# vgl-hub/kreeq

Hardware: AMD Instinct MI355X
Metric: distinct+total k-mers/sec at k=21 (count path) (higher is better)
Workload: dtype u64

## Files before the change

include/kreeq_amd.h:

```cpp
#ifndef KREEQ_AMD_H
#define KREEQ_AMD_H

#include <stdint.h>

#ifdef __cplusplus
extern "C" {
#endif

#define KQ_ABI_VERSION 4

typedef enum {
    KQ_OK = 0,
    KQ_ERR_INVALID = -1,
    KQ_ERR_NO_DEVICE = -2,
    KQ_ERR_HIP = -3,
    KQ_ERR_NOMEM = -4,
    KQ_ERR_TABLE_FULL = -5,
    KQ_ERR_CAPACITY = -6,
    KQ_ERR_MISMATCH = -7
} kq_status;

typedef struct kq_handle kq_handle;

typedef struct {
    uint64_t key;
    uint32_t fw[4], bw[4], cov;
    uint32_t hc;
} kq_entry;

typedef struct {
    uint32_t fw, bw, cov;
    uint8_t  isFw;
    uint8_t  pad[3];
} kq_dbgbase;

typedef struct {
    uint64_t total;
    uint64_t unique;
    uint64_t distinct;
    uint64_t missing;
    uint64_t edges;
} kq_stats;

typedef struct {
    uint64_t kmers_counted;
    uint64_t slots_used;
    uint64_t slots_total;
    uint64_t hc_used;
    uint64_t hc_total;
    uint64_t table_bytes;
    uint64_t table_passes;
} kq_info;


int  kq_create(kq_handle** out, int device, int k, int map_count, uint64_t capacity_hint);
void kq_destroy(kq_handle* h);
int  kq_clear(kq_handle* h);
int  kq_set_stream(kq_handle* h, void* hip_stream);
void* kq_get_stream(kq_handle* h);
enum { KQ_OPT_TRUST_CAPACITY = 1, KQ_OPT_COUNT_PATH = 2, KQ_OPT_SLICE_KMERS = 3, KQ_OPT_COUNT_MAP_RANGE = 4, KQ_OPT_PROFILE = 5,
       KQ_OPT_LOOKUP_PATH = 6, KQ_OPT_MERGE_PATH = 7, KQ_OPT_NARROW_MID = 8, KQ_OPT_PENDING_BYTES = 9, KQ_OPT_BUCKET_WINDOW = 10, KQ_OPT_OVERLAP = 11, KQ_OPT_COUNT_MAP_PASSES = 12, KQ_OPT_KERNEL_SET = 13, KQ_OPT_SHARD_WINDOW = 14,
       KQ_OPT_TEST_FAIL_PLAN = 100  };
int  kq_set_option(kq_handle* h, int option, int64_t value);
int  kq_get_profile(kq_handle* h, char* buf, uint64_t cap);
int  kq_sync(kq_handle* h);
int  kq_flush(kq_handle* h);
int  kq_get_info(kq_handle* h, kq_info* out);
const char* kq_last_error(void);
int  kq_abi_version(void);
int  kq_device_available(void);
int  kq_device_memory(int device, uint64_t* free_bytes, uint64_t* total_bytes);


int  kq_count_batch(kq_handle* h, const char* bases, uint64_t len);
int  kq_count_batch_dev(kq_handle* h, const char* d_bases, uint64_t len);

void* kq_host_alloc(uint64_t bytes);
void  kq_host_free(void* p);
int  kq_count_batch_async(kq_handle* h, const char* bases, uint64_t len, uint64_t* ticket);
int  kq_host_wait(kq_handle* h, uint64_t ticket);

void kq_pack_bases(const char* bases, uint64_t len, uint32_t* codes, uint16_t* inv);
int  kq_count_packed_dev(kq_handle* h, const uint32_t* d_codes, const uint16_t* d_inv, uint64_t n_bases);
int  kq_count_packed_async(kq_handle* h, const uint32_t* codes, const uint16_t* inv, uint64_t n_bases, uint64_t* ticket);

int  kq_pack_bases_dev(kq_handle* h, const char* d_bases, uint64_t len, uint32_t* d_codes, uint16_t* d_inv);

enum { KQ_FASTX_FASTQ = 1, KQ_FASTX_FASTA = 2 };
int  kq_parse_fastx_dev(kq_handle* h, const char* d_text, uint64_t len, int format, char* d_bases, uint64_t cap, uint64_t* n_bases);
int  kq_count_fastx_dev(kq_handle* h, const char* d_text, uint64_t len, int format);
int  kq_count_fastx_async(kq_handle* h, const char* text, uint64_t len, int format, uint64_t* ticket);

int  kq_emit_records(kq_handle* h, const char* bases, uint64_t len,
                     uint64_t* keys, uint8_t* edges, uint64_t cap, uint64_t* n_out);
int  kq_emit_partitioned_dev(kq_handle* h, const char* d_bases, uint64_t len, int n_parts,
                             uint64_t* d_keys, uint8_t* d_edges, uint64_t cap,
                             uint64_t* part_counts);

int  kq_emit_packed_dev(kq_handle* h, const char* d_bases, uint64_t len, int n_parts,
                        uint64_t* d_recs, uint64_t cap, uint64_t* part_counts);
int  kq_insert_packed_dev(kq_handle* h, const uint64_t* d_recs, uint64_t n);

int  kq_emit_sharded_dev(kq_handle* h, const char* d_bases, uint64_t len, int n_parts, uint32_t* d_recs, uint8_t* d_aux, uint64_t cap,
                         uint64_t* d_bucket_counts, uint64_t* part_counts);
int  kq_insert_sharded_dev(kq_handle* h, const uint32_t* d_recs, const uint8_t* d_aux, uint64_t n, int n_peers, const uint64_t* d_bucket_counts);

int  kq_emit_sharded8_dev(kq_handle* h, const char* d_bases, uint64_t len, int n_parts, uint64_t* d_recs, uint64_t cap,
                          uint64_t* d_bucket_counts, uint64_t* part_counts);
int  kq_insert_sharded8_dev(kq_handle* h, const uint64_t* d_recs, uint64_t n, int n_peers, const uint64_t* d_bucket_counts);

int  kq_insert_records(kq_handle* h, const uint64_t* keys, const uint8_t* edges, uint64_t n);
int  kq_insert_records_dev(kq_handle* h, const uint64_t* d_keys, const uint8_t* d_edges, uint64_t n);


int  kq_summary(kq_handle* h, kq_stats* out);
int  kq_histogram(kq_handle* h, uint64_t* cov, uint64_t* cnt, uint64_t cap, uint64_t* n_out);


int  kq_lookup_sequence(kq_handle* h, const char* bases, uint64_t len, uint32_t cov_cutoff,
                        uint16_t map_lo, uint16_t map_hi, kq_dbgbase* per_base,
                        uint64_t counters[3]);
int  kq_lookup_sequence_dev(kq_handle* h, const char* d_bases, uint64_t len, uint32_t cov_cutoff,
                            uint16_t map_lo, uint16_t map_hi, kq_dbgbase* d_per_base,
                            uint64_t* d_counters);


int  kq_lookup_keys(kq_handle* h, const uint64_t* keys, uint64_t n, kq_entry* out);

int  kq_branch_scan(kq_handle* h, const char* bases, uint64_t len, uint32_t cov_cutoff, uint8_t* flags);


int  kq_merge(kq_handle* dst, kq_handle* src);

int  kq_import(kq_handle* h, const kq_entry* entries, uint64_t n);
int  kq_export(kq_handle* h, uint16_t map_lo, uint16_t map_hi, kq_entry* out, uint64_t cap,
               uint64_t* n_out);

#ifdef __cplusplus
}
#endif
#endif
```

kreeq_amd/build.py:

```python
import os
import shutil
import subprocess

PKG = os.path.dirname(os.path.abspath(__file__))
ROOT = os.path.dirname(PKG)
LIB = os.path.join(PKG, "lib", "libkreeq_amd.so")
CLI = os.path.join(PKG, "bin", "kreeq")
HOSTLIB = os.path.join(PKG, "lib", "libkreeq_host.so")

HIP_SOURCES = [os.path.join(PKG, "csrc", "kreeq_amd.hip")]
HIP_DEPS = HIP_SOURCES + [os.path.join(PKG, "csrc", f) for f in ("kq_device.h", "kq_partition.h", "kq_kernels.h", "kq_fastx.h")] + [os.path.join(ROOT, "include", "kreeq_amd.h")]
HOST_DIR = os.path.join(PKG, "host")


def _stale(target, deps):
    if not os.path.exists(target):
        return True
    t = os.path.getmtime(target)
    return any(os.path.getmtime(d) > t for d in deps if os.path.exists(d))


def hipcc():
    for c in (shutil.which("hipcc"), "/opt/rocm/bin/hipcc"):
        if c and os.path.exists(c):
            return c
    raise RuntimeError("hipcc not found: the HIP library cannot be built (there is no CPU fallback)")


def build_lib(force=False, verbose=False, out=None, defines=()):
    target = out or LIB
    if force or _stale(target, HIP_DEPS):
        os.makedirs(os.path.dirname(target), exist_ok=True)
        cmd = [hipcc(), "-O3", "-std=c++17", "--offload-arch=gfx950", "-fPIC", "-shared", "-Wall", "-Wextra",
               "-o", target] + ["-D" + d for d in defines] + HIP_SOURCES
        if verbose:
            print(" ".join(cmd))
        subprocess.check_call(cmd)
    return target


def host_sources():
    if not os.path.isdir(HOST_DIR):
        return []
    return sorted(os.path.join(HOST_DIR, f) for f in os.listdir(HOST_DIR) if f.endswith(".cpp") and f != "hostlib.cpp")


def build_hostlib(force=False, verbose=False):
    srcs = [os.path.join(HOST_DIR, f) for f in ("hostlib.cpp", "kreeq_db.cpp")]
    deps = srcs + [os.path.join(HOST_DIR, "kreeq_db.h"), os.path.join(ROOT, "include", "kreeq_amd.h")]
    if force or _stale(HOSTLIB, deps):
        os.makedirs(os.path.dirname(HOSTLIB), exist_ok=True)
        cmd = ["g++", "-O2", "-std=c++17", "-Wall", "-Wextra", "-fPIC", "-shared", "-pthread", "-I", os.path.join(ROOT, "include"), "-o", HOSTLIB] + srcs
        if verbose:
            print(" ".join(cmd))
        subprocess.check_call(cmd)
    return HOSTLIB


def build_cli(force=False, verbose=False):
    srcs = host_sources()
    if not srcs:
        return None
    deps = srcs + [os.path.join(HOST_DIR, f) for f in os.listdir(HOST_DIR) if f.endswith(".h")] + [LIB]
    if force or _stale(CLI, deps):
        os.makedirs(os.path.dirname(CLI), exist_ok=True)
        cmd = ["g++", "-O2", "-std=c++17", "-Wall", "-Wextra", "-pthread", "-I", os.path.join(ROOT, "include"), "-o", CLI] + srcs + \
              ["-L", os.path.dirname(LIB), "-lkreeq_amd", "-lz", "-Wl,-rpath,$ORIGIN/../lib"]
        if verbose:
            print(" ".join(cmd))
        subprocess.check_call(cmd)
    return CLI


def build_all(force=False, verbose=False):
    build_lib(force, verbose)
    build_cli(force, verbose)
    build_hostlib(force, verbose)
```

kreeq_amd/capi.py:

```python
import ctypes as C
import os

import numpy as np

from . import build as _build

ENTRY_DTYPE = np.dtype([("key", "<u8"), ("fw", "<u4", 4), ("bw", "<u4", 4), ("cov", "<u4"), ("hc", "<u4")])
DBGBASE_DTYPE = np.dtype([("fw", "<u4"), ("bw", "<u4"), ("cov", "<u4"), ("isFw", "u1"), ("pad", "u1", 3)])

SYMBOLS = ["kq_create", "kq_destroy", "kq_clear", "kq_set_option", "kq_get_profile", "kq_set_stream", "kq_get_stream", "kq_sync", "kq_flush", "kq_get_info", "kq_last_error",
           "kq_abi_version", "kq_device_available", "kq_device_memory", "kq_count_batch", "kq_count_batch_dev", "kq_host_alloc", "kq_host_free", "kq_count_batch_async", "kq_host_wait", "kq_pack_bases", "kq_count_packed_dev", "kq_count_packed_async",
           "kq_pack_bases_dev", "kq_parse_fastx_dev", "kq_count_fastx_dev", "kq_count_fastx_async", "kq_emit_records",
           "kq_emit_partitioned_dev", "kq_emit_packed_dev", "kq_insert_packed_dev", "kq_emit_sharded_dev", "kq_insert_sharded_dev", "kq_emit_sharded8_dev", "kq_insert_sharded8_dev", "kq_insert_records", "kq_insert_records_dev", "kq_summary", "kq_histogram",
           "kq_lookup_sequence", "kq_lookup_sequence_dev", "kq_lookup_keys", "kq_branch_scan", "kq_merge", "kq_import", "kq_export"]

FASTX_FASTQ, FASTX_FASTA = 1, 2


class KqError(RuntimeError):
    def __init__(self, code, msg):
        super().__init__(f"kreeq_amd error {code}: {msg}")
        self.code = code


class Stats(C.Structure):
    _fields_ = [("total", C.c_uint64), ("unique", C.c_uint64), ("distinct", C.c_uint64), ("missing", C.c_uint64),
                ("edges", C.c_uint64)]


class Info(C.Structure):
    _fields_ = [("kmers_counted", C.c_uint64), ("slots_used", C.c_uint64), ("slots_total", C.c_uint64), ("hc_used", C.c_uint64),
                ("hc_total", C.c_uint64), ("table_bytes", C.c_uint64), ("table_passes", C.c_uint64)]


_lib = None


def lib_path():
    return _build.LIB


def _preload_process_hip_runtime():
    import importlib.util

    try:
        spec = importlib.util.find_spec("torch")
    except (ImportError, ValueError):
        spec = None
    if not spec or not spec.origin:
        return
    d = os.path.join(os.path.dirname(spec.origin), "lib")
    for name in ("libhsa-runtime64.so", "libamdhip64.so"):
        p = os.path.join(d, name)
        if os.path.exists(p):
            try:
                C.CDLL(p, mode=C.RTLD_GLOBAL)
            except OSError:
                return


def load():
    global _lib
    if _lib is not None:
        return _lib
    path = os.environ.get("KQ_LIB") or _build.LIB
    if not os.path.exists(path):
        raise KqError(-2, f"{path} is missing: build it with `python -c 'import __graft_entry__ as g; g.build()'` "
                          "(the product has no CPU fallback)")
    _preload_process_hip_runtime()
    L = C.CDLL(path)
    vp, u64, u32, u16, ci = C.c_void_p, C.c_uint64, C.c_uint32, C.c_uint16, C.c_int
    L.kq_create.argtypes = [C.POINTER(vp), ci, ci, ci, u64]
    L.kq_destroy.argtypes = [vp]
    L.kq_destroy.restype = None
    L.kq_clear.argtypes = [vp]
    L.kq_set_stream.argtypes = [vp, vp]
    L.kq_set_option.argtypes = [vp, ci, C.c_int64]
    L.kq_get_profile.argtypes = [vp, C.c_char_p, u64]
    L.kq_get_stream.argtypes = [vp]
    L.kq_get_stream.restype = vp
    L.kq_sync.argtypes = [vp]
    L.kq_flush.argtypes = [vp]
    L.kq_get_info.argtypes = [vp, C.POINTER(Info)]
    L.kq_last_error.restype = C.c_char_p
    L.kq_device_memory.argtypes = [ci, C.POINTER(u64), C.POINTER(u64)]
    L.kq_count_batch.argtypes = [vp, vp, u64]
    L.kq_count_batch_dev.argtypes = [vp, vp, u64]
    L.kq_host_alloc.argtypes = [u64]
    L.kq_host_alloc.restype = vp
    L.kq_host_free.argtypes = [vp]
    L.kq_host_free.restype = None
    L.kq_count_batch_async.argtypes = [vp, vp, u64, C.POINTER(u64)]
    L.kq_host_wait.argtypes = [vp, u64]
    L.kq_pack_bases.argtypes = [vp, u64, vp, vp]
    L.kq_pack_bases.restype = None
    L.kq_count_packed_dev.argtypes = [vp, vp, vp, u64]
    L.kq_count_packed_async.argtypes = [vp, vp, vp, u64, C.POINTER(u64)]
    L.kq_pack_bases_dev.argtypes = [vp, vp, u64, vp, vp]
    L.kq_parse_fastx_dev.argtypes = [vp, vp, u64, ci, vp, u64, C.POINTER(u64)]
    L.kq_count_fastx_dev.argtypes = [vp, vp, u64, ci]
    L.kq_count_fastx_async.argtypes = [vp, vp, u64, ci, C.POINTER(u64)]
    L.kq_emit_records.argtypes = [vp, vp, u64, vp, vp, u64, C.POINTER(u64)]
    L.kq_emit_partitioned_dev.argtypes = [vp, vp, u64, ci, vp, vp, u64, vp]
    L.kq_emit_packed_dev.argtypes = [vp, vp, u64, ci, vp, u64, vp]
    L.kq_insert_packed_dev.argtypes = [vp, vp, u64]
    L.kq_emit_sharded_dev.argtypes = [vp, vp, u64, ci, vp, vp, u64, vp, vp]
    L.kq_insert_sharded_dev.argtypes = [vp, vp, vp, u64, ci, vp]
    L.kq_emit_sharded8_dev.argtypes = [vp, vp, u64, ci, vp, u64, vp, vp]
    L.kq_insert_sharded8_dev.argtypes = [vp, vp, u64, ci, vp]
    L.kq_insert_records.argtypes = [vp, vp, vp, u64]
    L.kq_insert_records_dev.argtypes = [vp, vp, vp, u64]
    L.kq_summary.argtypes = [vp, C.POINTER(Stats)]
    L.kq_histogram.argtypes = [vp, vp, vp, u64, C.POINTER(u64)]
    L.kq_lookup_sequence.argtypes = [vp, vp, u64, u32, u16, u16, vp, vp]
    L.kq_lookup_sequence_dev.argtypes = [vp, vp, u64, u32, u16, u16, vp, vp]
    L.kq_lookup_keys.argtypes = [vp, vp, u64, vp]
    L.kq_branch_scan.argtypes = [vp, vp, u64, u32, vp]
    L.kq_merge.argtypes = [vp, vp]
    L.kq_import.argtypes = [vp, vp, u64]
    L.kq_export.argtypes = [vp, u16, u16, vp, u64, C.POINTER(u64)]
    _lib = L
    return L


def _check(rc):
    if rc != 0:
        raise KqError(rc, load().kq_last_error().decode(errors="replace"))


def _p(a):
    return a.ctypes.data_as(C.c_void_p) if a is not None else None


def pack_bases(bases: bytes):
    buf = np.frombuffer(bases, dtype=np.uint8)
    units = (len(buf) + 15) // 16
    codes, inv = np.zeros(max(units, 1), dtype=np.uint32), np.zeros(max(units, 1), dtype=np.uint16)
    load().kq_pack_bases(_p(buf) if len(buf) else None, len(buf), _p(codes), _p(inv))
    return codes[:units], inv[:units]


def device_available():
    return bool(load().kq_device_available())


def device_memory(device=0):
    f, t = C.c_uint64(0), C.c_uint64(0)
    _check(load().kq_device_memory(device, C.byref(f), C.byref(t)))
    return f.value, t.value


class KreeqDB:

    def __init__(self, k=21, map_count=128, device=0, capacity_hint=0):
        self.k, self.map_count, self.device = k, map_count, device
        self._h = C.c_void_p()
        _check(load().kq_create(C.byref(self._h), device, k, map_count, capacity_hint))

    def close(self, _load=load):
        if getattr(self, "_h", None):
            _load().kq_destroy(self._h)
            self._h = None

    __del__ = close

    @property
    def handle(self):
        return self._h

    def set_stream(self, hip_stream_ptr):
        _check(load().kq_set_stream(self._h, C.c_void_p(hip_stream_ptr)))

    def sync(self):
        _check(load().kq_sync(self._h))

    def flush(self):
        _check(load().kq_flush(self._h))

    def set_option(self, option, value):
        opt = {"trust_capacity": 1, "count_path": 2, "slice_kmers": 3, "count_map_range": 4, "profile": 5, "lookup_path": 6, "merge_path": 7, "narrow_mid": 8, "pending_bytes": 9, "bucket_window": 10, "overlap": 11, "count_map_passes": 12, "kernel_set": 13, "shard_window": 14, "test_fail_plan": 100}[option]
        if option == "count_map_range":
            value = int(value[0]) | (int(value[1]) << 16)
        if option in ("count_path", "lookup_path", "merge_path"):
            value = {"auto": 0, "direct": 1, "partitioned": 2}[value]
        _check(load().kq_set_option(self._h, opt, int(value)))

    def clear(self):
        _check(load().kq_clear(self._h))

    def profile(self):
        buf = C.create_string_buffer(1024)
        _check(load().kq_get_profile(self._h, buf, 1024))
        return {k: float(v) for k, v in (kv.split("=") for kv in buf.value.decode().split(";") if kv)}

    def info(self):
        i = Info()
        _check(load().kq_get_info(self._h, C.byref(i)))
        return {f: getattr(i, f) for f, _ in Info._fields_}

    def count_batch(self, bases: bytes):
        buf = np.frombuffer(bases, dtype=np.uint8)
        _check(load().kq_count_batch(self._h, _p(buf), len(buf)))

    def count_batch_async(self, host_ptr, n):
        t = C.c_uint64(0)
        _check(load().kq_count_batch_async(self._h, C.c_void_p(host_ptr), n, C.byref(t)))
        return t.value

    def count_packed_dev(self, codes_ptr, inv_ptr, n_bases):
        _check(load().kq_count_packed_dev(self._h, C.c_void_p(codes_ptr), C.c_void_p(inv_ptr), n_bases))

    def count_packed_async(self, codes_ptr, inv_ptr, n_bases):
        t = C.c_uint64(0)
        _check(load().kq_count_packed_async(self._h, C.c_void_p(codes_ptr), C.c_void_p(inv_ptr), n_bases, C.byref(t)))
        return t.value

    def pack_bases_dev(self, bases_ptr, n, codes_ptr, inv_ptr):
        _check(load().kq_pack_bases_dev(self._h, C.c_void_p(bases_ptr), n, C.c_void_p(codes_ptr), C.c_void_p(inv_ptr)))

    def parse_fastx_dev(self, text_ptr, n, fmt, out_ptr, cap):
        nb = C.c_uint64(0)
        rc = load().kq_parse_fastx_dev(self._h, C.c_void_p(text_ptr), n, fmt, C.c_void_p(out_ptr) if out_ptr else None, cap, C.byref(nb))
        if rc != 0:
            e = KqError(rc, load().kq_last_error().decode(errors="replace"))
            e.needed = nb.value
            raise e
        return nb.value

    def count_fastx_dev(self, text_ptr, n, fmt):
        _check(load().kq_count_fastx_dev(self._h, C.c_void_p(text_ptr), n, fmt))

    def count_fastx_async(self, host_ptr, n, fmt):
        t = C.c_uint64(0)
        _check(load().kq_count_fastx_async(self._h, C.c_void_p(host_ptr), n, fmt, C.byref(t)))
        return t.value

    def host_wait(self, ticket):
        _check(load().kq_host_wait(self._h, ticket))

    def count_batch_dev(self, ptr, n):
        _check(load().kq_count_batch_dev(self._h, C.c_void_p(ptr), n))

    def emit_records(self, bases: bytes):
        buf = np.frombuffer(bases, dtype=np.uint8)
        n = C.c_uint64(0)
        _check(load().kq_emit_records(self._h, _p(buf), len(buf), None, None, 0, C.byref(n)))
        keys = np.empty(n.value, dtype=np.uint64)
        edges = np.empty(n.value, dtype=np.uint8)
        if n.value:
            _check(load().kq_emit_records(self._h, _p(buf), len(buf), _p(keys), _p(edges), n.value, C.byref(n)))
        return keys, edges

    def emit_partitioned_dev(self, bases_ptr, n, n_parts, keys_ptr, edges_ptr, cap):
        counts = np.zeros(n_parts, dtype=np.uint64)
        _check(load().kq_emit_partitioned_dev(self._h, C.c_void_p(bases_ptr), n, n_parts, C.c_void_p(keys_ptr), C.c_void_p(edges_ptr),
                                              cap, _p(counts)))
        return counts

    def emit_packed_dev(self, bases_ptr, n, n_parts, recs_ptr, cap):
        counts = np.zeros(n_parts, dtype=np.uint64)
        _check(load().kq_emit_packed_dev(self._h, C.c_void_p(bases_ptr), n, n_parts, C.c_void_p(recs_ptr), cap, _p(counts)))
        return counts

    def insert_packed_dev(self, recs_ptr, n):
        _check(load().kq_insert_packed_dev(self._h, C.c_void_p(recs_ptr), n))

    def emit_sharded_dev(self, bases_ptr, n, n_parts, recs_ptr, aux_ptr, cap, bucket_counts_ptr, sync=True):
        counts = np.zeros(n_parts, dtype=np.uint64) if sync else None
        _check(load().kq_emit_sharded_dev(self._h, C.c_void_p(bases_ptr), n, n_parts, C.c_void_p(recs_ptr), C.c_void_p(aux_ptr), cap,
                                          C.c_void_p(bucket_counts_ptr), _p(counts)))
        return counts

    def insert_sharded_dev(self, recs_ptr, aux_ptr, n, n_peers, bucket_counts_ptr):
        _check(load().kq_insert_sharded_dev(self._h, C.c_void_p(recs_ptr), C.c_void_p(aux_ptr), n, n_peers, C.c_void_p(bucket_counts_ptr)))

    def emit_sharded8_dev(self, bases_ptr, n, n_parts, recs_ptr, cap, bucket_counts_ptr, sync=True):
        counts = np.zeros(n_parts, dtype=np.uint64) if sync else None
        _check(load().kq_emit_sharded8_dev(self._h, C.c_void_p(bases_ptr), n, n_parts, C.c_void_p(recs_ptr), cap,
                                           C.c_void_p(bucket_counts_ptr), _p(counts)))
        return counts

    def insert_sharded8_dev(self, recs_ptr, n, n_peers, bucket_counts_ptr):
        _check(load().kq_insert_sharded8_dev(self._h, C.c_void_p(recs_ptr), n, n_peers, C.c_void_p(bucket_counts_ptr)))

    def insert_records(self, keys, edges):
        keys = np.ascontiguousarray(keys, dtype=np.uint64)
        edges = np.ascontiguousarray(edges, dtype=np.uint8)
        assert len(keys) == len(edges)
        _check(load().kq_insert_records(self._h, _p(keys), _p(edges), len(keys)))

    def insert_records_dev(self, keys_ptr, edges_ptr, n):
        _check(load().kq_insert_records_dev(self._h, C.c_void_p(keys_ptr), C.c_void_p(edges_ptr), n))

    def summary(self, with_hist=False):
        st = Stats()
        _check(load().kq_summary(self._h, C.byref(st)))
        d = {f: getattr(st, f) for f, _ in Stats._fields_}
        if with_hist:
            n = C.c_uint64(0)
            _check(load().kq_histogram(self._h, None, None, 0, C.byref(n)))
            cov = np.zeros(n.value, dtype=np.uint64)
            cnt = np.zeros(n.value, dtype=np.uint64)
            _check(load().kq_histogram(self._h, _p(cov), _p(cnt), n.value, C.byref(n)))
            d["hist"] = dict(zip(cov.tolist(), cnt.tolist()))
        return d

    def lookup_sequence(self, bases: bytes, cov_cutoff=0, map_lo=0, map_hi=None, per_base=False, per_base_buf=None):
        if map_hi is None:
            map_hi = self.map_count
        buf = np.frombuffer(bases, dtype=np.uint8)
        ctr = np.zeros(3, dtype=np.uint64)
        pb = per_base_buf if per_base_buf is not None else (np.zeros(len(buf), dtype=DBGBASE_DTYPE) if per_base else None)
        _check(load().kq_lookup_sequence(self._h, _p(buf), len(buf), cov_cutoff, map_lo, map_hi, _p(pb), _p(ctr)))
        return ctr, pb

    def lookup_sequence_dev(self, bases_ptr, n, counters_ptr, cov_cutoff=0, map_lo=0, map_hi=None, per_base_ptr=None):
        if map_hi is None:
            map_hi = self.map_count
        _check(load().kq_lookup_sequence_dev(self._h, C.c_void_p(bases_ptr), n, cov_cutoff, map_lo, map_hi,
                                             C.c_void_p(per_base_ptr) if per_base_ptr else None, C.c_void_p(counters_ptr)))

    def lookup_keys(self, keys):
        keys = np.ascontiguousarray(keys, dtype=np.uint64)
        out = np.zeros(len(keys), dtype=ENTRY_DTYPE)
        _check(load().kq_lookup_keys(self._h, _p(keys), len(keys), _p(out)))
        return out

    def branch_scan(self, bases: bytes, cov_cutoff=0):
        buf = np.frombuffer(bases, dtype=np.uint8)
        flags = np.zeros(len(buf), dtype=np.uint8)
        _check(load().kq_branch_scan(self._h, _p(buf), len(buf), cov_cutoff, _p(flags)))
        return flags

    def merge(self, other):
        _check(load().kq_merge(self._h, other._h))

    def import_entries(self, entries):
        entries = np.ascontiguousarray(entries, dtype=ENTRY_DTYPE)
        _check(load().kq_import(self._h, _p(entries), len(entries)))

    def export(self, map_lo=0, map_hi=None):
        if map_hi is None:
            map_hi = self.map_count
        n = C.c_uint64(0)
        _check(load().kq_export(self._h, map_lo, map_hi, None, 0, C.byref(n)))
        out = np.zeros(n.value, dtype=ENTRY_DTYPE)
        if n.value:
            _check(load().kq_export(self._h, map_lo, map_hi, _p(out), n.value, C.byref(n)))
        return out
```

kreeq_amd/csrc/kq_kernels.h:

```cpp
#pragma once

#include <hip/hip_runtime.h>

#include <type_traits>

#include "../../include/kreeq_amd.h"
#include "kq_device.h"
#include "kq_partition.h"

using namespace kq;


__global__ __launch_bounds__(TILE_THREADS) void k_count_direct(TableView t, const uint8_t* __restrict__ ab,
                                                                uint64_t lead, uint64_t len, int k, EmitRange er, PartCfg filt,
                                                                const uint16_t* __restrict__ pinv ) {
    uint32_t n_new = 0;
    uint64_t n_kmers = 0;
    scan_tiles(ab, lead, len, k, [&](uint64_t pos, uint64_t fw, uint64_t rv, uint32_t prev, uint32_t next) {
        if (pos < er.lo || pos >= er.hi) return;
        const bool is_fw = fw < rv;
        const uint64_t key = is_fw ? fw : rv;
        if (filt.filt_lo != 0 || filt.filt_hi != filt.map_count) {
            const uint32_t m = map_index(key, filt.map_count, filt.map_mask);
            if (m < filt.filt_lo || m >= filt.filt_hi) return;
// ... 257 lines not shown
                else { recs[cg[it]] = (uint32_t)cv[it]; recs_aux[cg[it]] = (uint8_t)(cv[it] >> 48); }
            }
        }
    }
}

__global__ __launch_bounds__(1024) void k_lv_units(const unsigned long long* __restrict__ seg_off, const unsigned long long* __restrict__ seg_hi, LevelCfg lv,
                                                   unsigned long long* __restrict__ unit_base) {
    __shared__ unsigned long long s_part[1024];
    const uint32_t tid = threadIdx.x, per = (lv.n_seg + 1023) / 1024;
    const uint32_t lo = min(tid * per, lv.n_seg), hi = min(lo + per, lv.n_seg);
    unsigned long long sum = 0;
    for (uint32_t b = lo; b < hi; ++b) sum += (seg_hi[b] - seg_off[b] + P2_UNIT - 1) / P2_UNIT;
    s_part[tid] = sum;
    __syncthreads();
    if (tid < 64) {
        unsigned long long loc[16], tot = 0;
#pragma unroll
        for (int j = 0; j < 16; ++j) { loc[j] = s_part[tid * 16 + j]; tot += loc[j]; }
        unsigned long long incl = tot;
#pragma unroll
        for (int o = 1; o < 64; o <<= 1) { unsigned long long nn = __shfl_up(incl, o, 64); if ((int)tid >= o) incl += nn; }
        unsigned long long run = incl - tot;
#pragma unroll
        for (int j = 0; j < 16; ++j) { s_part[tid * 16 + j] = run; run += loc[j]; }
        if (tid == 63) unit_base[lv.n_seg] = incl;
    }
    __syncthreads();
    unsigned long long run = s_part[tid];
    for (uint32_t b = lo; b < hi; ++b) { unit_base[b] = run; run += (seg_hi[b] - seg_off[b] + P2_UNIT - 1) / P2_UNIT; }
}
__device__ __forceinline__ uint32_t seg_of_unit(const unsigned long long* unit_base, uint32_t n_seg, uint64_t u) {
    uint32_t lo = 0, hi = n_seg;
    while (hi - lo > 1) { uint32_t mid = (lo + hi) >> 1; if (unit_base[mid] <= u) lo = mid; else hi = mid; }
    return lo;
}
template <int FMT>
__global__ __launch_bounds__(MS_THREADS) void k_lv_hist(const uint64_t* __restrict__ recs, const uint8_t* __restrict__ , LevelCfg lv,
                                                        const unsigned long long* __restrict__ seg_off, const unsigned long long* __restrict__ seg_hi,
                                                        const unsigned long long* __restrict__ unit_base, uint32_t* __restrict__ m2) {
    __shared__ uint32_t s_hist[NB_MAX];
    const uint64_t n_units = unit_base[lv.n_seg];
    for (uint64_t u = blockIdx.x; u < n_units; u += gridDim.x) {
        const uint32_t b_in = seg_of_unit(unit_base, lv.n_seg, u);
        const uint32_t b = lv.spb > 1 ? b_in / lv.spb : b_in;
        const uint64_t lo = seg_off[b_in] + (u - unit_base[b_in]) * P2_UNIT;
        const uint64_t hi = lo + P2_UNIT < seg_hi[b_in] ? lo + P2_UNIT : seg_hi[b_in];
        for (uint32_t i = threadIdx.x; i < lv.nb; i += MS_THREADS) s_hist[i] = 0;
        __syncthreads();
        const uint64_t last = hi - 1;
        if (FMT == FMT_NARROW) {
            const uint4* v4 = reinterpret_cast<const uint4*>(recs);
            const uint64_t q0 = lo >> 2, q1 = (hi + 3) >> 2;
            for (uint64_t qb = q0; qb < q1; qb += 4ull * MS_THREADS) {
                uint4 q[4];
#pragma unroll
                for (int j = 0; j < 4; ++j) q[j] = v4[min(qb + (uint64_t)j * MS_THREADS + threadIdx.x, q1 - 1)];
#pragma unroll
                for (int j = 0; j < 4; ++j) {
                    const uint64_t qi = qb + (uint64_t)j * MS_THREADS + threadIdx.x;
                    const uint32_t e[4] = {q[j].x, q[j].y, q[j].z, q[j].w};
#pragma unroll
                    for (int c = 0; c < 4; ++c) {
                        const uint64_t ri = 4 * qi + c;
                        if (qi < q1 && ri >= lo && ri < hi) atomicAdd(&s_hist[narrow_bin(lv, b, e[c])], 1u);
                    }
                }
            }
        } else
        for (uint64_t base = lo; base < hi; base += 8ull * MS_THREADS) {
            uint64_t r[8];
#pragma unroll
            for (int j = 0; j < 8; ++j) {
                const uint64_t i = min(base + (uint64_t)j * MS_THREADS + threadIdx.x, last);
                r[j] = FMT == FMT_NARROW ? (uint64_t)reinterpret_cast<const uint32_t*>(recs)[i] : recs[i];
            }
#pragma unroll
            for (int j = 0; j < 8; ++j)
                if (base + (uint64_t)j * MS_THREADS + threadIdx.x < hi) {
                    const uint32_t bin = FMT == FMT_NARROW ? narrow_bin(lv, b, (uint32_t)r[j])
                        : FMT == FMT_TOP8 ? narrow_bin(lv, b, (uint32_t)(r[j] >> 32))
                        : (FMT == FMT_PACK8 && lv.top8) ? (uint32_t)(rec_hash<false>(r[j]) >> (64 - NARROW_CBITS))
                        : level_bin(lv, b, hash_region(lv.in_raw ? table_hash(r[j], lv.k) : rec_hash<FMT == FMT_WIDE>(r[j]), lv.n_regions));
                    atomicAdd(&s_hist[bin], 1u);
                }
        }
        __syncthreads();
        for (uint32_t i = threadIdx.x; i < lv.nb; i += MS_THREADS) m2[u * lv.nb + i] = s_hist[i];
        __syncthreads();
    }
}
__global__ __launch_bounds__(256) void k_lv_offsets(uint32_t* __restrict__ m2, LevelCfg lv, const unsigned long long* __restrict__ unit_base,
                                                    unsigned long long* __restrict__ group_count) {
    const uint64_t r = ((uint64_t)blockIdx.x * blockDim.x + threadIdx.x) >> 6;
    const uint32_t lane = threadIdx.x & 63;
    const uint32_t n_lseg = lv.n_seg / lv.spb;
    if (r >= (uint64_t)n_lseg * lv.nb) return;
    const uint32_t b = (uint32_t)(r / lv.nb), bin = (uint32_t)(r % lv.nb);
    const uint64_t u0 = unit_base[b * lv.spb], u1 = unit_base[(b + 1) * lv.spb];
    unsigned long long run = 0;
    for (uint64_t base = u0; base < u1; base += 64) {
        const uint64_t u = base + lane;
        const uint32_t c = u < u1 ? m2[u * lv.nb + bin] : 0u;
        unsigned long long incl = c;
#pragma unroll
        for (int o = 1; o < 64; o <<= 1) { const unsigned long long n = __shfl_up(incl, o, 64); if ((int)lane >= o) incl += n; }
        if (u < u1) m2[u * lv.nb + bin] = (uint32_t)(run + incl - c);
        run += __shfl(incl, 63, 64);
    }
    if (lane == 0) group_count[r] = run;
}
__global__ __launch_bounds__(256) void k_lv_offsets_thread(uint32_t* __restrict__ m2, LevelCfg lv, const unsigned long long* __restrict__ unit_base,
                                                           unsigned long long* __restrict__ group_count) {
    const uint64_t r = (uint64_t)blockIdx.x * blockDim.x + threadIdx.x;
    const uint32_t n_lseg = lv.n_seg / lv.spb;
    if (r >= (uint64_t)n_lseg * lv.nb) return;
    const uint32_t b = (uint32_t)(r / lv.nb), bin = (uint32_t)(r % lv.nb);
    const uint64_t u0 = unit_base[b * lv.spb], u1 = unit_base[(b + 1) * lv.spb];
    unsigned long long run = 0;
    for (uint64_t u = u0; u < u1; ++u) {
        const uint32_t c = m2[u * lv.nb + bin];
        m2[u * lv.nb + bin] = (uint32_t)run;
        run += c;
    }
    group_count[r] = run;
}
#ifndef KQ_LV_THREADS
#define KQ_LV_THREADS 512
#define KQ_LV_ITEMS 8
#define KQ_LV_OCC 4
#endif
constexpr int LV_THREADS = KQ_LV_THREADS, LV_ITEMS = KQ_LV_ITEMS, LV_TILE = LV_THREADS * LV_ITEMS;
template <int FMT, int NBC>
__global__ __launch_bounds__(LV_THREADS, KQ_LV_OCC) void k_lv_scatter(const uint64_t* __restrict__ recs, const uint8_t* __restrict__ recs_aux, LevelCfg lv,
                                                           const unsigned long long* __restrict__ seg_off, const unsigned long long* __restrict__ seg_hi,
                                                           const unsigned long long* __restrict__ unit_base, const uint32_t* __restrict__ m2,
                                                           const unsigned long long* __restrict__ group_base, uint64_t* __restrict__ out,
                                                           uint8_t* __restrict__ out_aux) {
    constexpr bool WIDE = FMT == FMT_WIDE, TIGHT = FMT == FMT_NARROW_TO_TIGHT, NARROW = FMT == FMT_NARROW || TIGHT, CONVERT = FMT == FMT_PACK8_TO_NARROW,
                   TOP8 = FMT == FMT_TOP8, HAS_AUX = WIDE || NARROW;
    constexpr int MS_FMT = (CONVERT || TIGHT) ? FMT_NARROW : TOP8 ? FMT_PACK8 : FMT;
    const uint32_t* recs32 = reinterpret_cast<const uint32_t*>(recs);
    __shared__ MsShared<NBC, MS_FMT, LV_TILE> s;
    __shared__ uint32_t s_rst[TIGHT ? NBC : 1];
    const uint32_t nb = lv.nb;
    const uint64_t n_units = unit_base[lv.n_seg];
    for (uint64_t u = blockIdx.x; u < n_units; u += gridDim.x) {
        const uint32_t b_in = seg_of_unit(unit_base, lv.n_seg, u);
        const uint32_t b = lv.spb > 1 ? b_in / lv.spb : b_in;
        const uint64_t lo = seg_off[b_in] + (u - unit_base[b_in]) * P2_UNIT;
        const uint64_t hi = lo + P2_UNIT < seg_hi[b_in] ? lo + P2_UNIT : seg_hi[b_in];
        for (uint32_t i = threadIdx.x; i < nb; i += LV_THREADS)
            s.gbase[i] = (uint32_t)(group_base[(uint64_t)b * nb + i] + m2[u * nb + i]);
        if (TIGHT) {
            const uint32_t first = (b >> lv.nr_shift) * lv.nr_rps + (b & ((1u << lv.nr_shift) - 1u)) * lv.nr_sub;
            for (uint32_t i = threadIdx.x; i < nb; i += LV_THREADS) s_rst[i] = lv.rstart[first + i];
        }
        __syncthreads();
        uint64_t nxt[LV_ITEMS];
        uint32_t nxt_aux[LV_ITEMS];
        const uint64_t last = hi - 1;
#pragma unroll
        for (int j = 0; j < LV_ITEMS; ++j) {
            const uint64_t i = min(lo + (uint64_t)j * LV_THREADS + threadIdx.x, last);
            nxt[j] = NARROW ? (uint64_t)recs32[i] : recs[i];
            nxt_aux[j] = HAS_AUX ? recs_aux[i] : 0;
        }
#pragma unroll
        for (int j = 0; j < LV_ITEMS; ++j) { landed(nxt[j]); if (HAS_AUX) landed(nxt_aux[j]); }
        for (uint64_t pos = lo; pos < hi; pos += LV_TILE) {
            uint64_t rec[LV_ITEMS];
            uint32_t aux[LV_ITEMS], bin[LV_ITEMS];
#pragma unroll
            for (int j = 0; j < LV_ITEMS; ++j) {
                const uint64_t i = pos + (uint64_t)j * LV_THREADS + threadIdx.x;
                rec[j] = (WIDE && lv.in_raw) ? table_hash(nxt[j], lv.k) : nxt[j];
                aux[j] = nxt_aux[j];
                if (TIGHT) {
                    const uint32_t bn = i >= hi ? nb : narrow_bin(lv, b, (uint32_t)rec[j]);
                    rec[j] = narrow_word(tight_rec(b >> lv.nr_shift, (uint32_t)rec[j], aux[j], s_rst[bn < nb ? bn : 0u]), 0u, bn);
                }
                else if (NARROW) rec[j] = narrow_word((uint32_t)rec[j], aux[j], i >= hi ? nb : narrow_bin(lv, b, (uint32_t)rec[j]));
                else if (CONVERT) {
                    const uint64_t hh = rec_hash<false>(rec[j]);
                    rec[j] = narrow_word(narrow_main(hh), narrow_aux(hh, (uint32_t)(rec[j] >> REC_EDGE_SHIFT) & 63u), i >= hi ? nb : (uint32_t)(hh >> (64 - NARROW_CBITS)));
                }
                else if (TOP8) bin[j] = i >= hi ? nb : narrow_bin(lv, b, (uint32_t)(rec[j] >> 32));
                else bin[j] = i >= hi ? nb : level_bin(lv, b, hash_region(rec_hash<WIDE>(rec[j]), lv.n_regions));
            }
#pragma unroll
            for (int j = 0; j < LV_ITEMS; ++j) {
                const uint64_t i = min(pos + LV_TILE + (uint64_t)j * LV_THREADS + threadIdx.x, last);
                nxt[j] = NARROW ? (uint64_t)recs32[i] : recs[i];
                nxt_aux[j] = HAS_AUX ? recs_aux[i] : 0;
            }
            block_multisplit<MS_FMT, LV_THREADS, LV_ITEMS>(s, rec, aux, bin, nb, out, out_aux, [&] {
#pragma unroll
                for (int j = 0; j < LV_ITEMS; ++j) { landed(nxt[j]); if (HAS_AUX) landed(nxt_aux[j]); }
            }, NBC <= 512 ? lv.rep_shift : 0u);
        }
    }
}
#ifndef KQ_LVS_OCC
#define KQ_LVS_OCC 4
#define KQ_LVS_OCC_TIGHT 4
#endif
template <bool TIGHT>
__global__ __launch_bounds__(LV_THREADS, TIGHT ? KQ_LVS_OCC_TIGHT : KQ_LVS_OCC) void k_lv_scatter_s(const uint32_t* __restrict__ recs32, const uint8_t* __restrict__ recs_aux, LevelCfg lv,
                                                           const unsigned long long* __restrict__ seg_off, const unsigned long long* __restrict__ seg_hi,
                                                           const unsigned long long* __restrict__ unit_base, const uint32_t* __restrict__ m2,
                                                           const unsigned long long* __restrict__ group_base, uint32_t* __restrict__ out,
                                                           uint8_t* __restrict__ out_aux) {
    constexpr int NC = 512;
    static_assert(LV_THREADS == NC && LV_ITEMS == 8, "one counter per thread");
    __shared__ uint64_t s_buf[LV_TILE];
    __shared__ uint32_t s_hist[2][NC], s_loff[NC + 1], s_grel[NC], s_wave[LV_THREADS / 64];
    __shared__ uint32_t s_rst[TIGHT ? NC : 1];
    const int tid = threadIdx.x;
    const uint32_t nb = lv.nb, rs = lv.rep_shift, n_ctr = (nb + 1) << rs;
    const uint32_t sub = (uint32_t)tid & ((1u << rs) - 1u), my_bin = (uint32_t)tid >> rs;
    const bool own_bin = sub == 0 && my_bin < nb;
    const uint64_t n_units = unit_base[lv.n_seg];
    for (uint64_t u = blockIdx.x; u < n_units; u += gridDim.x) {
        const uint32_t b_in = seg_of_unit(unit_base, lv.n_seg, u);
        const uint32_t b = lv.spb > 1 ? b_in / lv.spb : b_in;
        const uint64_t lo = seg_off[b_in] + (u - unit_base[b_in]) * P2_UNIT;
        const uint64_t hi = lo + P2_UNIT < seg_hi[b_in] ? lo + P2_UNIT : seg_hi[b_in];
        uint32_t gabs = own_bin ? (uint32_t)(group_base[(uint64_t)b * nb + my_bin] + m2[u * nb + my_bin]) : 0u;
        if (TIGHT) {
            const uint32_t first = (b >> lv.nr_shift) * lv.nr_rps + (b & ((1u << lv.nr_shift) - 1u)) * lv.nr_sub;
            if ((uint32_t)tid < nb) s_rst[tid] = lv.rstart[first + tid];
        }
        s_hist[0][tid] = 0;
        __syncthreads();
        uint32_t nxt[LV_ITEMS], nxt_aux[LV_ITEMS];
        const uint64_t last = hi - 1;
#pragma unroll
        for (int j = 0; j < LV_ITEMS; ++j) {
            const uint64_t i = min(lo + (uint64_t)j * LV_THREADS + tid, last);
            nxt[j] = recs32[i];
            nxt_aux[j] = recs_aux[i];
        }
#pragma unroll
        for (int j = 0; j < LV_ITEMS; ++j) { landed(nxt[j]); landed(nxt_aux[j]); }
        uint32_t par = 0;
        for (uint64_t pos = lo; pos < hi; pos += LV_TILE, par ^= 1u) {
            uint32_t* hist = s_hist[par];
            uint64_t w[LV_ITEMS];
#pragma unroll
            for (int j = 0; j < LV_ITEMS; ++j) {
                const uint64_t i = pos + (uint64_t)j * LV_THREADS + tid;
                const uint32_t bn = i >= hi ? nb : narrow_bin(lv, b, nxt[j]);
                w[j] = TIGHT ? narrow_word(tight_rec(b >> lv.nr_shift, nxt[j], nxt_aux[j], s_rst[bn < nb ? bn : 0u]), 0u, bn) : narrow_word(nxt[j], nxt_aux[j], bn);
                if (bn != nb) atomicAdd(&hist[(bn << rs) | sub], 1u);
            }
#pragma unroll
            for (int j = 0; j < LV_ITEMS; ++j) {
                const uint64_t i = min(pos + LV_TILE + (uint64_t)j * LV_THREADS + tid, last);
                nxt[j] = recs32[i];
                nxt_aux[j] = recs_aux[i];
            }
            __syncthreads();
            const uint32_t cnt = (uint32_t)tid < n_ctr ? hist[tid] : 0u;
            uint32_t incl = cnt;
#pragma unroll
            for (int o = 1; o < 64; o <<= 1) { const uint32_t n = __shfl_up(incl, o, 64); if ((tid & 63) >= o) incl += n; }
            if ((tid & 63) == 63) s_wave[tid >> 6] = incl;
            s_hist[par ^ 1u][tid] = 0;
            __syncthreads();
            uint32_t excl = incl - cnt;
            for (int v = 0; v < (tid >> 6); ++v) excl += s_wave[v];
            s_loff[tid] = excl;
            hist[tid] = excl;
            if (own_bin) s_grel[my_bin] = gabs - excl;
            __syncthreads();
            if (own_bin) gabs += s_loff[(my_bin + 1) << rs] - excl;
#pragma unroll
            for (int j = 0; j < LV_ITEMS; ++j) {
                const uint32_t bn = narrow_word_bin(w[j]);
                if (bn != nb) s_buf[atomicAdd(&hist[(bn << rs) | sub], 1u)] = w[j];
            }
            __syncthreads();
            const uint32_t total = s_loff[nb << rs];
            uint64_t cv[LV_ITEMS];
            uint32_t cg[LV_ITEMS];
#pragma unroll
            for (int it = 0; it < LV_ITEMS; ++it) cv[it] = s_buf[tid + it * LV_THREADS];
#pragma unroll
            for (int it = 0; it < LV_ITEMS; ++it) cg[it] = s_grel[(uint32_t)(tid + it * LV_THREADS) < total ? narrow_word_bin(cv[it]) : 0u] + (tid + it * LV_THREADS);
#pragma unroll
            for (int j = 0; j < LV_ITEMS; ++j) { landed(nxt[j]); landed(nxt_aux[j]); }
#pragma unroll
            for (int it = 0; it < LV_ITEMS; ++it) {
                if ((uint32_t)(tid + it * LV_THREADS) < total) {
                    out[cg[it]] = (uint32_t)cv[it];
                    if (!TIGHT) out_aux[cg[it]] = (uint8_t)(cv[it] >> 48);
                }
            }
        }
    }
}
__global__ void k_set2(unsigned long long* p, unsigned long long a, unsigned long long b) { p[0] = a; p[1] = b; }

constexpr uint32_t SCAN_CHUNK = 16384;
__global__ __launch_bounds__(1024) void k_scan_sums(const unsigned long long* __restrict__ a, uint64_t n, unsigned long long* __restrict__ sums) {
    const uint64_t lo = (uint64_t)blockIdx.x * SCAN_CHUNK, hi = lo + SCAN_CHUNK < n ? lo + SCAN_CHUNK : n;
    unsigned long long v = 0;
    for (uint64_t i = lo + threadIdx.x; i < hi; i += 1024) v += a[i];
    uint64_t t = block_sum(v);
    if (threadIdx.x == 0) sums[blockIdx.x] = t;
}
__global__ __launch_bounds__(1024) void k_scan_apply(unsigned long long* __restrict__ a, uint64_t n, const unsigned long long* __restrict__ sums) {
    __shared__ unsigned long long s_part[1024];
    const uint64_t lo = (uint64_t)blockIdx.x * SCAN_CHUNK + (uint64_t)threadIdx.x * (SCAN_CHUNK / 1024);
    unsigned long long v[SCAN_CHUNK / 1024], sum = 0;
#pragma unroll
    for (uint32_t j = 0; j < SCAN_CHUNK / 1024; ++j) { v[j] = lo + j < n ? a[lo + j] : 0; sum += v[j]; }
    s_part[threadIdx.x] = sum;
    __syncthreads();
    if (threadIdx.x < 64) {
        unsigned long long loc[16], tot = 0;
#pragma unroll
        for (int j = 0; j < 16; ++j) { loc[j] = s_part[threadIdx.x * 16 + j]; tot += loc[j]; }
        unsigned long long incl = tot;
#pragma unroll
        for (int o = 1; o < 64; o <<= 1) { unsigned long long nn = __shfl_up(incl, o, 64); if ((int)threadIdx.x >= o) incl += nn; }
        unsigned long long run = incl - tot;
#pragma unroll
        for (int j = 0; j < 16; ++j) { s_part[threadIdx.x * 16 + j] = run; run += loc[j]; }
    }
    __syncthreads();
    unsigned long long run = sums[blockIdx.x] + s_part[threadIdx.x];
#pragma unroll
    for (uint32_t j = 0; j < SCAN_CHUNK / 1024; ++j) { if (lo + j < n) a[lo + j] = run; run += v[j]; }
}


template <class T> __device__ __forceinline__ T ld_global(const T* p) { return *(const __attribute__((address_space(1))) T*)p; }

template <uint32_t GRP>
struct SetTickets {
    uint64_t lo; uint32_t cnt, first, n_grp;
    __device__ __forceinline__ void build(const P3Set* __restrict__ sets, uint32_t n_sets, uint64_t r, uint32_t lane) {
        lo = 0; cnt = 0;
        if (lane < n_sets) { const unsigned long long* b = ld_global(&sets[lane].base); lo = ld_global(b + r); cnt = (uint32_t)(ld_global(b + r + 1) - lo); }
        const uint32_t mine = (cnt + GRP - 1) / GRP;
        uint32_t incl = mine;
#pragma unroll
        for (int o = 1; o < P3_MAX_SETS; o <<= 1) { const uint32_t v = __shfl_up(incl, o, 64); if ((int)lane >= o) incl += v; }
        first = incl - mine;
        n_grp = __builtin_amdgcn_readlane(incl, 63);
    }
    __device__ __forceinline__ void locate(uint32_t g, uint32_t& q, uint32_t& off, uint32_t& q_cnt, uint64_t& q_lo) const {
        const uint64_t nonempty = __ballot(cnt != 0);
        const uint64_t m = __ballot(cnt != 0 && first <= g);
        q = (g < n_grp && m) ? 63u - (uint32_t)__clzll((unsigned long long)m) : (uint32_t)__ffsll((unsigned long long)nonempty) - 1u;
        const uint32_t f = __builtin_amdgcn_readlane(first, q);
        q_cnt = __builtin_amdgcn_readlane(cnt, q);
        q_lo = ((uint64_t)__builtin_amdgcn_readlane((uint32_t)(lo >> 32), q) << 32) | __builtin_amdgcn_readlane((uint32_t)lo, q);
        off = (g < n_grp ? g - f : 0u) * GRP;
    }
};

template <int THREADS, bool HOT, uint32_t GRP>
__device__ __forceinline__ bool region_gate(SetTickets<GRP>& tk, const TableView& t, const P3Set* __restrict__ sets, uint32_t n_sets, uint64_t r,
                                            int table_is_empty, unsigned long long* __restrict__ hot_list ) {
    const int tid = threadIdx.x;
    tk.build(sets, n_sets, r, (uint32_t)tid & 63u);
    uint64_t n_recs = tk.cnt;
#pragma unroll
    for (int o = 32; o > 0; o >>= 1) n_recs += __shfl_xor(n_recs, o, 64);
    if (n_recs == 0) {
        if (!HOT && table_is_empty == 2) {
            ulonglong2* g2 = reinterpret_cast<ulonglong2*>(t.slots + (r << REGION_SHIFT));
            for (int i = tid; i < (int)REGION_SLOTS; i += THREADS) g2[i] = make_ulonglong2(0ull, 0ull);
        }
        return false;
    }
    if (!HOT && n_recs > 32ull * REGION_SLOTS) {
        if (tid == 0) hot_list[1 + atomicAdd(&hot_list[0], 1ull)] = r;
        return false;
    }
    return true;
}
constexpr int HC_LDS = 64;
__device__ __forceinline__ void hc_lds_reset(uint64_t (&hckey)[HC_LDS], uint32_t (&hccnt)[HC_LDS][8]) {
    const int tid = threadIdx.x;
    if (tid < HC_LDS) {
        hckey[tid] = EMPTY_KEY;
#pragma unroll
        for (int e = 0; e < 8; ++e) hccnt[tid][e] = 0;
    }
}
__device__ __forceinline__ void hc_lds_add(const TableView& t, uint64_t (&hckey)[HC_LDS], uint32_t (&hccnt)[HC_LDS][8], uint64_t h, const uint32_t (&e)[8]) {
    const uint64_t key = key_of_hash(h, t.k);
    int hslot = -1;
    uint32_t hp = (uint32_t)(h >> 40) & (HC_LDS - 1);
    for (int probe = 0; probe < HC_LDS; ++probe, hp = (hp + 1) & (HC_LDS - 1)) {
        uint64_t cur = __hip_atomic_load(&hckey[hp], __ATOMIC_RELAXED, __HIP_MEMORY_SCOPE_WORKGROUP);
        if (cur == EMPTY_KEY) cur = atomicCAS((unsigned long long*)&hckey[hp], (unsigned long long)EMPTY_KEY, (unsigned long long)key);
        if (cur == EMPTY_KEY || cur == key) { hslot = (int)hp; break; }
    }
    if (hslot >= 0) {
#pragma unroll
        for (int w = 0; w < 8; ++w) if (e[w]) atomicAdd(&hccnt[hslot][w], e[w]);
    } else {
        hc_add(t, h, 0, 0, e);
    }
}
__device__ __forceinline__ void hc_lds_flush(const TableView& t, uint64_t (&hckey)[HC_LDS], uint32_t (&hccnt)[HC_LDS][8]) {
    const int tid = threadIdx.x;
    if (tid < HC_LDS && hckey[tid] != EMPTY_KEY) {
        HcSlot* hs = hc_upsert(t, hckey[tid]);
        if (!hs) atomicOr(&t.st->err_hc_full, 1u);
        else {
#pragma unroll
            for (int e = 0; e < 8; ++e) if (hccnt[tid][e]) atomicAdd((unsigned long long*)&hs->cnt[e], (unsigned long long)hccnt[tid][e]);
        }
    }
}
template <class C>
__device__ __forceinline__ void region_totals_wave(uint32_t n_new, uint32_t n_ok, C& s_new, C& s_kmers) {
#pragma unroll
    for (int o = 32; o > 0; o >>= 1) { n_new += __shfl_down(n_new, o, 64); n_ok += __shfl_down(n_ok, o, 64); }
    if ((threadIdx.x & 63) == 0) { if (n_new) atomicAdd(&s_new, (C)n_new); if (n_ok) atomicAdd(&s_kmers, (C)n_ok); }
}
template <class C>
__device__ __forceinline__ void region_totals_store(const TableView& t, const C& s_new, const C& s_kmers) {
    if (threadIdx.x == 0) {
        if (s_new) atomicAdd(&t.st->slots_used, (unsigned long long)s_new);
        if (s_kmers) atomicAdd(&t.st->kmers_added, (unsigned long long)s_kmers);
    }
}

#ifndef KQ_P3_THREADS
#define KQ_P3_THREADS 512
#define KQ_P3_OCC 6
#define KQ_P3_PF 2
#endif
constexpr int P3_THREADS = KQ_P3_THREADS;
template <int FMT, bool HOT>
__global__ __launch_bounds__(P3_THREADS, HOT ? 4 : KQ_P3_OCC) void k_count_regions(TableView t, const P3Set* __restrict__ sets, uint32_t n_sets,
                                                              int aux_fmt, int table_is_empty,
                                                              unsigned long long* __restrict__ hot_list ,
                                                              uint32_t narrow_rps ) {
    constexpr bool WIDE = FMT == FMT_WIDE, NARROW = FMT == FMT_NARROW, TOP8 = FMT == FMT_TOP8, HAS_AUX = WIDE || NARROW;
    constexpr int PF = KQ_P3_PF;
    constexpr uint64_t GRP = 64ull * PF;
// ... 844 lines not shown
```

kreeq_amd/csrc/kq_partition.h:

```cpp
#pragma once
#include "kq_device.h"

namespace kq {

constexpr int MS_THREADS = 256;
constexpr int MS_ITEMS = 16;
constexpr int MS_TILE = MS_THREADS * MS_ITEMS;
constexpr int NB_MAX = 2048;
constexpr int SEG_MAX = 65536;
constexpr uint32_t SUB_BITS_MAX = 8;
constexpr int REC_EDGE_SHIFT = 56;
constexpr int PART_MAX_K = 28;
constexpr int AUX_IDX6 = 0, AUX_EDGE_BYTE = 1, AUX_TIGHT = 2;

struct PartCfg {
    uint64_t n_regions;
    uint32_t g_shift;
    uint32_t n_coarse;
    uint32_t mode;
    uint32_t map_count;
    uint32_t map_mask;
    uint32_t filt_lo, filt_hi;
    uint32_t raw_out;
    uint32_t narrow;
    uint32_t owner_sub;
    uint32_t sub_bits;
    uint32_t win_lo, win_hi;
    uint32_t n_rng;
};

constexpr int P3_MAX_SETS = 64;
struct P3Set { const uint64_t* recs; const uint8_t* aux; const unsigned long long* base; uint64_t n_max; };

struct LevelCfg {
    uint64_t n_regions;
    uint32_t n_seg, nb, seg_shift, out_shift;
    uint32_t in_raw;
    uint32_t k;
    uint32_t narrow;
    uint32_t top8;
    uint32_t nr_shift, nr_rps, nr_sub, nr_div, nr_inv;
    uint32_t nr_mid, nr_fshift, nr_fmask, nr_f24;
    uint32_t spb;
    uint32_t rep_shift;
    const uint32_t* rstart = nullptr;
};
__device__ __forceinline__ uint32_t level_bin(const LevelCfg& lv, uint32_t b, uint64_t region) {
    return (uint32_t)(region >> lv.out_shift) - (lv.seg_shift >= 32 ? 0u : (b << (lv.seg_shift - lv.out_shift)));
}

__device__ __forceinline__ uint32_t edge_idx6(bool is_fw, uint32_t prev, uint32_t next) {
    uint32_t f, b;
    if (is_fw) { f = next < 4 ? next : 7u; b = prev < 4 ? prev : 7u; }
    else       { f = prev < 4 ? 3u - prev : 7u; b = next < 4 ? 3u - next : 7u; }
    return f | (b << 3);
}
__device__ __forceinline__ uint32_t edge_idx6_any(bool is_fw, uint32_t prev, uint32_t next) {
    const uint32_t f = is_fw ? next : prev, b = is_fw ? prev : next, m = is_fw ? 0u : 0x1Bu;
    return (f | (b << 3)) ^ m;
}
__device__ __forceinline__ uint64_t rec_pack(uint64_t key, bool is_fw, uint32_t prev, uint32_t next) {
    return key | ((uint64_t)edge_idx6(is_fw, prev, next) << REC_EDGE_SHIFT);
}
__device__ __forceinline__ uint64_t idx6_to_pack(uint32_t v) {
    const uint32_t f = v & 7u, b = (v >> 3) & 7u;
    return (f < 4 ? 1ull << (8 * f) : 0ull) | (b < 4 ? 1ull << (8 * (4 + b)) : 0ull);
}
__device__ __forceinline__ uint32_t idx6_to_edge_byte(uint32_t v) {
    const uint32_t f = v & 7u, b = (v >> 3) & 7u;
    return (f < 4 ? 1u << (7 - f) : 0u) | (b < 4 ? 1u << (7 - (4 + b)) : 0u);
}
__device__ __forceinline__ uint64_t rec_key(uint64_t rec) { return rec & ((1ull << REC_EDGE_SHIFT) - 1); }
__device__ __forceinline__ uint64_t rec_edge_pack(uint64_t rec) {
    const uint32_t f = (uint32_t)(rec >> REC_EDGE_SHIFT) & 7u, b = (uint32_t)(rec >> (REC_EDGE_SHIFT + 3)) & 7u;
    return (f < 4 ? 1ull << (8 * f) : 0ull) | (b < 4 ? 1ull << (8 * (4 + b)) : 0ull);
}
template <bool WIDE>
__device__ __forceinline__ uint64_t rec_hash(uint64_t rec) { return WIDE ? rec : rec << 8; }
__device__ __forceinline__ uint64_t rec_pack_hash(uint64_t h, bool is_fw, uint32_t prev, uint32_t next) {
    return (h >> 8) | ((uint64_t)edge_idx6(is_fw, prev, next) << REC_EDGE_SHIFT);
}

constexpr int FMT_PACK8 = 0, FMT_WIDE = 1, FMT_NARROW = 2;
constexpr int FMT_PACK8_TO_NARROW = 3;
constexpr uint32_t NARROW_CBITS = 8, NARROW_MAX_K = 21;
constexpr int FMT_TOP8 = 4;
constexpr int FMT_TIGHT = 5;
constexpr int FMT_NARROW_TO_TIGHT = 6;
constexpr uint64_t TIGHT_MIN_REGIONS = 1ull << 16;
__device__ __forceinline__ uint32_t tight_rec(uint32_t bucket, uint32_t main32, uint32_t aux, uint32_t rstart_r) {
    const uint32_t d = ((bucket << (32 - NARROW_CBITS)) | (main32 >> NARROW_CBITS)) - rstart_r;
    return (d << 16) | ((main32 & 0xFFu) << 8) | ((aux & 3u) << 6) | (aux >> 2);
}
__device__ __forceinline__ uint64_t tight_hash(uint32_t t, uint32_t rstart_r) { return ((uint64_t)((t >> 16) + rstart_r) << 32) | ((uint64_t)((t >> 6) & 1023u) << 22); }
__device__ __forceinline__ uint64_t top8_rec(uint64_t h, uint32_t idx6) { return ((h << NARROW_CBITS) & ~63ull) | idx6; }
__device__ __forceinline__ uint64_t top8_hash(uint32_t bucket, uint64_t rec) { return ((uint64_t)bucket << (64 - NARROW_CBITS)) | ((rec & ~63ull) >> NARROW_CBITS); }
__device__ __forceinline__ uint32_t narrow_main(uint64_t h) { return (uint32_t)(h >> (32 - NARROW_CBITS)); }
__device__ __forceinline__ uint32_t narrow_aux(uint64_t h, uint32_t idx6) { return ((uint32_t)(h >> (30 - NARROW_CBITS)) & 3u) | (idx6 << 2); }
__device__ __forceinline__ uint64_t narrow_hash(uint32_t bucket, uint32_t main32, uint32_t aux) {
    return ((uint64_t)bucket << (64 - NARROW_CBITS)) | ((uint64_t)main32 << (32 - NARROW_CBITS)) | ((uint64_t)(aux & 3u) << (30 - NARROW_CBITS));
}
__device__ __forceinline__ uint64_t narrow_word(uint32_t main32, uint32_t aux, uint32_t bin) { return (uint64_t)main32 | ((uint64_t)(bin | (aux << 16)) << 32); }
__device__ __forceinline__ uint32_t narrow_word_bin(uint64_t w) { return (uint32_t)(w >> 32) & 0xFFFFu; }
__device__ __forceinline__ uint32_t narrow_region(uint32_t bucket, uint32_t main32, uint64_t n_regions) {
    return __umulhi((bucket << (32 - NARROW_CBITS)) | (main32 >> NARROW_CBITS), (uint32_t)n_regions);
}
__device__ __forceinline__ uint32_t narrow_bin(const LevelCfg& lv, uint32_t , uint32_t main32) {
    const uint32_t f = main32 >> NARROW_CBITS;
    if (lv.nr_mid) return f >> lv.nr_fshift;
    const uint32_t fs = f & lv.nr_fmask;
    return lv.nr_f24 ? umul24u(fs, lv.nr_sub) >> lv.nr_fshift : (uint32_t)(((uint64_t)fs * lv.nr_sub) >> lv.nr_fshift);
}

template <int NBC, int FMT, int TILE = MS_TILE>
struct MsShared {
    static constexpr int tile = TILE;
    uint64_t stage[TILE];
    uint16_t sbin[FMT != FMT_NARROW ? TILE : 4];
    uint8_t  saux[FMT == FMT_WIDE ? TILE : 8];
    uint32_t hist[NBC];
    uint32_t loff[NBC];
    uint32_t gbase[NBC];
    uint32_t wave_sum[16];
};

template <int THREADS, class S>
__device__ __forceinline__ void ms_scan(S& s, uint32_t nb) {
    constexpr int NBC = (int)(sizeof(s.hist) / sizeof(uint32_t));
    constexpr int MS_BINS_PER_THREAD = (NBC + THREADS - 1) / THREADS;
    const int tid = threadIdx.x;
    uint32_t v[MS_BINS_PER_THREAD], sum = 0;
#pragma unroll
    for (int j = 0; j < MS_BINS_PER_THREAD; ++j) { uint32_t b = MS_BINS_PER_THREAD * tid + j; v[j] = (b < nb) ? s.hist[b] : 0; sum += v[j]; }
    uint32_t incl = sum;
#pragma unroll
    for (int o = 1; o < 64; o <<= 1) { uint32_t n = __shfl_up(incl, o, 64); if ((tid & 63) >= o) incl += n; }
    if ((tid & 63) == 63) s.wave_sum[tid >> 6] = incl;
    __syncthreads();
    uint32_t base = 0;
    for (int w = 0; w < (tid >> 6); ++w) base += s.wave_sum[w];
    uint32_t run = base + incl - sum;
#pragma unroll
    for (int j = 0; j < MS_BINS_PER_THREAD; ++j) { uint32_t b = MS_BINS_PER_THREAD * tid + j; if (b < nb) s.loff[b] = run; run += v[j]; }
    __syncthreads();
}

__device__ __forceinline__ void landed(uint32_t& v) { asm volatile("" : "+v"(v)); }
__device__ __forceinline__ void landed(uint64_t& v) { asm volatile("" : "+v"(v)); }
struct NoHook { __device__ __forceinline__ void operator()() const {} };
template <int FMT, int THREADS = MS_THREADS, int ITEMS = MS_ITEMS, class S, class F = NoHook>
__device__ __forceinline__ void block_multisplit(S& s, const uint64_t (&rec)[ITEMS], const uint32_t (&aux)[ITEMS],
                                                 const uint32_t (&bin)[ITEMS], uint32_t nb,
                                                 uint64_t* __restrict__ out, uint8_t* __restrict__ out_aux, F pre_store = F(), uint32_t rs = 0) {
    const int tid = threadIdx.x;
    const uint32_t sub = (uint32_t)tid & ((1u << rs) - 1u), n_ctr = (nb + 1) << rs;
    for (uint32_t b = tid; b < n_ctr; b += THREADS) s.hist[b] = 0;
    __syncthreads();
    static_assert(THREADS * ITEMS <= S::tile, "round size");
    uint32_t rank[ITEMS];
#pragma unroll
    for (int i = 0; i < ITEMS; ++i) {
        const uint32_t b = FMT == FMT_NARROW ? narrow_word_bin(rec[i]) : bin[i];
        rank[i] = 0;
        if (b != nb) rank[i] = atomicAdd(&s.hist[(b << rs) | sub], 1u);
    }
    __syncthreads();
    ms_scan<THREADS>(s, n_ctr);
    for (uint32_t b = tid; b < nb; b += THREADS) s.gbase[b] -= s.loff[b << rs];
#pragma unroll
    for (int i = 0; i < ITEMS; ++i) {
        const uint32_t b = FMT == FMT_NARROW ? narrow_word_bin(rec[i]) : bin[i];
        if (b == nb) continue;
        const uint32_t p = s.loff[(b << rs) | sub] + rank[i];
        if (FMT == FMT_NARROW) {
            s.stage[p] = rec[i];
        } else {
            s.stage[p] = rec[i];
            s.sbin[p] = (uint16_t)bin[i];
            if (FMT == FMT_WIDE) s.saux[p] = (uint8_t)aux[i];
        }
    }
    __syncthreads();
    const uint32_t total = s.loff[nb << rs];
    uint32_t cb[ITEMS];
    uint32_t cg[ITEMS];
    uint64_t cv[ITEMS];
    if (FMT == FMT_NARROW) {
#pragma unroll
        for (int it = 0; it < ITEMS; ++it) { cv[it] = s.stage[tid + it * THREADS]; cb[it] = (uint32_t)(tid + it * THREADS) < total ? narrow_word_bin(cv[it]) : 0u; }
    } else {
#pragma unroll
        for (int it = 0; it < ITEMS; ++it) { const uint32_t j = tid + it * THREADS; cb[it] = j < total ? s.sbin[j] : 0u; cv[it] = s.stage[j]; }
    }
#pragma unroll
    for (int it = 0; it < ITEMS; ++it) cg[it] = s.gbase[cb[it]] + (tid + it * THREADS);
    pre_store();
#pragma unroll
    for (int it = 0; it < ITEMS; ++it) {
// ... 34 lines not shown
```

kreeq_amd/csrc/kreeq_amd.hip:

```cpp
#include <hip/hip_runtime.h>
#include <hipcub/hipcub.hpp>

#include <algorithm>
#include <cstdarg>
#include <cstdio>
#include <cstdlib>
#include <cstring>
#include <mutex>
#include <new>
#include <numeric>
#include <string>
#include <thread>
#include <type_traits>
#include <vector>

#include "../../include/kreeq_amd.h"
#include "kq_device.h"
#include "kq_partition.h"

using namespace kq;

#include "kq_kernels.h"
#include "kq_fastx.h"


static thread_local std::string g_err;
static int fail(int code, const char* fmt, ...) {
    char buf[512];
    va_list ap; va_start(ap, fmt); vsnprintf(buf, sizeof buf, fmt, ap); va_end(ap);
    g_err = buf;
    return code;
}
#define HIPC(expr)                                                                                   \
    do {                                                                                             \
        hipError_t e_ = (expr);                                                                      \
        if (e_ != hipSuccess)                                                                        \
            return fail(e_ == hipErrorOutOfMemory ? KQ_ERR_NOMEM : KQ_ERR_HIP, "%s: %s (%s:%d)", #expr, \
                        hipGetErrorString(e_), __FILE__, __LINE__);                                  \
    } while (0)

struct Scrambled {
    void* p = nullptr; size_t bytes = 0, chunk = 0;
    std::vector<hipMemGenericAllocationHandle_t> hs;
    bool vmm = false;
};
static void scr_free(Scrambled& b) {
    if (!b.p) return;
    (void)hipDeviceSynchronize();
    if (b.vmm) {
        (void)hipMemUnmap(b.p, b.hs.size() * b.chunk);
        for (auto& hnd : b.hs) (void)hipMemRelease(hnd);
        (void)hipMemAddressFree(b.p, b.hs.size() * b.chunk);
    } else (void)hipFree(b.p);
    b = Scrambled();
}
static bool scr_try_vmm(Scrambled& b, size_t bytes, int device) {
    static const size_t chunk_mb = getenv("KQ_SCRAMBLE_MB") ? (size_t)atoi(getenv("KQ_SCRAMBLE_MB")) : 2;
    if (!chunk_mb) return false;
    hipMemAllocationProp prop = {};
    prop.type = hipMemAllocationTypePinned; prop.location.type = hipMemLocationTypeDevice; prop.location.id = device;
    size_t gran = 0;
    if (hipMemGetAllocationGranularity(&gran, &prop, hipMemAllocationGranularityMinimum) != hipSuccess || !gran) { (void)hipGetLastError(); return false; }
    const size_t chunk = ((chunk_mb << 20) + gran - 1) / gran * gran, n = (bytes + chunk - 1) / chunk;
    void* base = nullptr;
    if (hipMemAddressReserve(&base, n * chunk, 0, nullptr, 0) != hipSuccess) { (void)hipGetLastError(); return false; }
    std::vector<hipMemGenericAllocationHandle_t> hs;
    hs.reserve(n);
    bool ok = true;
    for (size_t i = 0; i < n && ok; ++i) { hipMemGenericAllocationHandle_t hnd; ok = hipMemCreate(&hnd, chunk, &prop, 0) == hipSuccess; if (ok) hs.push_back(hnd); }
    size_t mapped = 0;
    if (ok) {
        size_t mul = 7919;
        while (std::gcd(mul, n) != 1) ++mul;
        for (; mapped < n && ok; ++mapped) ok = hipMemMap((char*)base + mapped * chunk, chunk, 0, hs[(mapped * mul + 13) % n], 0) == hipSuccess;
        if (!ok) --mapped;
    }
    if (ok) {
        hipMemAccessDesc acc = {};
        acc.location = prop.location; acc.flags = hipMemAccessFlagsProtReadWrite;
        ok = hipMemSetAccess(base, n * chunk, &acc, 1) == hipSuccess;
    }
    if (!ok) {
        (void)hipGetLastError();
        if (mapped) (void)hipMemUnmap(base, mapped * chunk);
        for (auto& hnd : hs) (void)hipMemRelease(hnd);
        (void)hipMemAddressFree(base, n * chunk);
        return false;
    }
    b.p = base; b.bytes = n * chunk; b.chunk = chunk; b.hs.swap(hs); b.vmm = true;
    return true;
}
static int scr_ensure(Scrambled& b, size_t need, int device) {
    if (b.bytes >= need) return KQ_OK;
    scr_free(b);
    const size_t sz = need + std::min<size_t>(need / 4, (size_t)256 << 20) + 4096;
    if (scr_try_vmm(b, sz, device)) return KQ_OK;
    if (hipMalloc(&b.p, sz) != hipSuccess) { (void)hipGetLastError(); b.p = nullptr; return fail(KQ_ERR_NOMEM, "partition scratch allocation failed"); }
    b.bytes = sz; b.vmm = false;
    return KQ_OK;
}

struct DevBuf { void* p = nullptr; size_t bytes = 0; };
struct ScratchSet { DevBuf part; Scrambled part2; };

struct kq_handle;
static void arena_release(kq_handle* h);
struct kq_handle {
    int device = 0, k = 0, map_count = 0;
    hipStream_t own_stream = nullptr, stream = nullptr;
    int n_cu = 256;
    Slot* slots = nullptr;
    uint64_t n_regions = 0;
    uint32_t win_lo = 0, win_hi = 256;
    bool windowed = false;
    HcSlot* hc = nullptr;
    uint64_t hc_cap = 0;
    uint32_t* rstart = nullptr;
    DevState* st = nullptr;
    DevState* st_host = nullptr;
    DevBuf scratch;
    DevBuf stage;
    uint64_t kmers_bound = 0;
    uint64_t used_bound = 0;
    uint64_t hc_check_at = 0;
    bool table_empty = true;
    uint32_t mid_rps = 2048;
    int merge_path = 0;
    int lookup_path = 0;
    bool slots_dirty = false;
    bool trust_capacity = false;
    int count_path = 0;
    uint64_t slice_kmers = 1ull << 28;
    bool slice_user = false;
    uint32_t filt_lo = 0, filt_hi = 0;
    bool profile = false;
    std::vector<std::pair<const char*, hipEvent_t>> marks;
    ScratchSet work, fork_work;
    hipStream_t base = nullptr;
    hipStream_t fork_stream[2] = {nullptr, nullptr};
    bool fork_busy[2] = {false, false};
    bool fork_stale[2] = {false, false};
    static constexpr int EV_RING = 64;
    hipEvent_t ev_ring[EV_RING] = {};
    uint64_t ev_next = 0;
    hipEvent_t ev_pass = nullptr;
    int overlap = 1;
    int kernel_set = 0;
    struct HistKey { const void* ab; const void* pinv; uint64_t lead, len, er_lo, er_hi; uint32_t g1, n_rng; int k;
                     bool operator==(const HistKey& o) const { return ab == o.ab && pinv == o.pinv && lead == o.lead && len == o.len && er_lo == o.er_lo && er_hi == o.er_hi && g1 == o.g1 && n_rng == o.n_rng && k == o.k; } };
    struct HistEntry { HistKey key; unsigned long long* m1_all; size_t bytes; };
    std::vector<HistEntry> hist_cache;
    size_t hist_cache_bytes = 0;
    int map_passes = 1;
    void* arena = nullptr; size_t arena_bytes = 0, arena_used = 0;
    Scrambled arena_scr;
    P3Set* d_sets = nullptr;
    int n_pend = 0, pend_fmt = -1, pend_aux_fmt = 0;
    uint64_t pend_records = 0;
    int64_t pend_budget = -1;
    uint64_t table_passes = 0;
    static constexpr int IN_SLOTS = 3, IN_TICKETS = 512;
    hipStream_t copy_stream = nullptr;
    DevBuf in_buf[IN_SLOTS];
    hipEvent_t in_consumed[IN_SLOTS] = {nullptr, nullptr, nullptr};
    std::vector<hipEvent_t> in_copied;
    uint64_t in_next = 0;
    std::mutex in_m;
    uint8_t in_bad[IN_TICKETS] = {};
    DevBuf fx_units, fx_out, in_cmp[IN_SLOTS];
    FxResult* fx_res = nullptr;
    FxResult* fx_res_host = nullptr;
    int fx_bad = 0;
    bool hist_cache_off = false;
    bool test_fail_plan = false;
    DevBuf hot;

    TableView view() const {
        TableView v; v.slots = slots - (reg_lo() << REGION_SHIFT); v.n_regions = n_regions; v.hc = hc; v.hc_mask = hc_cap - 1; v.st = st; v.k = (uint32_t)k;
        v.reg_lo = reg_lo(); v.reg_hi = reg_hi();
        v.rps = k >= HI_K ? (uint32_t)(n_regions >> 8) : 0u;
        v.rstart = rstart;
        return v;
    }
    uint64_t reg_lo() const { return windowed ? (uint64_t)win_lo * (n_regions >> 8) : 0; }
    uint64_t reg_hi() const { return windowed ? (uint64_t)win_hi * (n_regions >> 8) : n_regions; }
    uint64_t n_alloc_regions() const { return reg_hi() - reg_lo(); }
    uint64_t n_slots() const { return n_alloc_regions() << REGION_SHIFT; }
};

static void marks_reset(kq_handle* h);
static int flush_pending(kq_handle* h);

static int ev_get(kq_handle* h, hipEvent_t* out) {
    hipEvent_t& e = h->ev_ring[h->ev_next++ % kq_handle::EV_RING];
    if (!e) HIPC(hipEventCreateWithFlags(&e, hipEventDisableTiming));
    else HIPC(hipEventSynchronize(e));
    *out = e;
    return KQ_OK;
}
static int join_forks(kq_handle* h) {
    for (int w = 0; w < 2; ++w) {
        if (!h->fork_busy[w]) continue;
        hipEvent_t e; int rc = ev_get(h, &e); if (rc) return rc;
        HIPC(hipEventRecord(e, h->fork_stream[w]));
        HIPC(hipStreamWaitEvent(h->base, e, 0));
        h->fork_busy[w] = false;
    }
    return KQ_OK;
}

static int grid_for(const kq_handle* h, uint64_t work_items, int per_block, int per_cu = 8) {
    uint64_t blocks = (work_items + per_block - 1) / per_block;
    uint64_t cap = (uint64_t)h->n_cu * per_cu;
    if (blocks > cap) blocks = cap;
    if (blocks < 1) blocks = 1;
    return (int)blocks;
}

static void arena_release(kq_handle* h) {
    if (!h->arena) return;
    if (h->arena_scr.p) scr_free(h->arena_scr); else (void)hipFree(h->arena);
    h->arena = nullptr; h->arena_bytes = 0;
}
static int ensure_buf(DevBuf& b, size_t need) {
    if (b.bytes >= need) return KQ_OK;
    if (b.p) { HIPC(hipFree(b.p)); b = DevBuf(); }
    size_t sz = need + std::min<size_t>(need / 4, (size_t)256 << 20) + 4096;
    HIPC(hipMalloc(&b.p, sz));
    b.bytes = sz;
    return KQ_OK;
}

static void clear_words(kq_handle* h, void* p, uint32_t words_per_slot, uint64_t n_slots) {
    const uint64_t n_pairs = n_slots * words_per_slot / 2;
    hipLaunchKernelGGL(k_clear_slots, dim3(grid_for(h, n_pairs, 256)), dim3(256), 0, h->stream, (ulonglong2*)p, words_per_slot, n_pairs);
}
static void clear_main(kq_handle* h, Slot* p, uint64_t n_slots) { (void)hipMemsetAsync(p, 0, (size_t)n_slots * sizeof(Slot), h->stream); }
static void materialize(kq_handle* h) {
    if (!h->slots_dirty) return;
    clear_main(h, h->slots, h->n_slots());
    h->slots_dirty = false;
}
static int alloc_main(kq_handle* h, uint64_t n_regions, uint64_t alloc_regions, Slot** out, uint32_t** rstart_out) {
    Slot* p = nullptr;
    uint32_t* rs = nullptr;
    size_t bytes = (size_t)(alloc_regions << REGION_SHIFT) * sizeof(Slot);
    HIPC(hipMalloc((void**)&p, bytes));
    if (hipMalloc((void**)&rs, (size_t)(n_regions + 1) * sizeof(uint32_t)) != hipSuccess) { (void)hipFree(p); return fail(KQ_ERR_NOMEM, "region index allocation failed"); }
    clear_main(h, p, alloc_regions << REGION_SHIFT);
    hipLaunchKernelGGL(k_region_starts, dim3(grid_for(h, n_regions + 1, 256)), dim3(256), 0, h->stream, rs, n_regions);
    *out = p; *rstart_out = rs;
    return KQ_OK;
}
static int alloc_hc(kq_handle* h, uint64_t cap, HcSlot** out) {
    HcSlot* p = nullptr;
    size_t bytes = (size_t)cap * sizeof(HcSlot);
    HIPC(hipMalloc((void**)&p, bytes));
    clear_words(h, p, sizeof(HcSlot) / 8, cap);
    *out = p;
    return KQ_OK;
}

static int read_state_raw(kq_handle* h) {
    HIPC(hipMemcpyAsync(h->st_host, h->st, sizeof(DevState), hipMemcpyDeviceToHost, h->stream));
    HIPC(hipStreamSynchronize(h->stream));
    return KQ_OK;
}
static int read_state(kq_handle* h) {
    int frc = flush_pending(h);
    if (frc) return frc;
    return read_state_raw(h);
}
static int check_errors(kq_handle* h) {
    int rc = read_state(h);
    if (rc) return rc;
    if (h->st_host->err_table_full) return fail(KQ_ERR_TABLE_FULL, "k-mer table region overflow (slots %llu / %llu)",
                                                 (unsigned long long)h->st_host->slots_used, (unsigned long long)h->n_slots());
    if (h->st_host->err_hc_full) return fail(KQ_ERR_TABLE_FULL, "high-copy side table overflow (%llu / %llu)",
                                              (unsigned long long)h->st_host->hc_used, (unsigned long long)h->hc_cap);
    return KQ_OK;
}

static int grow_main(kq_handle* h, uint64_t need_slots) {
    int frc = flush_pending(h);
    if (frc) return frc;
    uint64_t want = h->n_slots(), new_regions = h->n_regions;
    while (want < need_slots) { want *= 2; new_regions *= 2; }
    if (new_regions >= (1ull << 32)) return fail(KQ_ERR_TABLE_FULL, "cannot grow k-mer table to %llu slots: region index overflow", (unsigned long long)want);
    Slot* fresh = nullptr;
    uint32_t* fresh_rs = nullptr;
    int rc = alloc_main(h, new_regions, want >> REGION_SHIFT, &fresh, &fresh_rs);
    if (rc) return rc == KQ_ERR_NOMEM ? fail(KQ_ERR_TABLE_FULL, "cannot grow k-mer table to %llu slots: out of device memory",
                                             (unsigned long long)want) : rc;
    Slot* old = h->slots; const uint64_t n_old = h->n_slots();
    const TableView old_view = h->view();
    uint32_t* old_rs = h->rstart;
    h->slots = fresh; h->n_regions = new_regions; h->rstart = fresh_rs;
    if (h->slots_dirty) h->slots_dirty = false;
    else hipLaunchKernelGGL(k_rehash, dim3(grid_for(h, n_old, 256)), dim3(256), 0, h->stream, h->view(), old_view);
    HIPC(hipStreamSynchronize(h->stream));
    HIPC(hipFree(old));
    if (old_rs) HIPC(hipFree(old_rs));
    return KQ_OK;
}
static int grow_hc(kq_handle* h, uint64_t need) {
    uint64_t want = h->hc_cap;
    while (want < need) want *= 2;
    HcSlot* fresh = nullptr;
    int rc = alloc_hc(h, want, &fresh);
    if (rc) return rc;
    HcSlot* old = h->hc; const uint64_t n_old = h->hc_cap;
    h->hc = fresh; h->hc_cap = want;
    HIPC(hipMemsetAsync(&h->st->hc_used, 0, sizeof(unsigned long long), h->stream));
    hipLaunchKernelGGL(k_rehash_hc, dim3(grid_for(h, n_old, 256)), dim3(256), 0, h->stream, h->view(), old, n_old);
    HIPC(hipStreamSynchronize(h->stream));
    HIPC(hipFree(old));
    return KQ_OK;
}

constexpr uint64_t HC_CAP_BIG = 1ull << 25;
static int reserve(kq_handle* h, uint64_t extra, uint64_t extra_instances) {
    int rc;
    bool state_read = false;
    if (!h->trust_capacity) {
        uint64_t need = (uint64_t)((double)(h->used_bound + extra) / 0.85) + REGION_SLOTS;
        if (need > h->n_slots()) {
            rc = read_state(h); if (rc) return rc;
            state_read = true;
            h->used_bound = h->st_host->slots_used;
            need = (uint64_t)((double)(h->used_bound + extra) / 0.85) + REGION_SLOTS;
            if (need > h->n_slots()) { rc = grow_main(h, need); if (rc) return rc; }
        }
    }
    h->used_bound += extra;
    h->kmers_bound += extra_instances;
    const uint64_t bound = h->kmers_bound / 255 + 1;
    uint64_t need_hc = 2 * std::min<uint64_t>(bound, 1ull << 23);
    if (bound > (1ull << 23)) need_hc = HC_CAP_BIG;
    if (bound > (1ull << 23) && h->kmers_bound >= h->hc_check_at && h->n_pend == 0) {
        if (!state_read) { rc = read_state_raw(h); if (rc) return rc; }
        need_hc = std::max<uint64_t>(need_hc, 8 * h->st_host->hc_used);
        h->hc_check_at = 2 * h->kmers_bound;
    }
    if (need_hc > h->hc_cap) { rc = grow_hc(h, need_hc); if (rc) return rc; }
    return KQ_OK;
}

static inline void aligned_view(const char* d, const uint8_t** ab, uint64_t* lead) {
    uintptr_t p = (uintptr_t)d;
    *lead = p & 15;
    *ab = (const uint8_t*)(p - *lead);
}

static int stage_in(kq_handle* h, const void* host, size_t bytes, void** dev) {
    int rc = ensure_buf(h->stage, bytes + 64);
    if (rc) return rc;
    if (bytes) HIPC(hipMemcpyAsync(h->stage.p, host, bytes, hipMemcpyHostToDevice, h->stream));
    *dev = h->stage.p;
    return KQ_OK;
}

static void parallel_sort_entries(kq_entry* a, uint64_t n) {
    auto less = [](const kq_entry& x, const kq_entry& y) { return x.key < y.key; };
    unsigned hw = std::thread::hardware_concurrency();
    unsigned t = std::max(1u, std::min(16u, hw ? hw : 1u));
    while (t > 1 && n / t < (1u << 16)) t /= 2;
    if (t <= 1) { std::sort(a, a + n, less); return; }
    std::vector<uint64_t> cut(t + 1);
    for (unsigned i = 0; i <= t; ++i) cut[i] = n * i / t;
    {
        std::vector<std::thread> th;
        for (unsigned i = 0; i < t; ++i) th.emplace_back([&, i] { std::sort(a + cut[i], a + cut[i + 1], less); });
        for (auto& x : th) x.join();
    }
    for (unsigned width = 1; width < t; width *= 2) {
        std::vector<std::thread> th;
        for (unsigned i = 0; i + width < t; i += 2 * width) {
            const uint64_t lo = cut[i], mid = cut[i + width], hi = cut[std::min(i + 2 * width, t)];
            th.emplace_back([=] { std::inplace_merge(a + lo, a + mid, a + hi, less); });
        }
        for (auto& x : th) x.join();
    }
}

extern "C" {

const char* kq_last_error(void) { return g_err.c_str(); }
int kq_abi_version(void) { return KQ_ABI_VERSION; }

int kq_device_available(void) {
    int n = 0;
    if (hipGetDeviceCount(&n) != hipSuccess || n <= 0) return 0;
    hipDeviceProp_t p;
    if (hipGetDeviceProperties(&p, 0) != hipSuccess) return 0;
    return strncmp(p.gcnArchName, "gfx950", 6) == 0 ? 1 : 0;
}

int kq_device_memory(int device, uint64_t* free_bytes, uint64_t* total_bytes) {
    if (!free_bytes || !total_bytes) return fail(KQ_ERR_INVALID, "null argument");
    int n = 0;
    if (hipGetDeviceCount(&n) != hipSuccess || n <= 0) return fail(KQ_ERR_NO_DEVICE, "no HIP device visible (this library has no CPU path)");
    if (device < 0 || device >= n) return fail(KQ_ERR_NO_DEVICE, "device %d out of range (%d visible)", device, n);
    HIPC(hipSetDevice(device));
    size_t f = 0, t = 0;
    HIPC(hipMemGetInfo(&f, &t));
    *free_bytes = f; *total_bytes = t;
    return KQ_OK;
}

static uint64_t round_regions(uint64_t regions, int k) {
    if (regions < 16) regions = 16;
    if (regions >= (uint64_t)NB_MAX || k >= HI_K) regions = (regions + 255) / 256 * 256;
    if (regions >= (1ull << 19)) {
        uint32_t sbits = 3;
        while (sbits < SUB_BITS_MAX && (((regions + 255) / 256) >> sbits) > 256) ++sbits;
        const uint64_t unit = 256ull << sbits;
        regions = (regions + unit - 1) / unit * unit;
    }
    return regions;
}
static int set_window(kq_handle* h, uint32_t lo, uint32_t hi, bool shard = false) {
    if (lo >= hi || hi > 256) return fail(KQ_ERR_INVALID, "bucket window [%u, %u) is not a range of the 256 hash-prefix buckets", lo, hi);
    if (shard && h->k > (int)NARROW_MAX_K && h->k < HI_K)
        return fail(KQ_ERR_INVALID, "shard windows need k <= %u (5-byte records) or k >= %d (8-byte hash-remainder records); k = %u..%d shards own map ranges", NARROW_MAX_K, HI_K, NARROW_MAX_K + 1, HI_K - 1);
    if (!shard && h->k > (int)NARROW_MAX_K) return fail(KQ_ERR_INVALID, "bucket windows need k <= %u (5-byte records)", NARROW_MAX_K);
    if (!h->table_empty || h->n_pend || h->kmers_bound) return fail(KQ_ERR_INVALID, "the bucket window is chosen before anything is counted");
    if (h->windowed && hi - lo == h->win_hi - h->win_lo && !(lo == 0 && hi == 256)) {
        HIPC(hipStreamSynchronize(h->stream));
        h->win_lo = lo; h->win_hi = hi;
        return KQ_OK;
    }
    const uint64_t nb = hi - lo;
    const uint64_t alloc_now = h->n_alloc_regions();
    uint64_t virt = round_regions(std::max<uint64_t>((alloc_now + nb - 1) / nb * 256, (uint64_t)NB_MAX), h->k);
    if (virt >= (1ull << 32)) return fail(KQ_ERR_INVALID, "bucket window too narrow for a table of %llu regions", (unsigned long long)alloc_now);
    HIPC(hipStreamSynchronize(h->stream));
    const bool windowed = !(lo == 0 && hi == 256);
    const uint64_t alloc_new = windowed ? (uint64_t)(hi - lo) * (virt >> 8) : virt;
    Slot* fresh = nullptr;
    uint32_t* fresh_rs = nullptr;
    int rc = alloc_main(h, virt, alloc_new, &fresh, &fresh_rs);
    if (rc) return rc;
    HIPC(hipStreamSynchronize(h->stream));
    if (h->slots) (void)hipFree(h->slots);
    if (h->rstart) (void)hipFree(h->rstart);
    h->slots = fresh; h->rstart = fresh_rs;
    h->n_regions = virt; h->win_lo = lo; h->win_hi = hi; h->windowed = windowed;
    h->slots_dirty = false;
    return KQ_OK;
}

int kq_create(kq_handle** out, int device, int k, int map_count, uint64_t capacity_hint) {
    if (!out) return fail(KQ_ERR_INVALID, "out is null");
    *out = nullptr;
    if (k < 2 || k > 32) return fail(KQ_ERR_INVALID, "k must be in 2..32 (got %d)", k);
    if (map_count < 1 || map_count > 65535) return fail(KQ_ERR_INVALID, "map_count must be in 1..65535 (got %d)", map_count);
    int n = 0;
    if (hipGetDeviceCount(&n) != hipSuccess || n <= 0) return fail(KQ_ERR_NO_DEVICE, "no HIP device visible (this library has no CPU path)");
    if (device < 0 || device >= n) return fail(KQ_ERR_NO_DEVICE, "device %d out of range (%d visible)", device, n);
    HIPC(hipSetDevice(device));
    hipDeviceProp_t prop;
    HIPC(hipGetDeviceProperties(&prop, device));
    if (strncmp(prop.gcnArchName, "gfx950", 6) != 0)
        return fail(KQ_ERR_NO_DEVICE, "device %d is %s; this library carries gfx950 code only", device, prop.gcnArchName);
    kq_handle* h = new (std::nothrow) kq_handle();
    if (!h) return fail(KQ_ERR_NOMEM, "host allocation failed");
    h->device = device; h->k = k; h->map_count = map_count; h->n_cu = prop.multiProcessorCount;
    h->filt_hi = (uint32_t)map_count;
    hipError_t e = hipStreamCreateWithFlags(&h->own_stream, hipStreamNonBlocking);
    if (e != hipSuccess) { delete h; return fail(KQ_ERR_HIP, "hipStreamCreate: %s", hipGetErrorString(e)); }
    h->stream = h->base = h->own_stream;
    int rc = KQ_OK;
    do {
        if (hipMalloc((void**)&h->st, sizeof(DevState)) != hipSuccess || hipHostMalloc((void**)&h->st_host, sizeof(DevState)) != hipSuccess) {
            rc = fail(KQ_ERR_NOMEM, "state allocation failed"); break;
        }
        (void)hipMemsetAsync(h->st, 0, sizeof(DevState), h->stream);
        uint64_t slots = (uint64_t)((double)(capacity_hint ? capacity_hint : (1u << 20)) / 0.7);
        const uint64_t regions = round_regions((slots + REGION_SLOTS - 1) >> REGION_SHIFT, k);
        rc = alloc_main(h, regions, regions, &h->slots, &h->rstart); if (rc) break;
        h->n_regions = regions;
        uint64_t hc = 1u << 16;
        rc = alloc_hc(h, hc, &h->hc); if (rc) break;
        h->hc_cap = hc;
        if (hipStreamSynchronize(h->stream) != hipSuccess) { rc = fail(KQ_ERR_HIP, "table initialisation failed"); break; }
    } while (0);
    if (rc) { kq_destroy(h); return rc; }
    *out = h;
    return KQ_OK;
}

void kq_destroy(kq_handle* h) {
    if (!h) return;
    (void)hipSetDevice(h->device);
    if (h->stream) (void)hipStreamSynchronize(h->stream);
    if (h->slots) (void)hipFree(h->slots);
    if (h->rstart) (void)hipFree(h->rstart);
    if (h->hc) (void)hipFree(h->hc);
    if (h->st) (void)hipFree(h->st);
    if (h->st_host) (void)hipHostFree(h->st_host);
    if (h->scratch.p) (void)hipFree(h->scratch.p);
    if (h->stage.p) (void)hipFree(h->stage.p);
    if (h->work.part.p) (void)hipFree(h->work.part.p);
    scr_free(h->work.part2); scr_free(h->fork_work.part2);
    for (auto& e : h->hist_cache) (void)hipFree(e.m1_all);
    for (int w = 0; w < 2; ++w) { if (h->fork_stream[w]) { (void)hipStreamSynchronize(h->fork_stream[w]); (void)hipStreamDestroy(h->fork_stream[w]); } }
    if (h->fork_work.part.p) (void)hipFree(h->fork_work.part.p);
    for (auto e : h->ev_ring) if (e) (void)hipEventDestroy(e);
    if (h->ev_pass) (void)hipEventDestroy(h->ev_pass);
    for (int i = 0; i < kq_handle::IN_SLOTS; ++i) { if (h->in_buf[i].p) (void)hipFree(h->in_buf[i].p); if (h->in_consumed[i]) (void)hipEventDestroy(h->in_consumed[i]); }
    for (auto e : h->in_copied) (void)hipEventDestroy(e);
    for (int i = 0; i < kq_handle::IN_SLOTS; ++i) if (h->in_cmp[i].p) (void)hipFree(h->in_cmp[i].p);
    if (h->fx_units.p) (void)hipFree(h->fx_units.p);
    if (h->fx_out.p) (void)hipFree(h->fx_out.p);
    if (h->fx_res) (void)hipFree(h->fx_res);
    if (h->fx_res_host) (void)hipHostFree(h->fx_res_host);
    if (h->copy_stream) (void)hipStreamDestroy(h->copy_stream);
    arena_release(h);
    if (h->d_sets) (void)hipFree(h->d_sets);
    if (h->hot.p) (void)hipFree(h->hot.p);
    marks_reset(h);
    if (h->own_stream) (void)hipStreamDestroy(h->own_stream);
    delete h;
}

int kq_clear(kq_handle* h) {
    if (!h) return fail(KQ_ERR_INVALID, "null handle");
    HIPC(hipSetDevice(h->device));
    h->slots_dirty = true;
    clear_words(h, h->hc, sizeof(HcSlot) / 8, h->hc_cap);
    HIPC(hipMemsetAsync(h->st, 0, sizeof(DevState), h->stream));
    h->kmers_bound = 0;
    h->used_bound = 0;
    h->hc_check_at = 0;
    h->table_empty = true;
    h->n_pend = 0; h->arena_used = 0; h->pend_records = 0;
    h->fx_bad = 0;
    return KQ_OK;
}

int kq_set_stream(kq_handle* h, void* s) {
    if (!h) return fail(KQ_ERR_INVALID, "null handle");
    HIPC(hipStreamSynchronize(h->stream));
    h->stream = h->base = s ? (hipStream_t)s : h->own_stream;
    return KQ_OK;
}
int kq_set_option(kq_handle* h, int option, int64_t value) {
    if (!h) return fail(KQ_ERR_INVALID, "null handle");
    switch (option) {
        case KQ_OPT_TRUST_CAPACITY: h->trust_capacity = value != 0; return KQ_OK;
        case KQ_OPT_COUNT_PATH:
            if (value < 0 || value > 2) return fail(KQ_ERR_INVALID, "KQ_OPT_COUNT_PATH must be 0, 1 or 2");
            h->count_path = (int)value; return KQ_OK;
        case KQ_OPT_COUNT_MAP_RANGE: {
            const int64_t lo = value & 0xFFFF, hi = (value >> 16) & 0xFFFF;
            if (lo >= hi || hi > h->map_count) return fail(KQ_ERR_INVALID, "map range [%lld,%lld) outside [0,%d]", (long long)lo, (long long)hi, h->map_count);
            h->filt_lo = (uint32_t)lo; h->filt_hi = (uint32_t)hi; return KQ_OK;
        }
        case KQ_OPT_NARROW_MID:
            if (value < 2 || value > (1 << 14)) return fail(KQ_ERR_INVALID, "KQ_OPT_NARROW_MID must be in [2, 16384]");
            h->mid_rps = (uint32_t)value; return KQ_OK;
        case KQ_OPT_MERGE_PATH:
            if (value < 0 || value > 2) return fail(KQ_ERR_INVALID, "KQ_OPT_MERGE_PATH must be 0, 1 or 2");
            h->merge_path = (int)value; return KQ_OK;
        case KQ_OPT_LOOKUP_PATH:
            if (value < 0 || value > 2) return fail(KQ_ERR_INVALID, "KQ_OPT_LOOKUP_PATH must be 0, 1 or 2");
            h->lookup_path = (int)value; return KQ_OK;
        case KQ_OPT_PROFILE: h->profile = value != 0; if (!h->profile) marks_reset(h); return KQ_OK;
        case KQ_OPT_TEST_FAIL_PLAN: h->test_fail_plan = value != 0; return KQ_OK;
        case KQ_OPT_COUNT_MAP_PASSES: {
            if (value != 1 && value != 2 && value != 4 && value != 8) return fail(KQ_ERR_INVALID, "KQ_OPT_COUNT_MAP_PASSES must be 1, 2, 4 or 8");
            if ((h->map_count & (h->map_count - 1)) != 0 || value > h->map_count) return fail(KQ_ERR_INVALID, "KQ_OPT_COUNT_MAP_PASSES needs a power-of-two map count");
            HIPC(hipStreamSynchronize(h->stream));
            for (auto& e : h->hist_cache) (void)hipFree(e.m1_all);
            h->hist_cache.clear(); h->hist_cache_bytes = 0;
            h->map_passes = (int)value; return KQ_OK;
        }
        case KQ_OPT_KERNEL_SET:
            if (value < 0 || value > 7) return fail(KQ_ERR_INVALID, "KQ_OPT_KERNEL_SET is a mask of bits 1, 2, 4");
            h->kernel_set = (int)value; return KQ_OK;
        case KQ_OPT_OVERLAP:
            if (value < 0 || value > 2) return fail(KQ_ERR_INVALID, "KQ_OPT_OVERLAP must be 0, 1 or 2");
            h->overlap = (int)value; return KQ_OK;
        case KQ_OPT_PENDING_BYTES: {
            if (value < -1) return fail(KQ_ERR_INVALID, "KQ_OPT_PENDING_BYTES must be -1 (auto), 0 (off) or a byte count");
            int rc = flush_pending(h);
            if (rc) return rc;
            if (h->arena && value != h->pend_budget) { HIPC(hipStreamSynchronize(h->stream)); arena_release(h); }
            h->pend_budget = value; return KQ_OK;
        }
        case KQ_OPT_BUCKET_WINDOW:
            HIPC(hipSetDevice(h->device));
            return set_window(h, (uint32_t)(value & 0xFFFF), (uint32_t)((value >> 16) & 0xFFFF));
        case KQ_OPT_SHARD_WINDOW:
            HIPC(hipSetDevice(h->device));
            return set_window(h, (uint32_t)(value & 0xFFFF), (uint32_t)((value >> 16) & 0xFFFF), true);
        case KQ_OPT_SLICE_KMERS:
            if (value < 1) return fail(KQ_ERR_INVALID, "KQ_OPT_SLICE_KMERS must be positive");
            h->slice_kmers = (uint64_t)value; h->slice_user = true; return KQ_OK;
        default: return fail(KQ_ERR_INVALID, "unknown option %d", option);
    }
}
int kq_get_profile(kq_handle* h, char* buf, uint64_t cap) {
    if (!h || !buf || !cap) return fail(KQ_ERR_INVALID, "null argument");
    HIPC(hipSetDevice(h->device));
    HIPC(hipStreamSynchronize(h->stream));
    std::string out;
    for (size_t i = 1; i < h->marks.size(); ++i) {
        float ms = 0;
        HIPC(hipEventElapsedTime(&ms, h->marks[i - 1].second, h->marks[i].second));
        char tmp[96];
        snprintf(tmp, sizeof tmp, "%s%s=%.4f", out.empty() ? "" : ";", h->marks[i].first, ms);
        out += tmp;
    }
    if (out.size() + 1 > cap) return fail(KQ_ERR_CAPACITY, "profile buffer too small: need %zu", out.size() + 1);
    memcpy(buf, out.c_str(), out.size() + 1);
    return KQ_OK;
}
void* kq_get_stream(kq_handle* h) { return h ? (void*)h->stream : nullptr; }
int kq_sync(kq_handle* h) {
    if (!h) return fail(KQ_ERR_INVALID, "null handle");
    HIPC(hipSetDevice(h->device));
    HIPC(hipStreamSynchronize(h->stream));
    const int rc = check_errors(h);
    if (h->fx_bad) return fail(KQ_ERR_INVALID, "malformed %s text was submitted for counting and skipped (kq_clear resets this)", h->fx_bad == KQ_FASTX_FASTQ ? "FASTQ" : "FASTA");
    return rc;
}
int kq_flush(kq_handle* h) {
    if (!h) return fail(KQ_ERR_INVALID, "null handle");
    HIPC(hipSetDevice(h->device));
    return flush_pending(h);
}
int kq_get_info(kq_handle* h, kq_info* out) {
    if (!h || !out) return fail(KQ_ERR_INVALID, "null argument");
    HIPC(hipSetDevice(h->device));
    int rc = read_state(h);
    if (rc) return rc;
    out->kmers_counted = h->st_host->kmers_added;
    out->slots_used = h->st_host->slots_used;
    out->slots_total = h->n_slots();
    out->hc_used = h->st_host->hc_used;
    out->hc_total = h->hc_cap;
    out->table_bytes = h->n_slots() * sizeof(Slot) + h->hc_cap * sizeof(HcSlot);
    out->table_passes = h->table_passes;
    return KQ_OK;
}

struct PartPlan {
    PartCfg cfg;
    bool two_level;
    int fmt;
    uint64_t n_max, R;
    uint32_t g1;
    uint64_t m1_n, m2_n, sums_n, groups_n;
    uint64_t *recs1, *recs2;
    uint8_t *aux1, *aux2;
    unsigned long long *m1, *seg_off, *unit_base, *group_base, *sums, *total, *hot;
    uint32_t* m2;
    uint8_t* a1() const { return fmt == FMT_WIDE || fmt == FMT_NARROW ? aux1 : nullptr; }
    uint8_t* a2() const { return fmt == FMT_WIDE || fmt == FMT_NARROW ? aux2 : nullptr; }
};
static void plan_cfg(const kq_handle* h, PartCfg* cfg, bool allow_narrow = false) {
    cfg->n_regions = h->n_regions;
    uint32_t g = 1;
    while (((cfg->n_regions + (1ull << g) - 1) >> g) > 512 && g < 10) ++g;
    while (((cfg->n_regions + (1ull << g) - 1) >> g) >= (uint64_t)NB_MAX) ++g;
    cfg->g_shift = cfg->n_regions < (uint64_t)NB_MAX ? 0 : g;
    cfg->n_coarse = (uint32_t)((cfg->n_regions + (1ull << cfg->g_shift) - 1) >> cfg->g_shift);
    cfg->mode = 0; cfg->map_count = (uint32_t)h->map_count;
    cfg->map_mask = (h->map_count & (h->map_count - 1)) == 0 ? (uint32_t)h->map_count - 1 : 0;
    cfg->filt_lo = 0; cfg->filt_hi = (uint32_t)h->map_count;
    cfg->raw_out = 0;
    cfg->narrow = 0; cfg->sub_bits = 0; cfg->owner_sub = 0; cfg->n_rng = 0; cfg->win_lo = 0; cfg->win_hi = 1u << NARROW_CBITS;
    if (allow_narrow && (h->k <= (int)NARROW_MAX_K || h->k > PART_MAX_K) && cfg->n_regions >= (uint64_t)NB_MAX && cfg->n_regions % (1u << NARROW_CBITS) == 0) {
        const uint64_t rps = cfg->n_regions >> NARROW_CBITS;
        uint32_t sb = 0;
        if (rps >= h->mid_rps) {
            const uint64_t target_nb = std::max<uint64_t>(1, std::min<uint64_t>(256, h->mid_rps / 8));
            while ((rps >> sb) > target_nb && sb < SUB_BITS_MAX && rps % (2ull << sb) == 0) ++sb;
        }
        if ((rps >> sb) < (uint64_t)NB_MAX && (sb > 0 || rps < (uint64_t)NB_MAX)) { cfg->narrow = 1; cfg->sub_bits = sb; }
    }
    if (cfg->narrow) { cfg->n_coarse = 1u << NARROW_CBITS; if (cfg->g_shift == 0) cfg->g_shift = 1; }
}
static int plan_alloc(kq_handle* h, PartPlan* p, uint64_t n_max, uint64_t n_tiles, uint32_t p1_bins, bool allow_narrow = false,
                      uint64_t min_segs = 0 ) {
    if (h->test_fail_plan) { h->test_fail_plan = false; return fail(KQ_ERR_NOMEM, "partition scratch allocation failed (injected by KQ_OPT_TEST_FAIL_PLAN)"); }
    if (n_max >= (1ull << 32) - 16) return fail(KQ_ERR_INVALID, "a partition pass handles fewer than 2^32 records (got %llu): slice the input", (unsigned long long)n_max);
    plan_cfg(h, &p->cfg, allow_narrow);
    n_max = (n_max + 7) & ~7ull;
    p->two_level = p->cfg.g_shift != 0;
    p->fmt = !p->cfg.narrow ? FMT_PACK8 : h->k > PART_MAX_K ? FMT_TOP8 : FMT_NARROW;
    p->n_max = n_max; p->R = p->cfg.n_regions;
    p->g1 = (uint32_t)std::max<uint64_t>(1, std::min<uint64_t>(n_tiles, (uint64_t)h->n_cu * (p1_bins < 512 ? 18 : 12)));
    p->m1_n = (uint64_t)p1_bins * p->g1 * P1_F;
    const uint64_t nb_max = std::max<uint64_t>(std::max<uint64_t>(1ull << p->cfg.g_shift, p->cfg.n_coarse), p->cfg.narrow ? (p->cfg.n_regions >> NARROW_CBITS) >> p->cfg.sub_bits : 0);
    const uint64_t seg_max = std::max<uint64_t>(min_segs, p->cfg.narrow ? ((uint64_t)1 << NARROW_CBITS) << p->cfg.sub_bits : (uint64_t)NB_MAX);
    p->m2_n = (n_max / P2_UNIT + seg_max + 2) * nb_max;
    p->groups_n = std::max<uint64_t>(std::max<uint64_t>(p->R, (uint64_t)p->cfg.n_coarse << p->cfg.g_shift), min_segs) + 2;
    p->sums_n = std::max(p->m1_n, p->groups_n) / SCAN_CHUNK + 2;
    const uint64_t aux_words = (n_max + 7) / 8 + 1;
    const uint64_t rec_words = p->fmt == FMT_NARROW ? n_max / 2 + 2 : n_max;
    const bool split2 = (rec_words + aux_words) * 8 >= ((size_t)512 << 20);
    if (split2) { int rc2 = scr_ensure(h->work.part2, (size_t)(rec_words + aux_words) * 8, h->device); if (rc2) return rc2; }
    const size_t words = (size_t)((split2 ? 1 : 2) * (rec_words + aux_words) + p->m1_n + 2 * (seg_max + 2) + p->groups_n + p->sums_n + 4 + (p->R + 2) + (p->m2_n + 1) / 2);
    int rc = ensure_buf(h->work.part, words * 8);
    if (rc) return rc;
    p->recs1 = (uint64_t*)h->work.part.p;
    p->aux1 = (uint8_t*)(p->recs1 + rec_words);
    uint64_t* rest = (uint64_t*)(p->aux1 + aux_words * 8);
    if (split2) { p->recs2 = (uint64_t*)h->work.part2.p; p->aux2 = (uint8_t*)(p->recs2 + rec_words); }
    else { p->recs2 = rest; p->aux2 = (uint8_t*)(p->recs2 + rec_words); rest = (uint64_t*)(p->aux2 + aux_words * 8); }
    p->m1 = (unsigned long long*)rest;
    p->seg_off = p->m1 + p->m1_n;
    p->unit_base = p->seg_off + seg_max + 2;
    p->group_base = p->unit_base + seg_max + 2;
    p->sums = p->group_base + p->groups_n;
    p->total = p->sums + p->sums_n;
    p->hot = p->total + 4;
    p->m2 = (uint32_t*)(p->hot + p->R + 2);
    return KQ_OK;
}
static void scan_u64(kq_handle* h, unsigned long long* a, uint64_t n, unsigned long long* sums_scratch, unsigned long long* total) {
    if (n <= 2 * SCAN_CHUNK) {
        hipLaunchKernelGGL(k_exclusive_scan, dim3(1), dim3(1024), 0, h->stream, a, n, total);
        return;
    }
    const uint64_t chunks = (n + SCAN_CHUNK - 1) / SCAN_CHUNK;
    hipLaunchKernelGGL(k_scan_sums, dim3((unsigned)chunks), dim3(1024), 0, h->stream, a, n, sums_scratch);
    hipLaunchKernelGGL(k_exclusive_scan, dim3(1), dim3(1024), 0, h->stream, sums_scratch, chunks, total);
    hipLaunchKernelGGL(k_scan_apply, dim3((unsigned)chunks), dim3(1024), 0, h->stream, a, n, sums_scratch);
}
static void mark(kq_handle* h, const char* name) {
    if (!h->profile) return;
    hipEvent_t e;
    if (hipEventCreate(&e) != hipSuccess) return;
    (void)hipEventRecord(e, h->stream);
    h->marks.emplace_back(name, e);
}
static void marks_reset(kq_handle* h) {
    for (auto& m : h->marks) (void)hipEventDestroy(m.second);
    h->marks.clear();
}

static void run_p1(kq_handle* h, PartPlan* p, const PartCfg& cfg, const uint8_t* ab, uint64_t lead, uint64_t len, EmitRange er, uint64_t* out,
                   uint8_t* out_aux, int aux_fmt, const uint16_t* pinv = nullptr ) {
    const bool plain = cfg.mode == 0 && cfg.filt_lo == 0 && cfg.filt_hi == cfg.map_count;
    const bool owner_plain = cfg.mode == 1 && cfg.map_mask != 0 && cfg.filt_lo == 0 && cfg.filt_hi == cfg.map_count;
    const bool narrow_filt = cfg.mode == 0 && cfg.narrow && !plain && cfg.map_mask != 0 && h->k <= (int)NARROW_MAX_K;
    const bool narrow_win = plain && cfg.narrow && (h->k <= (int)NARROW_MAX_K || h->k > PART_MAX_K) && (cfg.win_lo != 0 || cfg.win_hi != (1u << NARROW_CBITS));
    const int binmode = owner_plain ? 3 : narrow_filt ? 4 : narrow_win ? 6 : !plain ? 0 : cfg.narrow ? 2 : 1;
    auto cached_hist = [&](const kq_handle::HistKey& key, size_t bytes, auto launch) -> kq_handle::HistEntry* {
        for (auto& e : h->hist_cache) if (e.key == key) return &e;
        if (h->hist_cache_bytes + bytes > ((size_t)4 << 30)) return nullptr;
        unsigned long long* buf = nullptr;
        if (hipMalloc((void**)&buf, bytes) != hipSuccess) { (void)hipGetLastError(); return nullptr; }
        launch(buf);
        h->hist_cache.push_back(kq_handle::HistEntry{key, buf, bytes});
        h->hist_cache_bytes += bytes;
        return &h->hist_cache.back();
    };
    bool have_hist = false;
    const size_t row = (size_t)p->g1 * sizeof(unsigned long long), block = row << NARROW_CBITS;
    if (narrow_filt && h->map_passes > 1 && P1_F == 1 && !h->hist_cache_off) {
        const uint32_t n = (uint32_t)h->map_passes, per = cfg.map_count / n, rr = cfg.filt_lo / per;
        if (cfg.filt_lo == rr * per && cfg.filt_hi == (rr + 1) * per) {
            const auto* ent = cached_hist({ab, pinv, lead, len, er.lo, er.hi, p->g1, n, h->k}, n * block, [&](unsigned long long* buf) {
                PartCfg all = cfg;
                all.n_rng = n; all.n_coarse = n << NARROW_CBITS;
                if (h->k == 21) hipLaunchKernelGGL((k_p1_hist<5, 21>), dim3(p->g1), dim3(TILE_THREADS), 0, h->stream, ab, lead, len, h->k, all, er, p->g1, buf, pinv);
                else hipLaunchKernelGGL((k_p1_hist<5, 0>), dim3(p->g1), dim3(TILE_THREADS), 0, h->stream, ab, lead, len, h->k, all, er, p->g1, buf, pinv);
            });
            if (ent) {
                (void)hipMemcpyAsync(p->m1, (const char*)ent->m1_all + rr * block, block, hipMemcpyDeviceToDevice, h->stream);
                have_hist = true;
            }
        }
    }
    if (narrow_win && h->map_passes > 1 && P1_F == 1 && !h->hist_cache_off) {
        const auto* ent = cached_hist({ab, pinv, lead, len, er.lo, er.hi, p->g1, 0xB0C4E7u, h->k}, block, [&](unsigned long long* buf) {
            PartCfg all = cfg;
            all.win_lo = 0; all.win_hi = 1u << NARROW_CBITS;
            if (h->k == 21) hipLaunchKernelGGL((k_p1_hist<2, 21>), dim3(p->g1), dim3(TILE_THREADS), 0, h->stream, ab, lead, len, h->k, all, er, p->g1, buf, pinv);
            else hipLaunchKernelGGL((k_p1_hist<2, 0>), dim3(p->g1), dim3(TILE_THREADS), 0, h->stream, ab, lead, len, h->k, all, er, p->g1, buf, pinv);
        });
        if (ent) {
            (void)hipMemcpyAsync(p->m1, ent->m1_all, block, hipMemcpyDeviceToDevice, h->stream);
            if (cfg.win_lo) (void)hipMemsetAsync(p->m1, 0, (size_t)cfg.win_lo * row, h->stream);
            if (cfg.win_hi < (1u << NARROW_CBITS)) (void)hipMemsetAsync((char*)p->m1 + (size_t)cfg.win_hi * row, 0, (size_t)((1u << NARROW_CBITS) - cfg.win_hi) * row, h->stream);
            have_hist = true;
        }
    }
#define KQ_P1H(B, K) hipLaunchKernelGGL((k_p1_hist<B, K>), dim3(p->g1 * P1_F), dim3(TILE_THREADS), 0, h->stream, ab, lead, len, h->k, cfg, er, p->g1, p->m1, pinv)
    if (have_hist) { }
    else if (binmode == 6) { if (h->k == 21) KQ_P1H(6, 21); else if (h->k == 31) KQ_P1H(6, 31); else KQ_P1H(6, 0); }
    else if (binmode == 2) { if (h->k == 21) KQ_P1H(2, 21); else KQ_P1H(2, 0); }
    else if (binmode == 1) { if (h->k == 31) KQ_P1H(1, 31); else KQ_P1H(1, 0); }
    else if (binmode == 3) { if (h->k == 21) KQ_P1H(3, 21); else KQ_P1H(3, 0); }
    else if (binmode == 4) { if (h->k == 21) KQ_P1H(4, 21); else KQ_P1H(4, 0); }
    else KQ_P1H(0, 0);
#undef KQ_P1H
    scan_u64(h, p->m1, (uint64_t)cfg.n_coarse * p->g1 * P1_F, p->sums, p->total);
    hipLaunchKernelGGL(k_p1_offsets, dim3((cfg.n_coarse + 256) / 256), dim3(256), 0, h->stream, p->m1, p->total, cfg, p->g1, p->seg_off);
    mark(h, "k_p1_hist+scan");
    const bool small = cfg.n_coarse < 512;
#define KQ_P1S(W, N, B, K) hipLaunchKernelGGL((k_p1_scatter<W, N, B, K>), dim3(p->g1), dim3(TILE_THREADS), 0, h->stream, ab, lead, len, h->k, cfg, er, p->m1, out, out_aux, aux_fmt, pinv)
#define KQ_P1T(B, K) do { if (h->kernel_set & 1) KQ_P1S(FMT_TOP8, 512, B, K); else \
        hipLaunchKernelGGL((k_p1_scatter_s<B, K, 1, true>), dim3(p->g1), dim3(TILE_THREADS), 0, h->stream, ab, lead, len, h->k, cfg, er, p->m1, (uint32_t*)out, out_aux, pinv); } while (0)
    if (cfg.narrow && h->k > PART_MAX_K) {
        if (narrow_win) { if (h->k == 31) KQ_P1T(6, 31); else KQ_P1T(6, 0); }
        else if (plain && h->k == 31) KQ_P1T(2, 31); else if (plain) KQ_P1T(2, 0); else KQ_P1T(0, 0);
    }
#define KQ_P1N(B, K, T) do { if (h->kernel_set & 1) KQ_P1S(FMT_NARROW, 512, B, K); else \
        hipLaunchKernelGGL((k_p1_scatter_s<B, K, T>), dim3(p->g1), dim3(TILE_THREADS * T), 0, h->stream, ab, lead, len, h->k, cfg, er, p->m1, (uint32_t*)out, out_aux, pinv); } while (0)
    else if (narrow_filt)  { if (h->k == 21) KQ_P1N(4, 21, 1); else KQ_P1N(4, 0, 1); }
    else if (narrow_win)   { if (h->k == 21) KQ_P1N(6, 21, 1); else KQ_P1N(6, 0, 1); }
    else if (cfg.narrow)   { if (plain && h->k == 21) KQ_P1N(2, 21, KQ_P1S_TPR); else if (plain) KQ_P1N(2, 0, KQ_P1S_TPR); else KQ_P1N(0, 0, 1); }
    else if (out_aux && plain && h->k == 31) { if (small) KQ_P1S(FMT_WIDE, 512, 1, 31); else KQ_P1S(FMT_WIDE, NB_MAX, 1, 31); }
    else if (out_aux) { if (small) KQ_P1S(FMT_WIDE, 512, 0, 0); else KQ_P1S(FMT_WIDE, NB_MAX, 0, 0); }
    else if (owner_plain && !out_aux && small) { if (h->k == 21) KQ_P1S(FMT_PACK8, 512, 3, 21); else KQ_P1S(FMT_PACK8, 512, 3, 0); }
    else if (plain)   { if (small) KQ_P1S(FMT_PACK8, 512, 1, 0); else KQ_P1S(FMT_PACK8, NB_MAX, 1, 0); }
    else              { if (small) KQ_P1S(FMT_PACK8, 512, 0, 0); else KQ_P1S(FMT_PACK8, NB_MAX, 0, 0); }
#undef KQ_P1S
#undef KQ_P1N
#undef KQ_P1T
    mark(h, "k_p1_scatter");
}
struct LevelIn { const uint64_t* recs; const uint8_t* aux; const unsigned long long *seg_lo, *seg_hi; uint32_t n_seg, spb; };
static LevelIn own_segments(const PartPlan& p, const uint64_t* recs, const uint8_t* aux, uint32_t n_seg) { return LevelIn{recs, aux, p.seg_off, p.seg_off + 1, n_seg, 1}; }
static void run_level(kq_handle* h, PartPlan* p, const LevelCfg& lv, const LevelIn& src, uint64_t* out, uint8_t* out_aux,
                      unsigned long long* gb = nullptr ) {
    if (!gb) gb = p->group_base;
    const uint64_t* in = src.recs; const uint8_t* in_aux = src.aux;
    const unsigned long long *seg_lo = src.seg_lo, *seg_hi = src.seg_hi;
    LevelCfg lvr = lv;
    lvr.rep_shift = 0;
    while (lvr.rep_shift < 6 && (((uint64_t)lv.nb + 1) << (lvr.rep_shift + 1)) <= 512) ++lvr.rep_shift;
    const LevelCfg& lv_ = lvr;
    const int fmt = lv.narrow == 2 ? FMT_TOP8 : lv.narrow ? FMT_NARROW : in_aux != nullptr ? FMT_WIDE : FMT_PACK8;
    const uint64_t groups = (uint64_t)(lv.n_seg / lv.spb) * lv.nb;
    hipLaunchKernelGGL(k_lv_units, dim3(1), dim3(1024), 0, h->stream, seg_lo, seg_hi, lv_, p->unit_base);
    const unsigned unit_grid = (unsigned)std::min<uint64_t>(p->n_max / P2_UNIT + lv.n_seg + 1, 1u << 30);
    if (fmt == FMT_TOP8) hipLaunchKernelGGL(k_lv_hist<FMT_TOP8>, dim3(unit_grid), dim3(MS_THREADS), 0, h->stream, in, in_aux, lv_, seg_lo, seg_hi, p->unit_base, p->m2);
    else if (fmt == FMT_NARROW) hipLaunchKernelGGL(k_lv_hist<FMT_NARROW>, dim3(unit_grid), dim3(MS_THREADS), 0, h->stream, in, in_aux, lv_, seg_lo, seg_hi, p->unit_base, p->m2);
    else if (fmt == FMT_WIDE) hipLaunchKernelGGL(k_lv_hist<FMT_WIDE>, dim3(unit_grid), dim3(MS_THREADS), 0, h->stream, in, in_aux, lv_, seg_lo, seg_hi, p->unit_base, p->m2);
    else hipLaunchKernelGGL(k_lv_hist<FMT_PACK8>, dim3(unit_grid), dim3(MS_THREADS), 0, h->stream, in, in_aux, lv_, seg_lo, seg_hi, p->unit_base, p->m2);
    if (p->n_max / P2_UNIT + 1 <= 8 * (uint64_t)(lv.n_seg / lv.spb))
        hipLaunchKernelGGL(k_lv_offsets_thread, dim3((unsigned)((groups + 255) / 256)), dim3(256), 0, h->stream, p->m2, lv_, p->unit_base, gb);
    else
        hipLaunchKernelGGL(k_lv_offsets, dim3((unsigned)((groups * 64 + 255) / 256)), dim3(256), 0, h->stream, p->m2, lv_, p->unit_base, gb);
    (void)hipMemsetAsync(gb + groups, 0, 8, h->stream);
    scan_u64(h, gb, groups + 1, p->sums, p->total + 1);
    mark(h, "k_lv_hist+offsets+scan");
    const bool small = lv.nb < 512;
#define KQ_LVS(W, N) hipLaunchKernelGGL((k_lv_scatter<W, N>), dim3(unit_grid), dim3(LV_THREADS), 0, h->stream, in, in_aux, lv_, \
                                        seg_lo, seg_hi, p->unit_base, p->m2, gb, out, out_aux)
    if (lv.top8)              { KQ_LVS(FMT_PACK8_TO_NARROW, 512); }
    else if (fmt == FMT_TOP8) { if (small) KQ_LVS(FMT_TOP8, 512); else KQ_LVS(FMT_TOP8, NB_MAX); }
#define KQ_LVN(T) hipLaunchKernelGGL((k_lv_scatter_s<T>), dim3(unit_grid), dim3(LV_THREADS), 0, h->stream, (const uint32_t*)in, in_aux, lv_, \
                                      seg_lo, seg_hi, p->unit_base, p->m2, gb, (uint32_t*)out, out_aux)
    else if (fmt == FMT_NARROW && small && lv.rstart && !(h->kernel_set & 4)) { KQ_LVN(true); }
    else if (fmt == FMT_NARROW && small && !lv.rstart && (h->kernel_set & 2)) { KQ_LVN(false); }
#undef KQ_LVN
    else if (fmt == FMT_NARROW && lv.rstart) { if (small) KQ_LVS(FMT_NARROW_TO_TIGHT, 512); else KQ_LVS(FMT_NARROW_TO_TIGHT, NB_MAX); }
    else if (fmt == FMT_NARROW) { if (small) KQ_LVS(FMT_NARROW, 512); else KQ_LVS(FMT_NARROW, NB_MAX); }
    else if (fmt == FMT_WIDE) { if (small) KQ_LVS(FMT_WIDE, 512); else KQ_LVS(FMT_WIDE, NB_MAX); }
    else                      { if (small) KQ_LVS(FMT_PACK8, 512); else KQ_LVS(FMT_PACK8, NB_MAX); }
#undef KQ_LVS
    mark(h, "k_lv_scatter");
}
static LevelCfg level_coarse_to_regions(const PartCfg& cfg) {
    LevelCfg lv; lv.n_regions = cfg.n_regions; lv.n_seg = cfg.n_coarse; lv.nb = 1u << cfg.g_shift; lv.seg_shift = cfg.g_shift; lv.out_shift = 0; lv.in_raw = 0; lv.k = 0; lv.narrow = 0; lv.top8 = 0;
    lv.nr_shift = lv.nr_rps = lv.nr_sub = lv.nr_inv = 0; lv.nr_div = 1;
    lv.nr_mid = 0; lv.nr_fshift = 24; lv.nr_fmask = 0xFFFFFFu; lv.nr_f24 = 0;
    lv.spb = 1;
    return lv;
}
static LevelCfg level_narrow(const PartCfg& cfg, uint32_t sub_bits = 0, bool middle = false, bool top8_records = false) {
    LevelCfg lv; lv.n_regions = cfg.n_regions;
    const uint32_t rps = (uint32_t)(cfg.n_regions >> NARROW_CBITS), subsz = rps >> sub_bits;
    lv.seg_shift = 0; lv.out_shift = 0; lv.in_raw = 0; lv.k = 0; lv.narrow = top8_records ? 2 : 1; lv.top8 = 0;
    lv.nr_rps = rps; lv.nr_sub = subsz;
    if (middle) { lv.n_seg = 1u << NARROW_CBITS; lv.nb = 1u << sub_bits; lv.nr_shift = 0; lv.nr_div = subsz; }
    else        { lv.n_seg = (1u << NARROW_CBITS) << sub_bits; lv.nb = subsz; lv.nr_shift = sub_bits; lv.nr_div = 1; }
    lv.nr_inv = lv.nr_div > 1 ? (uint32_t)(((1ull << 32) + lv.nr_div - 1) / lv.nr_div) : 0;
    lv.nr_mid = middle ? 1u : 0u; lv.nr_fshift = 24 - sub_bits; lv.nr_fmask = (1u << (24 - sub_bits)) - 1u;
    lv.nr_f24 = ((uint64_t)subsz << (24 - sub_bits)) <= (1ull << 32) && subsz < (1u << 24) ? 1u : 0u;
    lv.spb = 1;
    return lv;
}
static bool tight_ok(const kq_handle* h, const PartPlan& p) { return p.fmt == FMT_NARROW && p.R >= TIGHT_MIN_REGIONS && h->rstart != nullptr; }
static LevelCfg level_flat_to_coarse(const PartCfg& cfg) {
    LevelCfg lv; lv.n_regions = cfg.n_regions; lv.n_seg = 1; lv.nb = cfg.n_coarse; lv.seg_shift = 32; lv.out_shift = cfg.g_shift; lv.in_raw = 0; lv.k = 0; lv.narrow = 0; lv.top8 = 0;
    lv.nr_shift = lv.nr_rps = lv.nr_sub = lv.nr_inv = 0; lv.nr_div = 1;
    lv.nr_mid = 0; lv.nr_fshift = 24; lv.nr_fmask = 0xFFFFFFu; lv.nr_f24 = 0;
    lv.spb = 1;
    return lv;
}
__global__ void k_p3set(P3Set* sets, int i, P3Set v) { sets[i] = v; }

struct SetLayout { bool has_aux; size_t aux_off , base_off, total; };
static SetLayout set_bytes(uint64_t n_max, int fmt, uint64_t R) {
    const size_t rec = (fmt == FMT_NARROW || fmt == FMT_TIGHT) ? 4 : 8;
    SetLayout l;
    l.has_aux = fmt == FMT_NARROW || fmt == FMT_WIDE;
    l.aux_off = ((size_t)n_max * rec + 63) & ~(size_t)63;
    l.base_off = l.aux_off + (l.has_aux ? ((size_t)n_max + 63) & ~(size_t)63 : 0);
    l.total = (l.base_off + (size_t)(R + 2) * 8 + 255) & ~(size_t)255;
    return l;
}
struct Dest {
    int fmt, aux_fmt;
    bool tight = false;
    uint64_t* recs = nullptr; uint8_t* aux = nullptr; unsigned long long* base = nullptr; uint64_t n_max = 0;
    bool in_arena() const { return recs != nullptr; }
};
static int arena_take(kq_handle* h, uint64_t n_max, uint64_t R, Dest* d) {
    if (h->pend_budget == 0) return KQ_OK;
    const int fmt = d->fmt;
    const SetLayout lay = set_bytes(n_max, fmt, R);
    const size_t need = lay.total;
    bool was_full = false;
    if (h->n_pend && (h->n_pend >= P3_MAX_SETS || h->pend_fmt != fmt || h->arena_used + need > h->arena_bytes)) {
        was_full = h->pend_fmt == fmt && h->n_pend < P3_MAX_SETS;
        int rc = flush_pending(h);
        if (rc) return rc;
    }
    size_t want = h->arena_bytes;
    if (need > want) want = h->pend_budget > 0 ? (size_t)h->pend_budget : std::max<size_t>(4 * need, (size_t)64 << 20);
    else if (was_full && h->pend_budget < 0) want = 2 * h->arena_bytes;
    if (want > h->arena_bytes) {
        size_t free_b = 0, total_b = 0;
        if (hipMemGetInfo(&free_b, &total_b) != hipSuccess) return KQ_OK;
        size_t budget = want;
        const size_t avail = free_b + h->arena_bytes, reserve = std::max<size_t>(total_b / 8, (size_t)8 << 30);
        const size_t ceiling = avail > 2 * reserve ? avail - reserve : avail / 2;
        if (h->pend_budget < 0) budget = std::min<size_t>(want, std::min<size_t>(ceiling, std::max<size_t>(4 * need, 4 * (size_t)h->n_slots() * sizeof(Slot))));
        if (budget <= h->arena_bytes && need <= h->arena_bytes) budget = 0;
        if (budget && budget < need) return KQ_OK;
        if (budget) {
            if (h->arena) { HIPC(hipStreamSynchronize(h->stream)); HIPC(hipStreamSynchronize(h->base)); arena_release(h); }
            static const bool scramble_arena = !getenv("KQ_SCRAMBLE_ARENA") || atoi(getenv("KQ_SCRAMBLE_ARENA")) != 0;
            if (scramble_arena && budget >= ((size_t)1 << 30) && scr_try_vmm(h->arena_scr, budget, h->device)) h->arena = h->arena_scr.p;
            else
            if (hipMalloc(&h->arena, budget) != hipSuccess) { (void)hipGetLastError(); h->arena = nullptr; return KQ_OK; }
            h->arena_bytes = budget; h->arena_used = 0;
        }
    }
    uint8_t* set = (uint8_t*)h->arena + h->arena_used;
    d->recs = (uint64_t*)set;
    d->aux = lay.has_aux ? set + lay.aux_off : nullptr;
    d->base = (unsigned long long*)(set + lay.base_off);
    d->n_max = n_max;
    h->arena_used += need;
    return KQ_OK;
}
static int pend_add(kq_handle* h, const P3Set& set, int fmt, int aux_fmt) {
    if (h->n_pend && (h->n_pend >= P3_MAX_SETS || h->pend_fmt != fmt || h->pend_aux_fmt != aux_fmt)) {
        int rc = flush_pending(h);
        if (rc) return rc;
    }
    if (!h->d_sets) HIPC(hipMalloc((void**)&h->d_sets, sizeof(P3Set) * P3_MAX_SETS));
    hipLaunchKernelGGL(k_p3set, dim3(1), dim3(1), 0, h->stream, h->d_sets, h->n_pend, set);
    h->pend_fmt = fmt; h->pend_aux_fmt = aux_fmt;
    ++h->n_pend;
    h->pend_records += set.n_max;
    return KQ_OK;
}
static int flush_pending_base(kq_handle* h);
static int flush_pending(kq_handle* h) {
    if (!h->n_pend) return KQ_OK;
    hipStream_t work = h->stream;
    h->stream = h->base;
    int rc = join_forks(h);
    if (!rc) rc = flush_pending_base(h);
    if (!rc && h->fork_stream[0]) {
        hipEvent_t e; rc = ev_get(h, &e);
        if (!rc && hipEventRecord(e, h->base) != hipSuccess) rc = fail(KQ_ERR_HIP, "hipEventRecord failed");
        for (int w = 0; w < 2 && !rc; ++w) if (hipStreamWaitEvent(h->fork_stream[w], e, 0) != hipSuccess) rc = fail(KQ_ERR_HIP, "hipStreamWaitEvent failed");
    }
    h->stream = work;
    return rc;
}
static int flush_pending_base(kq_handle* h) {
    const uint64_t R = h->n_regions;
    int rc = ensure_buf(h->hot, (size_t)(R + 2) * 8);
    if (rc) return rc;
    if (h->kmers_bound / 255 + 1 > (1ull << 23)) {
        rc = read_state_raw(h); if (rc) return rc;
        const uint64_t need_hc = std::max<uint64_t>(HC_CAP_BIG, 8 * h->st_host->hc_used);
        if (need_hc > h->hc_cap) { rc = grow_hc(h, need_hc); if (rc) return rc; }
    }
    unsigned long long* hot = (unsigned long long*)h->hot.p;
    HIPC(hipMemsetAsync(hot, 0, 8, h->stream));
    const dim3 grid((unsigned)std::min<uint64_t>(h->n_alloc_regions(), 1u << 30)), grid_hot(h->n_cu), block(P3_THREADS);
    const int empty = h->slots_dirty ? 2 : h->table_empty ? 1 : 0;
    const int fmt = h->pend_fmt;
    const uint32_t rps = (fmt == FMT_NARROW || fmt == FMT_TIGHT || fmt == FMT_TOP8) ? (uint32_t)(R >> NARROW_CBITS) : 1u;
#define KQ_HOT(F) hipLaunchKernelGGL((k_count_regions<F, true>), grid_hot, block, 0, h->stream, h->view(), h->d_sets, (uint32_t)h->n_pend, h->pend_aux_fmt, empty, hot, rps)
#define KQ_P3(F) do { \
        hipLaunchKernelGGL((k_count_regions<F, false>), grid, block, 0, h->stream, h->view(), h->d_sets, (uint32_t)h->n_pend, h->pend_aux_fmt, empty, hot, rps); \
        KQ_HOT(F); } while (0)
#define KQ_Q4(KC, T) do { \
        hipLaunchKernelGGL((k_count_regions_q4<KC, T>), grid, dim3(Q4_THREADS), 0, h->stream, h->view(), h->d_sets, (uint32_t)h->n_pend, empty, hot, rps); \
        KQ_HOT(FMT_NARROW); } while (0)
    if (fmt == FMT_TIGHT)       { if (h->k == 21) KQ_Q4(21, true); else KQ_Q4(0, true); }
    else if (fmt == FMT_NARROW) { if (h->k == 21) KQ_Q4(21, false); else KQ_Q4(0, false); }
    else if (fmt == FMT_TOP8) KQ_P3(FMT_TOP8);
    else if (fmt == FMT_WIDE) KQ_P3(FMT_WIDE);
    else KQ_P3(FMT_PACK8);
#undef KQ_Q4
#undef KQ_P3
#undef KQ_HOT
    h->n_pend = 0; h->arena_used = 0; h->pend_records = 0;
    ++h->table_passes;
    h->slots_dirty = false;
    h->table_empty = false;
    mark(h, "k_count_regions");
    HIPC(hipGetLastError());
    return KQ_OK;
}

static bool part_table_ok(const kq_handle* h, bool narrow_possible) {
    if (h->n_regions <= (1ull << 20)) return true;
    if (!narrow_possible) return false;
    PartCfg c; plan_cfg(h, &c, true);
    return c.narrow != 0;
}
static int dest_take(kq_handle* h, const PartPlan& p, uint64_t n_max, Dest* d) {
    d->tight = tight_ok(h, p);
    if (d->tight) { d->fmt = FMT_TIGHT; d->aux_fmt = AUX_TIGHT; }
    return arena_take(h, n_max, p.R, d);
}
static P3Set sort_to_regions(kq_handle* h, PartPlan* p, const LevelIn& in, const Dest& d) {
    const bool arena = d.in_arena();
    uint64_t* fin = arena ? d.recs : p->recs2;
    uint8_t* fin_aux = arena ? d.aux : p->a2();
    unsigned long long* fin_base = arena ? d.base : p->group_base;
    if (p->fmt == FMT_NARROW || p->fmt == FMT_TOP8) {
        const uint32_t sb = p->cfg.sub_bits;
        const bool t8 = p->fmt == FMT_TOP8;
        const bool mid_to_2 = sb != 0 && in.recs == p->recs1;
        if (!arena && mid_to_2) { fin = p->recs1; fin_aux = p->a1(); }
        if (d.tight) fin_aux = nullptr;
        LevelCfg last = level_narrow(p->cfg, sb, false, t8);
        if (d.tight) last.rstart = h->rstart;
        if (sb == 0) {
            last.n_seg = in.n_seg; last.spb = in.spb;
            run_level(h, p, last, in, fin, fin_aux, fin_base);
        } else {
            LevelCfg mid = level_narrow(p->cfg, sb, true, t8);
            mid.n_seg = in.n_seg; mid.spb = in.spb;
            uint64_t* m = mid_to_2 ? p->recs2 : p->recs1;
            uint8_t* m_aux = mid_to_2 ? p->a2() : p->a1();
            run_level(h, p, mid, in, m, m_aux);
            (void)hipMemcpyAsync(p->seg_off, p->group_base, (size_t)(((1u << NARROW_CBITS) << sb) + 1) * 8, hipMemcpyDeviceToDevice, h->stream);
            run_level(h, p, last, own_segments(*p, m, m_aux, last.n_seg), fin, fin_aux, fin_base);
        }
    } else if (p->two_level) {
        run_level(h, p, level_coarse_to_regions(p->cfg), in, fin, fin_aux, fin_base);
    } else {
        return P3Set{in.recs, in.aux, in.seg_lo, p->n_max};
    }
    return P3Set{fin, fin_aux, fin_base, arena ? d.n_max : p->n_max};
}

static int submit(kq_handle* h, const P3Set& set, const Dest& d) {
    HIPC(hipGetLastError());
    int rc = pend_add(h, set, d.fmt, d.aux_fmt);
    if (rc) return rc;
    return d.in_arena() ? KQ_OK : flush_pending(h);
}

static int plan_sequence(kq_handle* h, PartPlan* p, uint64_t lead, uint64_t len) {
    PartCfg c0; plan_cfg(h, &c0, true);
    int rc = plan_alloc(h, p, len, n_tiles_of(lead, len), c0.n_coarse, true);
    if (rc) return rc;
    if (h->k > PART_MAX_K && p->fmt != FMT_TOP8) p->fmt = FMT_WIDE;
    return KQ_OK;
}

static int count_partitioned(kq_handle* h, const uint8_t* ab, uint64_t lead, uint64_t len, EmitRange er, const uint16_t* pinv = nullptr) {
    PartPlan p;
    int rc = plan_sequence(h, &p, lead, len);
    if (rc) return rc;
    p.cfg.filt_lo = h->filt_lo; p.cfg.filt_hi = h->filt_hi;
    if (h->windowed) { p.cfg.win_lo = h->win_lo; p.cfg.win_hi = h->win_hi; }
    const bool leveled = p.fmt == FMT_NARROW || p.fmt == FMT_TOP8 || p.two_level;
    Dest dst{p.fmt, AUX_IDX6};
    const bool filtered = p.cfg.filt_lo != 0 || p.cfg.filt_hi != p.cfg.map_count || h->windowed;
    if (leveled && !filtered) { rc = dest_take(h, p, p.n_max, &dst); if (rc) return rc; }
    marks_reset(h);
    mark(h, "start");
    run_p1(h, &p, p.cfg, ab, lead, len, er, p.recs1, p.a1(), AUX_IDX6, pinv);
    if (leveled && filtered) {
        unsigned long long n_recs = 0;
        HIPC(hipMemcpyAsync(&n_recs, p.total, sizeof n_recs, hipMemcpyDeviceToHost, h->stream));
        HIPC(hipStreamSynchronize(h->stream));
        rc = dest_take(h, p, std::min<uint64_t>(p.n_max, ((uint64_t)n_recs + 15) & ~7ull), &dst); if (rc) return rc;
    }
    return submit(h, sort_to_regions(h, &p, own_segments(p, p.recs1, p.a1(), p.cfg.n_coarse), dst), dst);
}
static int count_partitioned_records(kq_handle* h, const uint64_t* d_recs, const uint8_t* d_aux, int aux_fmt, uint64_t n, bool raw) {
    PartPlan p;
    int rc = plan_alloc(h, &p, n, 0, 1, !d_aux && !raw);
    if (rc) return rc;
    if (d_aux) p.fmt = FMT_WIDE;
    Dest dst{p.fmt, aux_fmt};
    LevelCfg first = level_flat_to_coarse(p.cfg);
    if (p.fmt == FMT_NARROW) {
        rc = dest_take(h, p, p.n_max, &dst); if (rc) return rc;
        first.top8 = 1;
    } else {
        first.in_raw = raw ? 1 : 0; first.k = (uint32_t)h->k;
    }
    hipLaunchKernelGGL(k_set2, dim3(1), dim3(1), 0, h->stream, p.seg_off, 0ull, (unsigned long long)n);
    run_level(h, &p, first, own_segments(p, d_recs, d_aux, 1), p.recs1, p.a1());
    LevelIn coarse{p.recs1, p.a1(), p.group_base, p.group_base + 1, p.cfg.n_coarse, 1};
    if (p.two_level) {
        HIPC(hipMemcpyAsync(p.seg_off, p.group_base, (size_t)(p.cfg.n_coarse + 1) * 8, hipMemcpyDeviceToDevice, h->stream));
        coarse = own_segments(p, p.recs1, p.a1(), p.cfg.n_coarse);
    }
    return submit(h, sort_to_regions(h, &p, coarse, dst), dst);
}

struct SliceView { const uint8_t* ab; const uint16_t* pinv; uint64_t lead, len; EmitRange er; };
static SliceView slice_view(const char* d_bases, const uint16_t* d_inv, uint64_t len, int k, uint64_t a, uint64_t b) {
    const uint64_t sub_off = a ? a - 1 : 0;
    SliceView v;
    v.len = std::min(len, b + k) - sub_off;
    v.er = EmitRange{a - sub_off, b - sub_off};
    v.pinv = nullptr;
    if (d_inv) { v.ab = (const uint8_t*)(reinterpret_cast<const uint32_t*>(d_bases) + sub_off / 16); v.pinv = d_inv + sub_off / 16; v.lead = sub_off % 16; }
    else aligned_view(d_bases + sub_off, &v.ab, &v.lead);
    return v;
}

static int count_seq_dev(kq_handle* h, const char* d_bases, const uint16_t* d_inv, uint64_t len) {
    if (!h || (!d_bases && len)) return fail(KQ_ERR_INVALID, "null argument");
    HIPC(hipSetDevice(h->device));
    if (len < (uint64_t)h->k) return KQ_OK;
    const uint64_t kmers = len - h->k + 1;
    uint64_t slice = h->slice_kmers;
    if (h->pend_budget != 0 && !h->slice_user && kmers > slice) {
        const uint64_t base_slice = slice;
        for (uint64_t cap : {1ull << 31, 1ull << 30}) {
            slice = std::min<uint64_t>(cap, std::max<uint64_t>(base_slice, h->n_slots() / 4));
            const uint64_t n_slices = (kmers + slice - 1) / slice;
            slice = (kmers + n_slices - 1) / n_slices;
            size_t free_b = 0, total_b = 0;
            if (cap == (1ull << 30) || slice <= (1ull << 30)) break;
            if (hipMemGetInfo(&free_b, &total_b) == hipSuccess && free_b + h->work.part.bytes >= (size_t)11 * slice + ((size_t)2 << 30)) break;
        }
    }
    if (h->pend_budget == 0 && !h->slice_user && kmers > slice && 2 * h->n_slots() > slice) {
        size_t free_b = 0, total_b = 0;
        if (hipMemGetInfo(&free_b, &total_b) == hipSuccess) {
            const uint64_t by_mem = (uint64_t)((free_b + h->work.part.bytes) / 24);
            slice = std::max(slice, std::min<uint64_t>(std::min<uint64_t>(2 * h->n_slots(), 1ull << 31), by_mem));
        }
    }
    struct ForkGuard {
        kq_handle* h; bool swapped = false;
        void leave() { if (swapped) { std::swap(h->work, h->fork_work); swapped = false; } h->stream = h->base; }
        ~ForkGuard() { leave(); (void)join_forks(h); }
    } guard{h};
    const bool forked = h->overlap && !h->profile && h->count_path != 1 && (kmers + slice - 1) / slice >= 2 && slice >= (1u << 20) &&
                        (h->overlap == 2 || (h->filt_lo == 0 && h->filt_hi == (uint32_t)h->map_count && !h->windowed));
    if (forked) {
        for (int w = 0; w < 2; ++w) if (!h->fork_stream[w]) HIPC(hipStreamCreateWithFlags(&h->fork_stream[w], hipStreamNonBlocking));
        hipEvent_t e_in; int erc = ev_get(h, &e_in); if (erc) return erc;
        HIPC(hipEventRecord(e_in, h->base));
        for (int w = 0; w < 2; ++w) HIPC(hipStreamWaitEvent(h->fork_stream[w], e_in, 0));
    }
    uint64_t slice_no = 0;
    for (uint64_t a = 0; a < kmers; a += slice, ++slice_no) {
        const uint64_t b = std::min(kmers, a + slice);
        int rc = reserve(h, b - a, b - a);
        if (rc) return rc;
        const SliceView v = slice_view(d_bases, d_inv, len, h->k, a, b);
        double pass_records = (double)(b - a);
        if (h->pend_budget != 0) {
            const double per_set = (double)set_bytes(b - a, FMT_PACK8, h->n_regions).total;
            const double room = h->arena ? (double)h->arena_bytes : 4.0 * (double)h->n_slots() * sizeof(Slot);
            pass_records = (double)h->pend_records + (double)(b - a) * std::max(1.0, std::min(8.0, room / per_set));
        }
        bool part = (b - a) >= (1u << 20) && part_table_ok(h, true) &&
                    (double)h->n_slots() * sizeof(Slot) <= 200.0 * pass_records;
        if (h->count_path == 1) part = false;
        if (h->count_path == 2) {
            if (!part_table_ok(h, true)) return fail(KQ_ERR_INVALID, "table too large for the partitioned path");
            part = true;
        }
        if (part) {
            if (forked) {
                const int w = (int)(slice_no & 1);
                if (w == 1) { std::swap(h->work, h->fork_work); guard.swapped = true; }
                h->stream = h->fork_stream[w];
                h->fork_busy[w] = true;
            }
            rc = count_partitioned(h, v.ab, v.lead, v.len, v.er, v.pinv);
            if (forked) h->fork_busy[slice_no & 1] = true;
            guard.leave();
            if (rc) return rc;
            continue;
        }
        if (forked) { rc = join_forks(h); if (rc) return rc; }
        PartCfg filt; plan_cfg(h, &filt);
        filt.filt_lo = h->filt_lo; filt.filt_hi = h->filt_hi;
        materialize(h);
        h->table_empty = false;
        hipLaunchKernelGGL(k_count_direct, dim3(grid_for(h, n_tiles_of(v.lead, v.len), 1, 32)), dim3(TILE_THREADS), 0, h->stream,
                           h->view(), v.ab, v.lead, v.len, h->k, v.er, filt, v.pinv);
        HIPC(hipGetLastError());
    }
    return KQ_OK;
}
int kq_count_batch_dev(kq_handle* h, const char* d_bases, uint64_t len) { return count_seq_dev(h, d_bases, nullptr, len); }
int kq_count_packed_dev(kq_handle* h, const uint32_t* d_codes, const uint16_t* d_inv, uint64_t n_bases) {
    if (!d_inv && n_bases) return fail(KQ_ERR_INVALID, "null argument");
    return count_seq_dev(h, (const char*)d_codes, d_inv, n_bases);
}
void kq_pack_bases(const char* bases, uint64_t len, uint32_t* codes, uint16_t* inv) {
    static const struct Lut { uint8_t v[256]; Lut() { for (int i = 0; i < 256; ++i) v[i] = 4; v['A'] = v['a'] = 0; v['C'] = v['c'] = 1; v['G'] = v['g'] = 2; v['T'] = v['t'] = 3; } } lut;
    const uint64_t full = len / 16;
    const uint8_t* b = (const uint8_t*)bases;
    for (uint64_t u = 0; u < full; ++u, b += 16) {
        uint32_t c = 0, m = 0;
        for (int i = 0; i < 16; ++i) { const uint32_t x = lut.v[b[i]]; c |= (x & 3u) << (2 * i); m |= (x >> 2) << i; }
        codes[u] = c; inv[u] = (uint16_t)m;
    }
    if (len % 16) {
        uint32_t c = 0, m = 0xFFFFu;
        for (uint64_t i = 0; i < len % 16; ++i) { const uint32_t x = lut.v[b[i]]; c |= (x & 3u) << (2 * i); if (!(x >> 2)) m &= ~(1u << i); }
        codes[full] = c; inv[full] = (uint16_t)m;
    }
}
int kq_count_batch(kq_handle* h, const char* bases, uint64_t len) {
    if (!h || (!bases && len)) return fail(KQ_ERR_INVALID, "null argument");
    HIPC(hipSetDevice(h->device));
    void* d = nullptr;
    int rc = stage_in(h, bases, len, &d);
    if (rc) return rc;
    rc = kq_count_batch_dev(h, (const char*)d, len);
    if (rc) return rc;
    HIPC(hipStreamSynchronize(h->stream));
    return KQ_OK;
}

void* kq_host_alloc(uint64_t bytes) {
    const size_t n = ((size_t)(bytes ? bytes : 1) + 4095) & ~(size_t)4095;
    void* p = aligned_alloc(4096, n);
// ... 780 lines not shown
```

Before: 51.31 billion.

## Split pending record arena into per-band extents so passes flush per region band

Adds an extent allocator and a banded pending mode. The pending record arena is split into per-band extents sized from the per-coarse-segment counts, and the tight last level writes each band through a displacement. Flushes then run the count pass one region band at a time, and only bands that were touched get cleared. The aim is to avoid full-table flushes and clears when the arena fills, and to keep more sets pending. In exchange it adds a host sync to read the segment bounds, much more bookkeeping, and per-band kernel launches, which may add overhead.

```diff
diff --git a/include/kreeq_amd.h b/include/kreeq_amd.h
--- a/include/kreeq_amd.h
+++ b/include/kreeq_amd.h
@@ -60,10 +60,12 @@
 void* kq_get_stream(kq_handle* h);
 enum { KQ_OPT_TRUST_CAPACITY = 1, KQ_OPT_COUNT_PATH = 2, KQ_OPT_SLICE_KMERS = 3, KQ_OPT_COUNT_MAP_RANGE = 4, KQ_OPT_PROFILE = 5,
        KQ_OPT_LOOKUP_PATH = 6, KQ_OPT_MERGE_PATH = 7, KQ_OPT_NARROW_MID = 8, KQ_OPT_PENDING_BYTES = 9, KQ_OPT_BUCKET_WINDOW = 10, KQ_OPT_OVERLAP = 11, KQ_OPT_COUNT_MAP_PASSES = 12, KQ_OPT_KERNEL_SET = 13, KQ_OPT_SHARD_WINDOW = 14,
+       KQ_OPT_PASS_BANDS = 15,
        KQ_OPT_TEST_FAIL_PLAN = 100  };
 int  kq_set_option(kq_handle* h, int option, int64_t value);
 int  kq_get_profile(kq_handle* h, char* buf, uint64_t cap);
 int  kq_sync(kq_handle* h);
+int kq_get_pass_regions(kq_handle* h, uint64_t* out);
 int  kq_flush(kq_handle* h);
 int  kq_get_info(kq_handle* h, kq_info* out);
 const char* kq_last_error(void);
diff --git a/kreeq_amd/build.py b/kreeq_amd/build.py
--- a/kreeq_amd/build.py
+++ b/kreeq_amd/build.py
@@ -9,7 +9,7 @@
 HOSTLIB = os.path.join(PKG, "lib", "libkreeq_host.so")
 
 HIP_SOURCES = [os.path.join(PKG, "csrc", "kreeq_amd.hip")]
-HIP_DEPS = HIP_SOURCES + [os.path.join(PKG, "csrc", f) for f in ("kq_device.h", "kq_partition.h", "kq_kernels.h", "kq_fastx.h")] + [os.path.join(ROOT, "include", "kreeq_amd.h")]
+HIP_DEPS = HIP_SOURCES + [os.path.join(PKG, "csrc", f) for f in ("kq_device.h", "kq_partition.h", "kq_kernels.h", "kq_fastx.h", "kq_arena.h")] + [os.path.join(ROOT, "include", "kreeq_amd.h")]
 HOST_DIR = os.path.join(PKG, "host")
 
 
diff --git a/kreeq_amd/capi.py b/kreeq_amd/capi.py
--- a/kreeq_amd/capi.py
+++ b/kreeq_amd/capi.py
@@ -8,7 +8,7 @@
 ENTRY_DTYPE = np.dtype([("key", "<u8"), ("fw", "<u4", 4), ("bw", "<u4", 4), ("cov", "<u4"), ("hc", "<u4")])
 DBGBASE_DTYPE = np.dtype([("fw", "<u4"), ("bw", "<u4"), ("cov", "<u4"), ("isFw", "u1"), ("pad", "u1", 3)])
 
-SYMBOLS = ["kq_create", "kq_destroy", "kq_clear", "kq_set_option", "kq_get_profile", "kq_set_stream", "kq_get_stream", "kq_sync", "kq_flush", "kq_get_info", "kq_last_error",
+SYMBOLS = ["kq_create", "kq_destroy", "kq_clear", "kq_set_option", "kq_get_profile", "kq_set_stream", "kq_get_stream", "kq_sync", "kq_flush", "kq_get_info", "kq_get_pass_regions", "kq_last_error",
            "kq_abi_version", "kq_device_available", "kq_device_memory", "kq_count_batch", "kq_count_batch_dev", "kq_host_alloc", "kq_host_free", "kq_count_batch_async", "kq_host_wait", "kq_pack_bases", "kq_count_packed_dev", "kq_count_packed_async",
            "kq_pack_bases_dev", "kq_parse_fastx_dev", "kq_count_fastx_dev", "kq_count_fastx_async", "kq_emit_records",
            "kq_emit_partitioned_dev", "kq_emit_packed_dev", "kq_insert_packed_dev", "kq_emit_sharded_dev", "kq_insert_sharded_dev", "kq_emit_sharded8_dev", "kq_insert_sharded8_dev", "kq_insert_records", "kq_insert_records_dev", "kq_summary", "kq_histogram",
@@ -178,7 +178,7 @@
         _check(load().kq_flush(self._h))
 
     def set_option(self, option, value):
-        opt = {"trust_capacity": 1, "count_path": 2, "slice_kmers": 3, "count_map_range": 4, "profile": 5, "lookup_path": 6, "merge_path": 7, "narrow_mid": 8, "pending_bytes": 9, "bucket_window": 10, "overlap": 11, "count_map_passes": 12, "kernel_set": 13, "shard_window": 14, "test_fail_plan": 100}[option]
+        opt = {"trust_capacity": 1, "count_path": 2, "slice_kmers": 3, "count_map_range": 4, "profile": 5, "lookup_path": 6, "merge_path": 7, "narrow_mid": 8, "pending_bytes": 9, "bucket_window": 10, "overlap": 11, "count_map_passes": 12, "kernel_set": 13, "shard_window": 14, "pass_bands": 15, "test_fail_plan": 100}[option]
         if option == "count_map_range":
             value = int(value[0]) | (int(value[1]) << 16)
         if option in ("count_path", "lookup_path", "merge_path"):
@@ -197,6 +197,11 @@
         i = Info()
         _check(load().kq_get_info(self._h, C.byref(i)))
         return {f: getattr(i, f) for f, _ in Info._fields_}
+
+    def pass_regions(self):
+        n = C.c_uint64(0)
+        _check(load().kq_get_pass_regions(self._h, C.byref(n)))
+        return n.value
 
     def count_batch(self, bases: bytes):
         buf = np.frombuffer(bases, dtype=np.uint8)
diff --git a/kreeq_amd/csrc/kq_arena.h b/kreeq_amd/csrc/kq_arena.h
--- /dev/null
+++ b/kreeq_amd/csrc/kq_arena.h
@@ -0,0 +1,66 @@
+#pragma once
+#include <cstddef>
+#include <cstdint>
+#include <vector>
+
+namespace kq {
+
+struct ExtentArena {
+    static constexpr size_t ALIGN = 256, NPOS = ~(size_t)0;
+    struct Range { size_t off, len; };
+    std::vector<Range> free_list;
+    size_t cap = 0, used = 0;
+    size_t cls = 0;
+
+    static size_t up(size_t v) { return (v + ALIGN - 1) & ~(ALIGN - 1); }
+    static size_t down(size_t v) { return v & ~(ALIGN - 1); }
+
+    void reset(size_t capacity) {
+        cap = down(capacity); used = 0; cls = 0;
+        free_list.clear();
+        if (cap) free_list.push_back(Range{0, cap});
+    }
+    bool empty() const { return used == 0; }
+
+    size_t alloc(size_t bytes) {
+        const size_t n = up(bytes ? bytes : 1);
+        for (size_t i = 0; i < free_list.size(); ++i) {
+            Range& r = free_list[i];
+            if (r.len < n) continue;
+            const size_t off = r.off;
+            if (r.len == n) free_list.erase(free_list.begin() + (std::ptrdiff_t)i);
+            else { r.off += n; r.len -= n; }
+            used += n;
+            return off;
+        }
+        return NPOS;
+    }
+    bool free(size_t off, size_t bytes) {
+        if (!bytes) return true;
+        if (off % ALIGN || bytes % ALIGN || off > cap || bytes > cap - off) return false;
+        size_t i = 0;
+        while (i < free_list.size() && free_list[i].off < off) ++i;
+        if (i > 0 && free_list[i - 1].off + free_list[i - 1].len > off) return false;
+        if (i < free_list.size() && off + bytes > free_list[i].off) return false;
+        const bool left = i > 0 && free_list[i - 1].off + free_list[i - 1].len == off;
+        const bool right = i < free_list.size() && off + bytes == free_list[i].off;
+        if (left && right) { free_list[i - 1].len += bytes + free_list[i].len; free_list.erase(free_list.begin() + (std::ptrdiff_t)i); }
+        else if (left) free_list[i - 1].len += bytes;
+        else if (right) { free_list[i].off = off; free_list[i].len += bytes; }
+        else free_list.insert(free_list.begin() + (std::ptrdiff_t)i, Range{off, bytes});
+        used -= bytes;
+        if (used == 0) cls = 0;
+        return true;
+    }
+    size_t largest_free() const { size_t m = 0; for (const Range& r : free_list) if (r.len > m) m = r.len; return m; }
+
+    size_t piece_bytes(size_t bytes) {
+        size_t step = ALIGN;
+        while (step * 128 <= bytes) step *= 2;
+        const size_t mine = (bytes + bytes / 64 + ALIGN + step - 1) / step * step;
+        if (mine > cls) cls = mine;
+        return bytes >= cls / 2 ? cls : mine;
+    }
+};
+
+}
diff --git a/kreeq_amd/csrc/kq_kernels.h b/kreeq_amd/csrc/kq_kernels.h
--- a/kreeq_amd/csrc/kq_kernels.h
+++ b/kreeq_amd/csrc/kq_kernels.h
@@ -433,6 +433,8 @@
         const uint64_t hi = lo + P2_UNIT < seg_hi[b_in] ? lo + P2_UNIT : seg_hi[b_in];
         for (uint32_t i = threadIdx.x; i < nb; i += LV_THREADS)
             s.gbase[i] = (uint32_t)(group_base[(uint64_t)b * nb + i] + m2[u * nb + i]);
+        uint64_t* outb = out;
+        if (TIGHT && lv.disp) outb = reinterpret_cast<uint64_t*>(reinterpret_cast<uint32_t*>(out) + lv.disp[(b >> lv.nr_shift) >> lv.disp_shift]);
         if (TIGHT) {
             const uint32_t first = (b >> lv.nr_shift) * lv.nr_rps + (b & ((1u << lv.nr_shift) - 1u)) * lv.nr_sub;
             for (uint32_t i = threadIdx.x; i < nb; i += LV_THREADS) s_rst[i] = lv.rstart[first + i];
@@ -475,7 +477,7 @@
                 nxt[j] = NARROW ? (uint64_t)recs32[i] : recs[i];
                 nxt_aux[j] = HAS_AUX ? recs_aux[i] : 0;
             }
-            block_multisplit<MS_FMT, LV_THREADS, LV_ITEMS>(s, rec, aux, bin, nb, out, out_aux, [&] {
+            block_multisplit<MS_FMT, LV_THREADS, LV_ITEMS>(s, rec, aux, bin, nb, outb, out_aux, [&] {
 #pragma unroll
                 for (int j = 0; j < LV_ITEMS; ++j) { landed(nxt[j]); if (HAS_AUX) landed(nxt_aux[j]); }
             }, NBC <= 512 ? lv.rep_shift : 0u);
@@ -508,6 +510,8 @@
         const uint64_t lo = seg_off[b_in] + (u - unit_base[b_in]) * P2_UNIT;
         const uint64_t hi = lo + P2_UNIT < seg_hi[b_in] ? lo + P2_UNIT : seg_hi[b_in];
         uint32_t gabs = own_bin ? (uint32_t)(group_base[(uint64_t)b * nb + my_bin] + m2[u * nb + my_bin]) : 0u;
+        uint32_t* outb = out;
+        if (TIGHT && lv.disp) outb = out + lv.disp[(b >> lv.nr_shift) >> lv.disp_shift];
         if (TIGHT) {
             const uint32_t first = (b >> lv.nr_shift) * lv.nr_rps + (b & ((1u << lv.nr_shift) - 1u)) * lv.nr_sub;
             if ((uint32_t)tid < nb) s_rst[tid] = lv.rstart[first + tid];
@@ -574,7 +578,7 @@
 #pragma unroll
             for (int it = 0; it < LV_ITEMS; ++it) {
                 if ((uint32_t)(tid + it * LV_THREADS) < total) {
-                    out[cg[it]] = (uint32_t)cv[it];
+                    outb[cg[it]] = (uint32_t)cv[it];
                     if (!TIGHT) out_aux[cg[it]] = (uint8_t)(cv[it] >> 48);
                 }
             }
diff --git a/kreeq_amd/csrc/kq_partition.h b/kreeq_amd/csrc/kq_partition.h
--- a/kreeq_amd/csrc/kq_partition.h
+++ b/kreeq_amd/csrc/kq_partition.h
@@ -44,6 +44,8 @@
     uint32_t spb;
     uint32_t rep_shift;
     const uint32_t* rstart = nullptr;
+    const long long* disp = nullptr;
+    uint32_t disp_shift = 0;
 };
 __device__ __forceinline__ uint32_t level_bin(const LevelCfg& lv, uint32_t b, uint64_t region) {
     return (uint32_t)(region >> lv.out_shift) - (lv.seg_shift >= 32 ? 0u : (b << (lv.seg_shift - lv.out_shift)));
diff --git a/kreeq_amd/csrc/kreeq_amd.hip b/kreeq_amd/csrc/kreeq_amd.hip
--- a/kreeq_amd/csrc/kreeq_amd.hip
+++ b/kreeq_amd/csrc/kreeq_amd.hip
@@ -17,6 +17,7 @@
 #include "../../include/kreeq_amd.h"
 #include "kq_device.h"
 #include "kq_partition.h"
+#include "kq_arena.h"
 
 using namespace kq;
 
@@ -103,6 +104,13 @@
 struct DevBuf { void* p = nullptr; size_t bytes = 0; };
 struct ScratchSet { DevBuf part; Scrambled part2; };
 
+constexpr int BANDS_MAX = 64;
+static int default_pass_bands() {
+    const char* e = getenv("KQ_PASS_BANDS");
+    if (!e) return 8;
+    const int v = atoi(e);
+    return (v == 0 || (v >= 2 && v <= BANDS_MAX && (v & (v - 1)) == 0)) ? v : 8;
+}
 struct kq_handle;
 static void arena_release(kq_handle* h);
 struct kq_handle {
@@ -159,6 +167,28 @@
     uint64_t pend_records = 0;
     int64_t pend_budget = -1;
     uint64_t table_passes = 0;
+    uint64_t pass_regions = 0;
+    int pass_bands = default_pass_bands();
+    bool ext_mode = false;
+    ExtentArena ext;
+    struct Piece { size_t off = 0, len = 0; };
+    struct PendSet {
+        bool own_extents = false;
+        size_t off = ExtentArena::NPOS, total = 0;
+        const unsigned long long* base = nullptr; uint64_t n_max = 0;
+        Piece piece[BANDS_MAX], base_ext;
+        uint8_t live[BANDS_MAX] = {}, freed[BANDS_MAX] = {};
+        long long disp[BANDS_MAX] = {};
+        int n_live = 0;
+    };
+    std::vector<PendSet> psets;
+    PendSet staged; bool staged_valid = false;
+    P3Set pend_host[P3_MAX_SETS];
+    P3Set* d_band_sets = nullptr;
+    int band_n[BANDS_MAX] = {}, band_next = 0;
+    uint8_t band_state[BANDS_MAX] = {};
+    static constexpr size_t PIN_SETS = 264, PIN_WORDS = PIN_SETS + (size_t)P3_MAX_SETS * (BANDS_MAX + 1);
+    unsigned long long* pin = nullptr;
     static constexpr int IN_SLOTS = 3, IN_TICKETS = 512;
     hipStream_t copy_stream = nullptr;
     DevBuf in_buf[IN_SLOTS];
@@ -190,6 +220,7 @@
 
 static void marks_reset(kq_handle* h);
 static int flush_pending(kq_handle* h);
+static void ext_reset(kq_handle* h);
 
 static int ev_get(kq_handle* h, hipEvent_t* out) {
     hipEvent_t& e = h->ev_ring[h->ev_next++ % kq_handle::EV_RING];
@@ -237,6 +268,15 @@
 }
 static void clear_main(kq_handle* h, Slot* p, uint64_t n_slots) { (void)hipMemsetAsync(p, 0, (size_t)n_slots * sizeof(Slot), h->stream); }
 static void materialize(kq_handle* h) {
+    if (h->ext_mode) {
+        const uint64_t band_slots = (h->n_regions / (uint64_t)h->pass_bands) << REGION_SHIFT;
+        for (int b = 0; b < h->pass_bands; ++b) {
+            if (h->band_state[b] == 2) clear_main(h, h->slots + (uint64_t)b * band_slots, band_slots);
+            h->band_state[b] = 0;
+        }
+        h->slots_dirty = false;
+        return;
+    }
     if (!h->slots_dirty) return;
     clear_main(h, h->slots, h->n_slots());
     h->slots_dirty = false;
@@ -518,6 +558,8 @@
     if (h->copy_stream) (void)hipStreamDestroy(h->copy_stream);
     arena_release(h);
     if (h->d_sets) (void)hipFree(h->d_sets);
+    if (h->d_band_sets) (void)hipFree(h->d_band_sets);
+    if (h->pin) (void)hipHostFree(h->pin);
     if (h->hot.p) (void)hipFree(h->hot.p);
     marks_reset(h);
     if (h->own_stream) (void)hipStreamDestroy(h->own_stream);
@@ -535,6 +577,7 @@
     h->hc_check_at = 0;
     h->table_empty = true;
     h->n_pend = 0; h->arena_used = 0; h->pend_records = 0;
+    ext_reset(h);
     h->fx_bad = 0;
     return KQ_OK;
 }
@@ -589,6 +632,12 @@
             if (h->arena && value != h->pend_budget) { HIPC(hipStreamSynchronize(h->stream)); arena_release(h); }
             h->pend_budget = value; return KQ_OK;
         }
+        case KQ_OPT_PASS_BANDS: {
+            if (value != 0 && (value < 2 || value > BANDS_MAX || (value & (value - 1)) != 0)) return fail(KQ_ERR_INVALID, "KQ_OPT_PASS_BANDS must be 0 (off) or a power of two in [2, %d]", BANDS_MAX);
+            int rc = flush_pending(h);
+            if (rc) return rc;
+            h->pass_bands = (int)value; return KQ_OK;
+        }
         case KQ_OPT_BUCKET_WINDOW:
             HIPC(hipSetDevice(h->device));
             return set_window(h, (uint32_t)(value & 0xFFFF), (uint32_t)((value >> 16) & 0xFFFF));
@@ -643,6 +692,12 @@
     out->hc_total = h->hc_cap;
     out->table_bytes = h->n_slots() * sizeof(Slot) + h->hc_cap * sizeof(HcSlot);
     out->table_passes = h->table_passes;
+    return KQ_OK;
+}
+
+int kq_get_pass_regions(kq_handle* h, uint64_t* out) {
+    if (!h || !out) return fail(KQ_ERR_INVALID, "null argument");
+    *out = h->pass_regions;
     return KQ_OK;
 }
 
@@ -913,96 +968,67 @@
     int fmt, aux_fmt;
     bool tight = false;
     uint64_t* recs = nullptr; uint8_t* aux = nullptr; unsigned long long* base = nullptr; uint64_t n_max = 0;
+    const long long* disp = nullptr; uint32_t disp_shift = 0;
+    bool need_bounds = false;
     bool in_arena() const { return recs != nullptr; }
 };
-static int arena_take(kq_handle* h, uint64_t n_max, uint64_t R, Dest* d) {
-    if (h->pend_budget == 0) return KQ_OK;
-    const int fmt = d->fmt;
-    const SetLayout lay = set_bytes(n_max, fmt, R);
-    const size_t need = lay.total;
-    bool was_full = false;
-    if (h->n_pend && (h->n_pend >= P3_MAX_SETS || h->pend_fmt != fmt || h->arena_used + need > h->arena_bytes)) {
-        was_full = h->pend_fmt == fmt && h->n_pend < P3_MAX_SETS;
-        int rc = flush_pending(h);
-        if (rc) return rc;
-    }
-    size_t want = h->arena_bytes;
-    if (need > want) want = h->pend_budget > 0 ? (size_t)h->pend_budget : std::max<size_t>(4 * need, (size_t)64 << 20);
-    else if (was_full && h->pend_budget < 0) want = 2 * h->arena_bytes;
-    if (want > h->arena_bytes) {
-        size_t free_b = 0, total_b = 0;
-        if (hipMemGetInfo(&free_b, &total_b) != hipSuccess) return KQ_OK;
-        size_t budget = want;
-        const size_t avail = free_b + h->arena_bytes, reserve = std::max<size_t>(total_b / 8, (size_t)8 << 30);
-        const size_t ceiling = avail > 2 * reserve ? avail - reserve : avail / 2;
-        if (h->pend_budget < 0) budget = std::min<size_t>(want, std::min<size_t>(ceiling, std::max<size_t>(4 * need, 4 * (size_t)h->n_slots() * sizeof(Slot))));
-        if (budget <= h->arena_bytes && need <= h->arena_bytes) budget = 0;
-        if (budget && budget < need) return KQ_OK;
-        if (budget) {
-            if (h->arena) { HIPC(hipStreamSynchronize(h->stream)); HIPC(hipStreamSynchronize(h->base)); arena_release(h); }
-            static const bool scramble_arena = !getenv("KQ_SCRAMBLE_ARENA") || atoi(getenv("KQ_SCRAMBLE_ARENA")) != 0;
-            if (scramble_arena && budget >= ((size_t)1 << 30) && scr_try_vmm(h->arena_scr, budget, h->device)) h->arena = h->arena_scr.p;
-            else
-            if (hipMalloc(&h->arena, budget) != hipSuccess) { (void)hipGetLastError(); h->arena = nullptr; return KQ_OK; }
-            h->arena_bytes = budget; h->arena_used = 0;
-        }
-    }
-    uint8_t* set = (uint8_t*)h->arena + h->arena_used;
-    d->recs = (uint64_t*)set;
-    d->aux = lay.has_aux ? set + lay.aux_off : nullptr;
-    d->base = (unsigned long long*)(set + lay.base_off);
-    d->n_max = n_max;
-    h->arena_used += need;
-    return KQ_OK;
-}
-static int pend_add(kq_handle* h, const P3Set& set, int fmt, int aux_fmt) {
-    if (h->n_pend && (h->n_pend >= P3_MAX_SETS || h->pend_fmt != fmt || h->pend_aux_fmt != aux_fmt)) {
-        int rc = flush_pending(h);
-        if (rc) return rc;
-    }
-    if (!h->d_sets) HIPC(hipMalloc((void**)&h->d_sets, sizeof(P3Set) * P3_MAX_SETS));
-    hipLaunchKernelGGL(k_p3set, dim3(1), dim3(1), 0, h->stream, h->d_sets, h->n_pend, set);
-    h->pend_fmt = fmt; h->pend_aux_fmt = aux_fmt;
-    ++h->n_pend;
-    h->pend_records += set.n_max;
-    return KQ_OK;
-}
-static int flush_pending_base(kq_handle* h);
-static int flush_pending(kq_handle* h) {
-    if (!h->n_pend) return KQ_OK;
-    hipStream_t work = h->stream;
-    h->stream = h->base;
-    int rc = join_forks(h);
-    if (!rc) rc = flush_pending_base(h);
-    if (!rc && h->fork_stream[0]) {
-        hipEvent_t e; rc = ev_get(h, &e);
-        if (!rc && hipEventRecord(e, h->base) != hipSuccess) rc = fail(KQ_ERR_HIP, "hipEventRecord failed");
-        for (int w = 0; w < 2 && !rc; ++w) if (hipStreamWaitEvent(h->fork_stream[w], e, 0) != hipSuccess) rc = fail(KQ_ERR_HIP, "hipStreamWaitEvent failed");
-    }
-    h->stream = work;
-    return rc;
-}
-static int flush_pending_base(kq_handle* h) {
-    const uint64_t R = h->n_regions;
-    int rc = ensure_buf(h->hot, (size_t)(R + 2) * 8);
+__global__ void k_band_bounds(const P3Set* __restrict__ sets, uint32_t n_sets, uint32_t nb, uint64_t regions_per_band, unsigned long long* __restrict__ out) {
+    const uint32_t i = blockIdx.x * blockDim.x + threadIdx.x;
+    if (i < n_sets * (nb + 1)) out[i] = sets[i / (nb + 1)].base[(uint64_t)(i % (nb + 1)) * regions_per_band];
+}
+__global__ void k_band_fill(P3Set* __restrict__ band_sets, const P3Set* __restrict__ sets, uint32_t n_sets, uint32_t nb) {
+    const uint32_t i = blockIdx.x * blockDim.x + threadIdx.x;
+    if (i < n_sets * nb) band_sets[(i / n_sets) * P3_MAX_SETS + i % n_sets] = sets[i % n_sets];
+}
+struct BandPieces { const unsigned long long* base; uint64_t n_max; uint32_t nb; const uint64_t* recs[BANDS_MAX]; uint8_t idx[BANDS_MAX]; };
+__global__ void k_band_add(P3Set* __restrict__ band_sets, BandPieces a) {
+    const uint32_t b = threadIdx.x;
+    if (b < a.nb) band_sets[b * P3_MAX_SETS + a.idx[b]] = P3Set{a.recs[b], nullptr, a.base, a.n_max};
+}
+struct Disp64 { long long v[BANDS_MAX]; };
+__global__ void k_band_disp(long long* __restrict__ out, Disp64 a, uint32_t nb) { if (threadIdx.x < nb) out[threadIdx.x] = a.v[threadIdx.x]; }
+
+static bool bands_ok(const kq_handle* h, int fmt) { return h->pass_bands > 0 && fmt == FMT_TIGHT && !h->windowed && h->pend_budget != 0; }
+static uint64_t band_regions(const kq_handle* h) { return h->n_regions / (uint64_t)h->pass_bands; }
+static int band_scratch(kq_handle* h) {
+    if (!h->d_band_sets) HIPC(hipMalloc((void**)&h->d_band_sets, sizeof(P3Set) * P3_MAX_SETS * BANDS_MAX));
+    if (!h->pin) HIPC(hipHostMalloc((void**)&h->pin, sizeof(unsigned long long) * kq_handle::PIN_WORDS));
+    return KQ_OK;
+}
+static void ext_reset(kq_handle* h) {
+    h->ext_mode = false; h->psets.clear(); h->staged_valid = false;
+    for (int b = 0; b < BANDS_MAX; ++b) { h->band_n[b] = 0; h->band_state[b] = 0; }
+    h->ext.reset(0);
+}
+static void ext_leave(kq_handle* h) {
+    ext_reset(h);
+    h->n_pend = 0; h->arena_used = 0; h->pend_records = 0;
+    h->slots_dirty = false; h->table_empty = false;
+}
+static int pass_prepare(kq_handle* h) {
+    int rc = ensure_buf(h->hot, (size_t)(h->n_regions + 2) * 8);
     if (rc) return rc;
     if (h->kmers_bound / 255 + 1 > (1ull << 23)) {
         rc = read_state_raw(h); if (rc) return rc;
         const uint64_t need_hc = std::max<uint64_t>(HC_CAP_BIG, 8 * h->st_host->hc_used);
         if (need_hc > h->hc_cap) { rc = grow_hc(h, need_hc); if (rc) return rc; }
     }
+    return KQ_OK;
+}
+static int pass_launch(kq_handle* h, uint64_t reg_lo, uint64_t reg_hi, const P3Set* sets, int n_sets, int empty) {
     unsigned long long* hot = (unsigned long long*)h->hot.p;
     HIPC(hipMemsetAsync(hot, 0, 8, h->stream));
-    const dim3 grid((unsigned)std::min<uint64_t>(h->n_alloc_regions(), 1u << 30)), grid_hot(h->n_cu), block(P3_THREADS);
-    const int empty = h->slots_dirty ? 2 : h->table_empty ? 1 : 0;
+    TableView view = h->view();
+    view.reg_lo = reg_lo; view.reg_hi = reg_hi;
+    const dim3 grid((unsigned)std::min<uint64_t>(reg_hi - reg_lo, 1u << 30)), grid_hot(h->n_cu), block(P3_THREADS);
     const int fmt = h->pend_fmt;
-    const uint32_t rps = (fmt == FMT_NARROW || fmt == FMT_TIGHT || fmt == FMT_TOP8) ? (uint32_t)(R >> NARROW_CBITS) : 1u;
-#define KQ_HOT(F) hipLaunchKernelGGL((k_count_regions<F, true>), grid_hot, block, 0, h->stream, h->view(), h->d_sets, (uint32_t)h->n_pend, h->pend_aux_fmt, empty, hot, rps)
+    const uint32_t rps = (fmt == FMT_NARROW || fmt == FMT_TIGHT || fmt == FMT_TOP8) ? (uint32_t)(h->n_regions >> NARROW_CBITS) : 1u;
+#define KQ_HOT(F) hipLaunchKernelGGL((k_count_regions<F, true>), grid_hot, block, 0, h->stream, view, sets, (uint32_t)n_sets, h->pend_aux_fmt, empty, hot, rps)
 #define KQ_P3(F) do { \
-        hipLaunchKernelGGL((k_count_regions<F, false>), grid, block, 0, h->stream, h->view(), h->d_sets, (uint32_t)h->n_pend, h->pend_aux_fmt, empty, hot, rps); \
+        hipLaunchKernelGGL((k_count_regions<F, false>), grid, block, 0, h->stream, view, sets, (uint32_t)n_sets, h->pend_aux_fmt, empty, hot, rps); \
         KQ_HOT(F); } while (0)
 #define KQ_Q4(KC, T) do { \
-        hipLaunchKernelGGL((k_count_regions_q4<KC, T>), grid, dim3(Q4_THREADS), 0, h->stream, h->view(), h->d_sets, (uint32_t)h->n_pend, empty, hot, rps); \
+        hipLaunchKernelGGL((k_count_regions_q4<KC, T>), grid, dim3(Q4_THREADS), 0, h->stream, view, sets, (uint32_t)n_sets, empty, hot, rps); \
         KQ_HOT(FMT_NARROW); } while (0)
     if (fmt == FMT_TIGHT)       { if (h->k == 21) KQ_Q4(21, true); else KQ_Q4(0, true); }
     else if (fmt == FMT_NARROW) { if (h->k == 21) KQ_Q4(21, false); else KQ_Q4(0, false); }
@@ -1012,12 +1038,288 @@
 #undef KQ_Q4
 #undef KQ_P3
 #undef KQ_HOT
-    h->n_pend = 0; h->arena_used = 0; h->pend_records = 0;
+    h->pass_regions += reg_hi - reg_lo;
+    HIPC(hipGetLastError());
+    return KQ_OK;
+}
+static int on_base(kq_handle* h, int (*fn)(kq_handle*, int), int arg) {
+    hipStream_t work = h->stream;
+    h->stream = h->base;
+    int rc = join_forks(h);
+    if (!rc) rc = fn(h, arg);
+    if (!rc && h->fork_stream[0]) {
+        hipEvent_t e; rc = ev_get(h, &e);
+        if (!rc && hipEventRecord(e, h->base) != hipSuccess) rc = fail(KQ_ERR_HIP, "hipEventRecord failed");
+        for (int w = 0; w < 2 && !rc; ++w) if (hipStreamWaitEvent(h->fork_stream[w], e, 0) != hipSuccess) rc = fail(KQ_ERR_HIP, "hipStreamWaitEvent failed");
+    }
+    h->stream = work;
+    return rc;
+}
+static int ext_enter(kq_handle* h) {
+    int rc = band_scratch(h);
+    if (rc) return rc;
+    const uint32_t nb = (uint32_t)h->pass_bands, n = (uint32_t)h->n_pend;
+    hipLaunchKernelGGL(k_band_bounds, dim3((n * (nb + 1) + 255) / 256), dim3(256), 0, h->stream, h->d_sets, n, nb, band_regions(h), h->pin + kq_handle::PIN_SETS);
+    hipLaunchKernelGGL(k_band_fill, dim3((n * nb + 255) / 256), dim3(256), 0, h->stream, h->d_band_sets, h->d_sets, n, nb);
+    HIPC(hipGetLastError());
+    HIPC(hipStreamSynchronize(h->stream));
+    ext_reset(h);
+    h->ext.reset(h->arena_bytes);
+    if (h->arena_used) (void)h->ext.alloc(h->arena_used);
+    for (uint32_t i = 0; i < n; ++i) {
+        const P3Set& st = h->pend_host[i];
+        kq_handle::PendSet ps;
+        ps.base = st.base; ps.n_max = st.n_max; ps.n_live = (int)nb;
+        const uint8_t* lo = (const uint8_t*)st.recs;
+        const bool mine = h->arena && lo >= (const uint8_t*)h->arena && lo < (const uint8_t*)h->arena + h->arena_used;
+        if (mine) { ps.off = (size_t)(lo - (const uint8_t*)h->arena); ps.total = set_bytes(st.n_max, FMT_TIGHT, h->n_regions).total; }
+        const unsigned long long* bd = h->pin + kq_handle::PIN_SETS + (size_t)i * (nb + 1);
+        for (uint32_t b = 0; b < nb; ++b) {
+            kq_handle::Piece pc{0, 0};
+            if (mine) {
+                const size_t a = ExtentArena::up(ps.off + 4 * (size_t)bd[b]), e = ExtentArena::down(ps.off + 4 * (size_t)bd[b + 1]);
+                if (e > a) pc = kq_handle::Piece{a, e - a};
+            }
+            ps.piece[b] = pc; ps.live[b] = 1;
+        }
+        h->psets.push_back(ps);
+    }
+    const int empty = h->slots_dirty ? 2 : h->table_empty ? 1 : 0;
+    for (uint32_t b = 0; b < nb; ++b) { h->band_n[b] = (int)n; h->band_state[b] = (uint8_t)empty; }
+    h->ext_mode = true;
+    return KQ_OK;
+}
+static void band_release(kq_handle* h, int b) {
+    for (size_t i = 0; i < h->psets.size();) {
+        kq_handle::PendSet& ps = h->psets[i];
+        if (ps.live[b]) {
+            ps.live[b] = 0; --ps.n_live;
+            if (ps.piece[b].len && (ps.own_extents || ps.n_live > 0)) { (void)h->ext.free(ps.piece[b].off, ps.piece[b].len); ps.freed[b] = 1; }
+        }
+        if (ps.n_live > 0) { ++i; continue; }
+        if (ps.own_extents) { if (ps.base_ext.len) (void)h->ext.free(ps.base_ext.off, ps.base_ext.len); }
+        else if (ps.off != ExtentArena::NPOS) {
+            std::vector<kq_handle::Piece> gone;
+            for (int q = 0; q < h->pass_bands; ++q) if (ps.freed[q]) gone.push_back(ps.piece[q]);
+            std::sort(gone.begin(), gone.end(), [](const kq_handle::Piece& x, const kq_handle::Piece& y) { return x.off < y.off; });
+            size_t at = ps.off;
+            for (const auto& g : gone) { if (g.off > at) (void)h->ext.free(at, g.off - at); at = g.off + g.len; }
+            if (ps.off + ps.total > at) (void)h->ext.free(at, ps.off + ps.total - at);
+        }
+        h->psets.erase(h->psets.begin() + (std::ptrdiff_t)i);
+        --h->n_pend;
+    }
+    h->band_n[b] = 0; h->band_state[b] = 0;
+}
+static int band_pass_base(kq_handle* h, int want) {
+    int rc = pass_prepare(h);
+    if (rc) return rc;
+    int b = want;
+    for (int i = 0; b < 0 && i < h->pass_bands; ++i) { const int c = (h->band_next + i) % h->pass_bands; if (h->band_n[c]) b = c; }
+    if (b < 0) return KQ_OK;
+    h->band_next = (b + 1) % h->pass_bands;
+    const uint64_t rb = band_regions(h);
+    rc = pass_launch(h, (uint64_t)b * rb, (uint64_t)(b + 1) * rb, h->d_band_sets + (size_t)b * P3_MAX_SETS, h->band_n[b], h->band_state[b]);
+    if (rc) return rc;
+    band_release(h, b);
     ++h->table_passes;
-    h->slots_dirty = false;
-    h->table_empty = false;
     mark(h, "k_count_regions");
-    HIPC(hipGetLastError());
+    if (h->psets.empty()) ext_leave(h);
+    return KQ_OK;
+}
+static int band_pass_entered(kq_handle* h, int want) {
+    if (!h->ext_mode) { int rc = ext_enter(h); if (rc) return rc; }
+    return band_pass_base(h, want);
+}
+static int band_pass(kq_handle* h, int want = -1) { return on_base(h, band_pass_entered, want); }
+
+static size_t arena_budget(kq_handle* h, size_t need, size_t want) {
+    size_t free_b = 0, total_b = 0;
+    if (hipMemGetInfo(&free_b, &total_b) != hipSuccess) return ~(size_t)0;
+    size_t budget = want;
+    const size_t avail = free_b + h->arena_bytes, reserve = std::max<size_t>(total_b / 8, (size_t)8 << 30);
+    const size_t ceiling = avail > 2 * reserve ? avail - reserve : avail / 2;
+    if (h->pend_budget < 0) budget = std::min<size_t>(want, std::min<size_t>(ceiling, std::max<size_t>(4 * need, 4 * (size_t)h->n_slots() * sizeof(Slot))));
+    if (budget <= h->arena_bytes && need <= h->arena_bytes) budget = 0;
+    return budget;
+}
+static int arena_take(kq_handle* h, uint64_t n_max, uint64_t R, Dest* d, const unsigned long long* bounds = nullptr, bool can_bound = false);
+static int ext_take(kq_handle* h, uint64_t n_max, uint64_t R, Dest* d, const unsigned long long* bounds) {
+    const int nb = h->pass_bands;
+    const SetLayout lay = set_bytes(n_max, FMT_TIGHT, R);
+    if (h->staged_valid) {
+        kq_handle::PendSet& ps = h->staged;
+        if (ps.own_extents) { for (int b = 0; b < nb; ++b) if (ps.piece[b].len) (void)h->ext.free(ps.piece[b].off, ps.piece[b].len); if (ps.base_ext.len) (void)h->ext.free(ps.base_ext.off, ps.base_ext.len); }
+        else if (ps.off != ExtentArena::NPOS) (void)h->ext.free(ps.off, ps.total);
+        h->staged_valid = false;
+    }
+    for (int attempt = 0; attempt <= nb + 1; ++attempt) {
+        if (h->ext_mode) for (int b = 0; b < nb; ++b) if (h->band_n[b] >= P3_MAX_SETS) { int rc = band_pass(h, b); if (rc) return rc; break; }
+        if (attempt) { int rc = band_pass(h); if (rc) return rc; }
+        else if (!h->ext_mode) { int rc = band_pass(h); if (rc) return rc; }
+        if (!h->ext_mode) return arena_take(h, n_max, R, d);
+        kq_handle::PendSet ps;
+        ps.n_max = n_max; ps.n_live = nb;
+        bool ok = true;
+        if (bounds) {
+            ps.own_extents = true;
+            for (int b = 0; b < nb && ok; ++b) {
+                const size_t bytes = 4 * (size_t)(bounds[b + 1] - bounds[b]), shift = (4 * (size_t)bounds[b]) & (ExtentArena::ALIGN - 1);
+                if (!bytes) continue;
+                size_t len = h->ext.piece_bytes(bytes), off = h->ext.alloc(len);
+                if (off == ExtentArena::NPOS) { len = ExtentArena::up(bytes + shift); off = h->ext.alloc(len); }
+                ok = off != ExtentArena::NPOS;
+                if (ok) ps.piece[b] = kq_handle::Piece{off, len};
+            }
+            const size_t base_bytes = ExtentArena::up((size_t)(R + 2) * 8 + (size_t)nb * 8);
+            const size_t bo = ok ? h->ext.alloc(base_bytes) : ExtentArena::NPOS;
+            ok = bo != ExtentArena::NPOS;
+            if (ok) ps.base_ext = kq_handle::Piece{bo, base_bytes};
+            if (!ok) { for (int b = 0; b < nb; ++b) if (ps.piece[b].len) (void)h->ext.free(ps.piece[b].off, ps.piece[b].len); if (ps.base_ext.len) (void)h->ext.free(ps.base_ext.off, ps.base_ext.len); }
+        } else {
+            const size_t off = h->ext.alloc(lay.total);
+            ok = off != ExtentArena::NPOS;
+            if (ok) { ps.off = off; ps.total = ExtentArena::up(lay.total); }
+        }
+        if (!ok) continue;
+        uint8_t* arena = (uint8_t*)h->arena;
+        if (bounds) {
+            Disp64 dv;
+            for (int b = 0; b < BANDS_MAX; ++b) dv.v[b] = 0;
+            for (int b = 0; b < nb; ++b) {
+                ps.live[b] = 1;
+                ps.disp[b] = dv.v[b] = (long long)((ps.piece[b].off + ((4 * (size_t)bounds[b]) & (ExtentArena::ALIGN - 1))) / 4) - (long long)bounds[b];
+            }
+            d->recs = (uint64_t*)arena; d->aux = nullptr;
+            d->base = (unsigned long long*)(arena + ps.base_ext.off);
+            d->disp = (long long*)(arena + ps.base_ext.off + (size_t)(R + 2) * 8);
+            hipLaunchKernelGGL(k_band_disp, dim3(1), dim3(BANDS_MAX), 0, h->stream, (long long*)d->disp, dv, (uint32_t)nb);
+            uint32_t sh = 0; while ((256u >> sh) > (uint32_t)nb) ++sh;
+            d->disp_shift = sh;
+        } else {
+            for (int b = 0; b < nb; ++b) { ps.live[b] = 1; ps.piece[b] = kq_handle::Piece{0, 0}; }
+            uint8_t* set = arena + ps.off;
+            d->recs = (uint64_t*)set; d->aux = nullptr;
+            d->base = (unsigned long long*)(set + lay.base_off);
+        }
+        ps.base = d->base;
+        d->n_max = n_max;
+        h->staged = ps; h->staged_valid = true;
+        return KQ_OK;
+    }
+    return fail(KQ_ERR_NOMEM, "pending arena: no room for a set after applying every band");
+}
+static int arena_take(kq_handle* h, uint64_t n_max, uint64_t R, Dest* d, const unsigned long long* bounds, bool can_bound) {
+    d->need_bounds = false;
+    if (h->pend_budget == 0) return KQ_OK;
+    const int fmt = d->fmt;
+    const SetLayout lay = set_bytes(n_max, fmt, R);
+    const size_t need = lay.total;
+    if (h->ext_mode) {
+        if (fmt == h->pend_fmt && bands_ok(h, fmt)) {
+            if (can_bound && !bounds) { d->need_bounds = true; return KQ_OK; }
+            return ext_take(h, n_max, R, d, bounds);
+        }
+        int rc = flush_pending(h);
+        if (rc) return rc;
+    }
+    bool was_full = false;
+    if (h->n_pend && (h->n_pend >= P3_MAX_SETS || h->pend_fmt != fmt || h->arena_used + need > h->arena_bytes)) {
+        was_full = h->pend_fmt == fmt && h->n_pend < P3_MAX_SETS;
+        if (was_full && bands_ok(h, fmt) && need <= h->arena_bytes && (h->pend_budget > 0 || arena_budget(h, need, 2 * h->arena_bytes) == 0)) {
+            if (can_bound && !bounds) { d->need_bounds = true; return KQ_OK; }
+            return ext_take(h, n_max, R, d, bounds);
+        }
+        int rc = flush_pending(h);
+        if (rc) return rc;
+    }
+    size_t want = h->arena_bytes;
+    if (need > want) want = h->pend_budget > 0 ? (size_t)h->pend_budget : std::max<size_t>(4 * need, (size_t)64 << 20);
+    else if (was_full && h->pend_budget < 0) want = 2 * h->arena_bytes;
+    if (want > h->arena_bytes) {
+        const size_t budget = arena_budget(h, need, want);
+        if (budget == ~(size_t)0) return KQ_OK;
+        if (budget && budget < need) return KQ_OK;
+        if (budget) {
+            if (h->arena) { HIPC(hipStreamSynchronize(h->stream)); HIPC(hipStreamSynchronize(h->base)); arena_release(h); }
+            static const bool scramble_arena = !getenv("KQ_SCRAMBLE_ARENA") || atoi(getenv("KQ_SCRAMBLE_ARENA")) != 0;
+            if (scramble_arena && budget >= ((size_t)1 << 30) && scr_try_vmm(h->arena_scr, budget, h->device)) h->arena = h->arena_scr.p;
+            else
+            if (hipMalloc(&h->arena, budget) != hipSuccess) { (void)hipGetLastError(); h->arena = nullptr; return KQ_OK; }
+            h->arena_bytes = budget; h->arena_used = 0;
+        }
+    }
+    uint8_t* set = (uint8_t*)h->arena + h->arena_used;
+    d->recs = (uint64_t*)set;
+    d->aux = lay.has_aux ? set + lay.aux_off : nullptr;
+    d->base = (unsigned long long*)(set + lay.base_off);
+    d->n_max = n_max;
+    h->arena_used += need;
+    return KQ_OK;
+}
+static int pend_add(kq_handle* h, const P3Set& set, int fmt, int aux_fmt) {
+    if (h->ext_mode) {
+        bool room = fmt == h->pend_fmt && aux_fmt == h->pend_aux_fmt;
+        for (int b = 0; b < h->pass_bands && room; ++b) room = h->band_n[b] < P3_MAX_SETS;
+        if (!room && h->staged_valid && h->staged.base == set.base) return fail(KQ_ERR_INVALID, "pending set of band extents does not match the pending format");
+        if (!room) { int rc = flush_pending(h); if (rc) return rc; }
+    }
+    if (h->ext_mode) {
+        kq_handle::PendSet ps;
+        const bool staged = h->staged_valid && h->staged.base == set.base;
+        if (staged) ps = h->staged;
+        else { ps.base = set.base; ps.n_max = set.n_max; ps.n_live = h->pass_bands; for (int b = 0; b < h->pass_bands; ++b) ps.live[b] = 1; }
+        if (staged) h->staged_valid = false;
+        BandPieces a;
+        a.base = set.base; a.n_max = set.n_max; a.nb = (uint32_t)h->pass_bands;
+        for (int b = 0; b < h->pass_bands; ++b) {
+            a.recs[b] = ps.own_extents ? (const uint64_t*)((const uint32_t*)h->arena + ps.disp[b]) : set.recs;
+            a.idx[b] = (uint8_t)h->band_n[b]++;
+        }
+        hipLaunchKernelGGL(k_band_add, dim3(1), dim3(BANDS_MAX), 0, h->stream, h->d_band_sets, a);
+        h->psets.push_back(ps);
+        ++h->n_pend;
+        h->pend_records += set.n_max;
+        return KQ_OK;
+    }
+    if (h->n_pend && (h->n_pend >= P3_MAX_SETS || h->pend_fmt != fmt || h->pend_aux_fmt != aux_fmt)) {
+        int rc = flush_pending(h);
+        if (rc) return rc;
+    }
+    if (!h->d_sets) HIPC(hipMalloc((void**)&h->d_sets, sizeof(P3Set) * P3_MAX_SETS));
+    hipLaunchKernelGGL(k_p3set, dim3(1), dim3(1), 0, h->stream, h->d_sets, h->n_pend, set);
+    h->pend_host[h->n_pend] = set;
+    h->pend_fmt = fmt; h->pend_aux_fmt = aux_fmt;
+    ++h->n_pend;
+    h->pend_records += set.n_max;
+    return KQ_OK;
+}
+static int flush_pending_base(kq_handle* h, int);
+static int flush_pending(kq_handle* h) {
+    if (!h->n_pend) return KQ_OK;
+    return on_base(h, flush_pending_base, 0);
+}
+static int flush_pending_base(kq_handle* h, int) {
+    int rc = pass_prepare(h);
+    if (rc) return rc;
+    if (h->ext_mode) {
+        const uint64_t rb = band_regions(h);
+        for (int b = 0; b < h->pass_bands; ++b) {
+            if (!h->band_n[b] && h->band_state[b] != 2) continue;
+            rc = pass_launch(h, (uint64_t)b * rb, (uint64_t)(b + 1) * rb, h->d_band_sets + (size_t)b * P3_MAX_SETS, h->band_n[b], h->band_state[b]);
+            if (rc) return rc;
+        }
+        ext_leave(h);
+    } else {
+        const int empty = h->slots_dirty ? 2 : h->table_empty ? 1 : 0;
+        rc = pass_launch(h, h->reg_lo(), h->reg_hi(), h->d_sets, h->n_pend, empty);
+        if (rc) return rc;
+        h->n_pend = 0; h->arena_used = 0; h->pend_records = 0;
+        h->slots_dirty = false;
+        h->table_empty = false;
+    }
+    ++h->table_passes;
+    mark(h, "k_count_regions");
     return KQ_OK;
 }
 
@@ -1027,10 +1329,10 @@
     PartCfg c; plan_cfg(h, &c, true);
     return c.narrow != 0;
 }
-static int dest_take(kq_handle* h, const PartPlan& p, uint64_t n_max, Dest* d) {
+static int dest_take(kq_handle* h, const PartPlan& p, uint64_t n_max, Dest* d, const unsigned long long* bounds = nullptr, bool can_bound = false) {
     d->tight = tight_ok(h, p);
     if (d->tight) { d->fmt = FMT_TIGHT; d->aux_fmt = AUX_TIGHT; }
-    return arena_take(h, n_max, p.R, d);
+    return arena_take(h, n_max, p.R, d, bounds, can_bound);
 }
 static P3Set sort_to_regions(kq_handle* h, PartPlan* p, const LevelIn& in, const Dest& d) {
     const bool arena = d.in_arena();
@@ -1044,7 +1346,7 @@
         if (!arena && mid_to_2) { fin = p->recs1; fin_aux = p->a1(); }
         if (d.tight) fin_aux = nullptr;
         LevelCfg last = level_narrow(p->cfg, sb, false, t8);
-        if (d.tight) last.rstart = h->rstart;
+        if (d.tight) { last.rstart = h->rstart; last.disp = d.disp; last.disp_shift = d.disp_shift; }
         if (sb == 0) {
             last.n_seg = in.n_seg; last.spb = in.spb;
             run_level(h, p, last, in, fin, fin_aux, fin_base);
@@ -1089,15 +1391,24 @@
     const bool leveled = p.fmt == FMT_NARROW || p.fmt == FMT_TOP8 || p.two_level;
     Dest dst{p.fmt, AUX_IDX6};
     const bool filtered = p.cfg.filt_lo != 0 || p.cfg.filt_hi != p.cfg.map_count || h->windowed;
-    if (leveled && !filtered) { rc = dest_take(h, p, p.n_max, &dst); if (rc) return rc; }
+    const bool banded = leveled && tight_ok(h, p) && bands_ok(h, FMT_TIGHT) && p.cfg.n_coarse == (1u << NARROW_CBITS);
+    if (leveled && !filtered) { rc = dest_take(h, p, p.n_max, &dst, nullptr, banded); if (rc) return rc; }
     marks_reset(h);
     mark(h, "start");
     run_p1(h, &p, p.cfg, ab, lead, len, er, p.recs1, p.a1(), AUX_IDX6, pinv);
-    if (leveled && filtered) {
-        unsigned long long n_recs = 0;
-        HIPC(hipMemcpyAsync(&n_recs, p.total, sizeof n_recs, hipMemcpyDeviceToHost, h->stream));
-        HIPC(hipStreamSynchronize(h->stream));
-        rc = dest_take(h, p, std::min<uint64_t>(p.n_max, ((uint64_t)n_recs + 15) & ~7ull), &dst); if (rc) return rc;
+    if (leveled && (filtered || dst.need_bounds)) {
+        unsigned long long n_recs = 0, bounds[BANDS_MAX + 1];
+        if (banded) {
+            rc = band_scratch(h); if (rc) return rc;
+            HIPC(hipMemcpyAsync(h->pin, p.seg_off, sizeof(unsigned long long) * ((1u << NARROW_CBITS) + 1), hipMemcpyDeviceToHost, h->stream));
+            HIPC(hipStreamSynchronize(h->stream));
+            n_recs = h->pin[1u << NARROW_CBITS];
+            for (int b = 0; b <= h->pass_bands; ++b) bounds[b] = h->pin[(size_t)b * ((1u << NARROW_CBITS) / (uint32_t)h->pass_bands)];
+        } else {
+            HIPC(hipMemcpyAsync(&n_recs, p.total, sizeof n_recs, hipMemcpyDeviceToHost, h->stream));
+            HIPC(hipStreamSynchronize(h->stream));
+        }
+        rc = dest_take(h, p, filtered ? std::min<uint64_t>(p.n_max, ((uint64_t)n_recs + 15) & ~7ull) : p.n_max, &dst, banded ? bounds : nullptr, false); if (rc) return rc;
     }
     return submit(h, sort_to_regions(h, &p, own_segments(p, p.recs1, p.a1(), p.cfg.n_coarse), dst), dst);
 }
```

Result: no change. 51.42 billion, median of 3 (+0.2%).
